# SarodYatawatta/federated-pytorch-test

Hardware: NVIDIA H100
Metric: train_images_per_sec (higher is better)
Workload: dtype tf32

## Files before the change

federated_pytorch_test_b200/csrc/bindings.cpp:

```cpp
#include <ATen/cuda/CUDAContext.h>
#include <c10/cuda/CUDAGuard.h>
#include <torch/extension.h>

#include <cstdlib>

#include "fedb200.h"

namespace fb = fedb200;
using torch::Tensor;

static cudaStream_t cur_stream() { return at::cuda::getCurrentCUDAStream().stream(); }
static const float* fptr(const Tensor& t) { return t.data_ptr<float>(); }
static float* fptr_mut(Tensor& t) { return t.data_ptr<float>(); }
static const float* opt_ptr(const c10::optional<Tensor>& t) { return (t.has_value() && t->defined()) ? t->data_ptr<float>() : nullptr; }

#define CHECK_F32_CUDA(x) TORCH_CHECK((x).is_cuda() && (x).scalar_type() == torch::kFloat32, #x " must be a CUDA float32 tensor")
#define CHECK_CONTIG(x) TORCH_CHECK((x).is_contiguous(), #x " must be contiguous")

void adam_prox(Tensor x, Tensor g, Tensor m, Tensor v, Tensor step, double lr, double b1, double b2, double eps,
               c10::optional<Tensor> z, c10::optional<Tensor> y, double rho, double l1, double l2,
               c10::optional<Tensor> rho_dev) {
  CHECK_F32_CUDA(x); CHECK_CONTIG(x); CHECK_CONTIG(g); CHECK_CONTIG(m); CHECK_CONTIG(v);
  c10::cuda::CUDAGuard guard(x.device());
  fb::adam_prox(fptr_mut(x), fptr(g), fptr_mut(m), fptr_mut(v), step.data_ptr<int>(), (int)x.numel(), (float)lr, (float)b1,
                (float)b2, (float)eps, opt_ptr(z), opt_ptr(y), (float)rho, (float)l1, (float)l2, cur_stream(), opt_ptr(rho_dev));
}
void bump_step(Tensor step) {
  c10::cuda::CUDAGuard guard(step.device());
  fb::bump_step(step.data_ptr<int>(), cur_stream());
}
Tensor l1_l2(Tensor g) {
  CHECK_F32_CUDA(g); CHECK_CONTIG(g);
  c10::cuda::CUDAGuard guard(g.device());
  auto out = torch::empty({2}, g.options());
  fb::l1_l2(fptr(g), (int)g.numel(), fptr_mut(out), cur_stream());
  return out;
}
std::vector<Tensor> make_pair(Tensor g, Tensor gprev, Tensor d, double t, double trust) {
  CHECK_F32_CUDA(g); CHECK_CONTIG(g); CHECK_CONTIG(gprev); CHECK_CONTIG(d);
  c10::cuda::CUDAGuard guard(g.device());
  auto y = torch::empty_like(g), s = torch::empty_like(g);
  auto out = torch::empty({3}, g.options());
  fb::make_pair(fptr(g), fptr(gprev), fptr(d), (float)t, (float)trust, fptr_mut(y), fptr_mut(s), (int)g.numel(), fptr_mut(out), cur_stream());
  return {y, s, out};
}
Tensor welford(Tensor g, Tensor mean, Tensor m2, int64_t n_iter) {
  CHECK_F32_CUDA(g);
  c10::cuda::CUDAGuard guard(g.device());
  auto out = torch::empty({1}, g.options());
  fb::welford(fptr(g), fptr_mut(mean), fptr_mut(m2), (int)g.numel(), 1.0f / (float)n_iter, fptr_mut(out), cur_stream());
  return out;
}
Tensor penalty_value(Tensor x, c10::optional<Tensor> z, c10::optional<Tensor> y, double rho, double l1, double l2) {
  CHECK_F32_CUDA(x); CHECK_CONTIG(x);
  c10::cuda::CUDAGuard guard(x.device());
  auto out = torch::empty({1}, x.options());
  fb::penalty_value(fptr(x), opt_ptr(z), opt_ptr(y), (float)rho, (float)l1, (float)l2, (int)x.numel(), fptr_mut(out), cur_stream());
  return out;
}
void penalty_grad(Tensor g, Tensor x, c10::optional<Tensor> z, c10::optional<Tensor> y, double rho, double l1, double l2) {
  CHECK_F32_CUDA(g); CHECK_CONTIG(g); CHECK_CONTIG(x);
  c10::cuda::CUDAGuard guard(g.device());
  fb::penalty_grad(fptr_mut(g), fptr(x), opt_ptr(z), opt_ptr(y), (float)rho, (float)l1, (float)l2, (int)g.numel(), cur_stream());
}
Tensor multi_dot(std::vector<Tensor> a, std::vector<Tensor> b) {
  TORCH_CHECK(a.size() == b.size() && !a.empty() && a.size() <= 8, "multi_dot: 1..8 pairs");
  c10::cuda::CUDAGuard guard(a[0].device());
  std::vector<const float*> pa, pb;
  for (size_t i = 0; i < a.size(); ++i) {
    CHECK_F32_CUDA(a[i]); CHECK_CONTIG(a[i]); CHECK_CONTIG(b[i]);
    TORCH_CHECK(a[i].numel() == a[0].numel() && b[i].numel() == a[0].numel(), "multi_dot: equal lengths required");
    pa.push_back(fptr(a[i])); pb.push_back(fptr(b[i]));
  }
  auto out = torch::empty({(int64_t)a.size()}, a[0].options());
  fb::multi_dot(pa.data(), pb.data(), (int)a.size(), (int)a[0].numel(), fptr_mut(out), cur_stream());
  return out;
}
Tensor lbfgs_two_loop(Tensor Y, Tensor S, Tensor order, Tensor g, double hdiag) {
  CHECK_F32_CUDA(Y); CHECK_CONTIG(Y); CHECK_CONTIG(S); CHECK_CONTIG(g);
  TORCH_CHECK(order.scalar_type() == torch::kInt32 && order.is_cuda(), "order must be a CUDA int32 tensor");
  c10::cuda::CUDAGuard guard(g.device());
  const int k = (int)order.numel(), n = (int)g.numel();
  auto d = torch::empty_like(g);
  auto work = torch::empty({(int64_t)fb::lbfgs_two_loop_work_floats(k)}, g.options());
  fb::lbfgs_two_loop(fptr(Y), fptr(S), order.data_ptr<int>(), k, n, (int)Y.size(1), fptr(g), (float)hdiag, fptr_mut(d), fptr_mut(work), cur_stream());
  return d;
}

Tensor normalize_u8(Tensor u8, std::vector<double> mean, std::vector<double> stdv, int64_t c_out, bool to_nchw) {
  TORCH_CHECK(u8.is_cuda() && u8.scalar_type() == torch::kUInt8 && u8.dim() == 4 && u8.size(3) == 3 && u8.is_contiguous(),
              "normalize_u8 expects a contiguous CUDA uint8 [N,H,W,3] tensor");
  c10::cuda::CUDAGuard guard(u8.device());
  const int64_t N = u8.size(0), H = u8.size(1), W = u8.size(2);
  float m3[3] = {(float)mean[0], (float)mean[1], (float)mean[2]}, s3[3] = {(float)stdv[0], (float)stdv[1], (float)stdv[2]};
  auto opts = torch::TensorOptions().dtype(torch::kFloat32).device(u8.device());
  Tensor out = to_nchw ? torch::empty({N, 3, H, W}, opts) : torch::empty({N, H, W, c_out}, opts);
  fb::normalize_u8_nhwc(u8.data_ptr<uint8_t>(), fptr_mut(out), (int)(N * H * W), (int)c_out, m3, s3, to_nchw ? 1 : 0, (int)H, (int)W, cur_stream());
  return out;
}
Tensor augment_normalize_u8(Tensor u8, c10::optional<Tensor> rows, int64_t key, int64_t counter, std::vector<double> mean,
                            std::vector<double> stdv, bool to_nchw) {
  TORCH_CHECK(u8.is_cuda() && u8.scalar_type() == torch::kUInt8 && u8.dim() == 4 && u8.size(3) == 3 && u8.is_contiguous(),
              "augment_normalize_u8 expects a contiguous CUDA uint8 [N,H,W,3] tensor");
  TORCH_CHECK(counter >= 0, "augment_normalize_u8: negative counter");
  c10::cuda::CUDAGuard guard(u8.device());
  int64_t N = u8.size(0);
  const int64_t H = u8.size(1), W = u8.size(2);
  const int64_t* rp = nullptr;
  if (rows.has_value() && rows->defined()) {
    TORCH_CHECK(rows->is_cuda() && rows->device() == u8.device() && rows->scalar_type() == torch::kInt64 && rows->dim() == 1 &&
                    rows->is_contiguous(),
                "augment_normalize_u8: rows must be a contiguous int64 vector on the images' device");
    N = rows->numel();
    rp = rows->data_ptr<int64_t>();
  }
  TORCH_CHECK(N * H * W < (int64_t(1) << 31), "augment_normalize_u8: batch too large");
  float m3[3] = {(float)mean[0], (float)mean[1], (float)mean[2]}, s3[3] = {(float)stdv[0], (float)stdv[1], (float)stdv[2]};
  auto opts = torch::TensorOptions().dtype(torch::kFloat32).device(u8.device());
  Tensor out = to_nchw ? torch::empty({N, 3, H, W}, opts) : torch::empty({N, H, W, 3}, opts);
  if (N == 0) return out;
  fb::augment_normalize_u8(u8.data_ptr<uint8_t>(), rp, fptr_mut(out), (int)N, (int)H, (int)W, (uint64_t)key, (uint64_t)counter,
                           m3, s3, to_nchw ? 1 : 0, cur_stream());
  return out;
}
void col_stats(Tensor y, Tensor stats) {
  CHECK_F32_CUDA(y); CHECK_CONTIG(y);
  c10::cuda::CUDAGuard guard(y.device());
  const int C = (int)y.size(-1);
  fb::col_stats(fptr(y), fptr_mut(stats), (int)(y.numel() / C), C, cur_stream());
}
std::vector<Tensor> bn_elu_fwd(Tensor y, c10::optional<Tensor> stats, Tensor gamma, Tensor beta, c10::optional<Tensor> residual,
                               c10::optional<Tensor> running_mean, c10::optional<Tensor> running_var, double eps,
                               double momentum, bool act, bool self_clean, bool use_running) {
  CHECK_F32_CUDA(y); CHECK_CONTIG(y);
  c10::cuda::CUDAGuard guard(y.device());
  const int C = (int)y.size(-1);
  const int M = (int)(y.numel() / C);
  auto out = torch::empty_like(y);
  float* rm = (running_mean.has_value() && running_mean->defined()) ? running_mean->data_ptr<float>() : nullptr;
  float* rv = (running_var.has_value() && running_var->defined()) ? running_var->data_ptr<float>() : nullptr;
  if (use_running) {
    TORCH_CHECK(rm != nullptr && rv != nullptr, "bn_elu_fwd: use_running needs running_mean and running_var");
    fb::bn_elu_fwd(fptr(y), nullptr, fptr(gamma), fptr(beta), opt_ptr(residual), fptr_mut(out), rm, rv, nullptr, nullptr, M, C,
                   (float)eps, 0.f, act ? 1 : 0, 0, cur_stream(), 1);
    return {out, Tensor(), Tensor()};
  }
  TORCH_CHECK(stats.has_value() && stats->defined(), "bn_elu_fwd: stats required");
  auto sm = torch::empty({C}, y.options()), si = torch::empty({C}, y.options());
  TORCH_CHECK(stats->numel() >= 2 * C + (self_clean ? 1 : 0), "stats buffer too small");
  fb::bn_elu_fwd(fptr(y), stats->data_ptr<float>(), fptr(gamma), fptr(beta), opt_ptr(residual), fptr_mut(out), rm, rv, fptr_mut(sm),
                 fptr_mut(si), M, C, (float)eps, (float)momentum, act ? 1 : 0, self_clean ? 1 : 0, cur_stream());
  return {out, sm, si};
}
std::vector<Tensor> bn_elu_bwd(Tensor dout, c10::optional<Tensor> out, Tensor y, Tensor mean, Tensor invstd, Tensor gamma,
                               c10::optional<Tensor> beta, c10::optional<Tensor> dgamma, c10::optional<Tensor> dbeta,
                               bool want_dres, bool act, c10::optional<Tensor> sums_buf) {
  CHECK_F32_CUDA(dout); CHECK_CONTIG(dout); CHECK_CONTIG(y);
  c10::cuda::CUDAGuard guard(y.device());
  const int C = (int)y.size(-1);
  const int M = (int)(y.numel() / C);
  const float* outp = nullptr;
  if (out.has_value() && out->defined()) { CHECK_CONTIG((*out)); outp = out->data_ptr<float>(); }
  const float* betap = opt_ptr(beta);
  static const bool fused_optin = [] { const char* e = std::getenv("FEDB200_BN_BWD_FUSED"); return e != nullptr && std::atoi(e) != 0; }();
  const bool persistent = !fused_optin && sums_buf.has_value() && sums_buf->defined();
  if (persistent) TORCH_CHECK(sums_buf->numel() == 2 * C + 1 && sums_buf->is_contiguous(), "bn_elu_bwd: sums buffer must be [2C + 1]");
  auto sums = persistent ? *sums_buf : torch::empty({2 * C + 1}, y.options());
  auto dy = torch::empty_like(y);
  Tensor dres;
  if (want_dres) dres = torch::empty_like(y);
  float* dg = (dgamma.has_value() && dgamma->defined()) ? dgamma->data_ptr<float>() : nullptr;
  float* db = (dbeta.has_value() && dbeta->defined()) ? dbeta->data_ptr<float>() : nullptr;
  if (fused_optin && fb::bn_elu_bwd_fused(fptr(dout), outp, fptr(y), fptr(mean), fptr(invstd), fptr(gamma), betap, fptr_mut(sums),
                                          fptr_mut(dy), want_dres ? dres.data_ptr<float>() : nullptr, dg, db, M, C, act ? 1 : 0,
                                          cur_stream()))
    return {dy, dres};
  fb::bn_elu_bwd_reduce(fptr(dout), outp, fptr(y), fptr(mean), fptr(invstd), fptr(gamma), betap, fptr_mut(sums), M, C,
                        act ? 1 : 0, persistent ? 1 : 0, cur_stream());
  fb::bn_elu_bwd_apply(fptr(dout), outp, fptr(y), fptr(mean), fptr(invstd), fptr(gamma), betap, fptr_mut(sums), fptr_mut(dy),
                       want_dres ? dres.data_ptr<float>() : nullptr, dg, db, M, C, act ? 1 : 0, persistent ? 1 : 0, cur_stream());
  return {dy, dres};
}
std::vector<Tensor> head_fwd(Tensor x, Tensor w, c10::optional<Tensor> bias) {
  CHECK_F32_CUDA(x); CHECK_CONTIG(x); CHECK_F32_CUDA(w); CHECK_CONTIG(w);
  TORCH_CHECK(x.dim() == 4 && w.dim() == 2 && x.size(3) == w.size(1), "head_fwd: x [N,H,W,C], w [O,C]");
  c10::cuda::CUDAGuard guard(x.device());
  const int NB = (int)x.size(0), HW = (int)(x.size(1) * x.size(2)), C = (int)x.size(3), O = (int)w.size(0);
  auto pooled = torch::empty({NB, C}, x.options());
  auto logits = torch::empty({NB, O}, x.options());
  fb::head_fwd(fptr(x), fptr(w), opt_ptr(bias), fptr_mut(pooled), fptr_mut(logits), NB, HW, C, O, cur_stream());
  return {logits, pooled};
}
Tensor head_bwd(Tensor dlogits, Tensor w, int64_t H, int64_t W) {
  CHECK_F32_CUDA(dlogits); CHECK_CONTIG(dlogits); CHECK_F32_CUDA(w); CHECK_CONTIG(w);
  c10::cuda::CUDAGuard guard(dlogits.device());
  const int NB = (int)dlogits.size(0), O = (int)dlogits.size(1), C = (int)w.size(1);
  auto dx = torch::empty({NB, H, W, C}, dlogits.options());
  fb::head_bwd(fptr(dlogits), fptr(w), fptr_mut(dx), NB, (int)(H * W), C, O, cur_stream());
  return dx;
}
Tensor avgpool_nhwc(Tensor x) {
  CHECK_F32_CUDA(x); CHECK_CONTIG(x);
  c10::cuda::CUDAGuard guard(x.device());
  auto out = torch::empty({x.size(0), x.size(3)}, x.options());
  fb::avgpool_nhwc(fptr(x), fptr_mut(out), (int)x.size(0), (int)(x.size(1) * x.size(2)), (int)x.size(3), cur_stream());
  return out;
}
Tensor avgpool_nhwc_bwd(Tensor dout, int64_t H, int64_t W) {
  CHECK_F32_CUDA(dout); CHECK_CONTIG(dout);
  c10::cuda::CUDAGuard guard(dout.device());
  auto dx = torch::empty({dout.size(0), H, W, dout.size(1)}, dout.options());
  fb::avgpool_nhwc_bwd(fptr(dout), fptr_mut(dx), (int)dout.size(0), (int)(H * W), (int)dout.size(1), cur_stream());
  return dx;
}
Tensor weight_flip(Tensor w) {
  CHECK_F32_CUDA(w); CHECK_CONTIG(w);
  c10::cuda::CUDAGuard guard(w.device());
  auto out = torch::empty({w.size(3), w.size(1), w.size(2), w.size(0)}, w.options());
  fb::weight_krsc_flip(fptr(w), fptr_mut(out), (int)w.size(0), (int)w.size(3), (int)w.size(1), (int)w.size(2), cur_stream());
  return out;
}

Tensor convT_pack(Tensor w) {
  CHECK_F32_CUDA(w);
  TORCH_CHECK(w.dim() == 4 && w.size(2) == 4 && w.size(3) == 4, "convT_pack: ConvTranspose2d(k=4) weight expected");
  c10::cuda::CUDAGuard guard(w.device());
  auto out = torch::empty({4 * w.size(1), 3, 3, w.size(0)}, w.options().memory_format(c10::MemoryFormat::Contiguous));
  fb::convT_pack(fptr(w), fptr_mut(out), (int)w.size(0), (int)w.size(1), w.stride(0), w.stride(1), w.stride(2), w.stride(3), cur_stream());
  return out;
}

Tensor linear_tf32(Tensor x, Tensor w, c10::optional<Tensor> bias, bool act) {
  CHECK_F32_CUDA(x); CHECK_F32_CUDA(w); CHECK_CONTIG(x); CHECK_CONTIG(w);
  TORCH_CHECK(x.dim() == 2 && w.dim() == 2 && x.size(1) == w.size(1), "linear_tf32: x [M,K], w [N,K]");
  c10::cuda::CUDAGuard guard(x.device());
  const int M = (int)x.size(0), K = (int)x.size(1), N = (int)w.size(0);
  auto out = torch::empty({M, N}, x.options());
  fb::linear_tf32(fptr(x), fptr(w), opt_ptr(bias), fptr_mut(out), M, N, K, K, K, N, act ? 1 : 0, cur_stream());
  return out;
}
bool conv_supported(int64_t H_out, int64_t W_out, int64_t C_in, int64_t stride) {
  return fb::conv_geometry_supported((int)H_out, (int)W_out, (int)C_in, (int)stride);
}
int64_t conv_orientation(int64_t NB, int64_t H_out, int64_t W_out, int64_t C_out, int64_t stride) {
  return fb::pick_conv_orientation((int)NB, (int)H_out, (int)W_out, (int)C_out, (int)stride);
}
bool conv_window_reuse(int64_t H_out, int64_t W_out, int64_t C_in, int64_t C_out, int64_t kh, int64_t stride, int64_t dil) {
  return fb::conv_window_reuse((int)H_out, (int)W_out, (int)C_in, (int)C_out, (int)kh, (int)stride, (int)dil);
}
Tensor conv2d_nhwc(Tensor x, Tensor w, c10::optional<Tensor> stats, int64_t stride, int64_t pad, int64_t dil, int64_t orient) {
  CHECK_F32_CUDA(x); CHECK_F32_CUDA(w); CHECK_CONTIG(x); CHECK_CONTIG(w);
  TORCH_CHECK(x.dim() == 4 && w.dim() == 4 && x.size(3) == w.size(3), "conv2d_nhwc: x [N,H,W,Ci], w [Co,kh,kw,Ci]");
  c10::cuda::CUDAGuard guard(x.device());
  const int NB = (int)x.size(0), H = (int)x.size(1), W = (int)x.size(2), Ci = (int)x.size(3);
  const int Co = (int)w.size(0), kh = (int)w.size(1), kw = (int)w.size(2);
  const int Ho = (H + 2 * (int)pad - (int)dil * (kh - 1) - 1) / (int)stride + 1;
  const int Wo = (W + 2 * (int)pad - (int)dil * (kw - 1) - 1) / (int)stride + 1;
  auto y = torch::empty({NB, Ho, Wo, Co}, x.options());
  float* st = (stats.has_value() && stats->defined()) ? stats->data_ptr<float>() : nullptr;
  fb::conv2d_nhwc_tf32(fptr(x), fptr(w), fptr_mut(y), st, NB, H, W, Ci, Co, kh, kw, (int)stride, (int)pad, (int)dil, Ho, Wo, cur_stream(),
                       (int)orient);
  return y;
}

Tensor conv2d_nhwc_sized(Tensor x, Tensor w, c10::optional<Tensor> stats, int64_t stride, int64_t pad, int64_t dil,
                         int64_t Ho, int64_t Wo) {
  CHECK_F32_CUDA(x); CHECK_F32_CUDA(w); CHECK_CONTIG(x); CHECK_CONTIG(w);
  TORCH_CHECK(x.dim() == 4 && w.dim() == 4 && x.size(3) == w.size(3), "conv2d_nhwc: x [N,H,W,Ci], w [Co,kh,kw,Ci]");
  TORCH_CHECK(Ho > 0 && Wo > 0, "conv2d_nhwc_sized: positive output size");
  c10::cuda::CUDAGuard guard(x.device());
  const int NB = (int)x.size(0), H = (int)x.size(1), W = (int)x.size(2), Ci = (int)x.size(3);
  const int Co = (int)w.size(0), kh = (int)w.size(1), kw = (int)w.size(2);
  auto y = torch::empty({NB, Ho, Wo, Co}, x.options());
  float* st = (stats.has_value() && stats->defined()) ? stats->data_ptr<float>() : nullptr;
  fb::conv2d_nhwc_tf32(fptr(x), fptr(w), fptr_mut(y), st, NB, H, W, Ci, Co, kh, kw, (int)stride, (int)pad, (int)dil, (int)Ho,
                       (int)Wo, cur_stream());
  return y;
}

bool conv_wgrad_supported(int64_t Cx, int64_t Co, int64_t stride, int64_t Wo, int64_t Ho) {
  return fb::conv_wgrad_supported((int)Cx, (int)Co, (int)stride, (int)Wo, (int)Ho);
}
void conv_wgrad(Tensor x, Tensor dy, Tensor dw, int64_t stride, int64_t pad, int64_t dil) {
  CHECK_F32_CUDA(x); CHECK_F32_CUDA(dy); CHECK_F32_CUDA(dw); CHECK_CONTIG(x); CHECK_CONTIG(dy); CHECK_CONTIG(dw);
  TORCH_CHECK(x.dim() == 4 && dy.dim() == 4 && dw.dim() == 4 && x.size(0) == dy.size(0) && dw.size(0) == dy.size(3) &&
              dw.size(3) <= x.size(3), "conv_wgrad: x [N,H,W,Cx], dy [N,Ho,Wo,Co], dw [Co,kh,kw,Cw<=Cx]");
  c10::cuda::CUDAGuard guard(x.device());
  const int NB = (int)x.size(0), H = (int)x.size(1), W = (int)x.size(2), Cx = (int)x.size(3);
  const int Ho = (int)dy.size(1), Wo = (int)dy.size(2), Co = (int)dy.size(3);
  const int kh = (int)dw.size(1), kw = (int)dw.size(2), Cw = (int)dw.size(3);
  fb::conv_wgrad_tf32(fptr(x), fptr(dy), fptr_mut(dw), NB, H, W, Cx, Cw, Co, kh, kw, (int)stride, (int)pad, (int)dil, Ho, Wo,
                      cur_stream());
}

bool conv_shuffle_supported(int64_t Ho, int64_t Wo, int64_t Cin, int64_t Ci) {
  return fb::conv_shuffle_supported((int)Ho, (int)Wo, (int)Cin, (int)Ci);
}
Tensor conv2d_nhwc_shuffle(Tensor x, Tensor w, int64_t pad, int64_t Ho, int64_t Wo) {
  CHECK_F32_CUDA(x); CHECK_F32_CUDA(w); CHECK_CONTIG(x); CHECK_CONTIG(w);
  TORCH_CHECK(x.dim() == 4 && w.dim() == 4 && x.size(3) == w.size(3) && w.size(0) % 4 == 0, "conv2d_nhwc_shuffle: x [N,H,W,Cin], w [4*Ci,kh,kw,Cin]");
  c10::cuda::CUDAGuard guard(x.device());
  const int NB = (int)x.size(0), H = (int)x.size(1), W = (int)x.size(2), Cin = (int)x.size(3);
  const int C4 = (int)w.size(0), kh = (int)w.size(1), kw = (int)w.size(2);
  auto out = torch::empty({NB, 2 * Ho, 2 * Wo, C4 / 4}, x.options());
  fb::conv2d_nhwc_shuffle_tf32(fptr(x), fptr(w), fptr_mut(out), NB, H, W, Cin, C4, kh, kw, (int)pad, (int)Ho, (int)Wo, cur_stream());
  return out;
}

bool conv_multidil_supported(int64_t Ho, int64_t Wo, int64_t Ci, int64_t stride, int64_t branches) {
  return fb::conv_multidil_supported((int)Ho, (int)Wo, (int)Ci, (int)stride, (int)branches);
}
Tensor conv2d_nhwc_multidil(Tensor x, Tensor w, c10::optional<Tensor> bias, bool act, int64_t kh, int64_t stride,
                            std::vector<int64_t> dils, std::vector<int64_t> pads, int64_t Ho, int64_t Wo) {
  CHECK_F32_CUDA(x); CHECK_F32_CUDA(w); CHECK_CONTIG(x); CHECK_CONTIG(w);
  TORCH_CHECK(x.dim() == 4 && w.dim() == 4 && x.size(3) == w.size(3), "conv2d_nhwc_multidil: x [N,H,W,Ci], w [Co,B*kh,kw,Ci]");
  const int B = (int)dils.size();
  TORCH_CHECK(B >= 1 && B <= 8 && (int)pads.size() == B && w.size(1) == B * kh, "conv2d_nhwc_multidil: branch tables");
  c10::cuda::CUDAGuard guard(x.device());
  const int NB = (int)x.size(0), H = (int)x.size(1), W = (int)x.size(2), Ci = (int)x.size(3);
  const int Co = (int)w.size(0), kw = (int)w.size(2);
  if (bias.has_value() && bias->defined()) TORCH_CHECK(bias->numel() == Co && bias->is_contiguous(), "bias must be [Co]");
  int d[8], pd[8];
  for (int b = 0; b < B; ++b) { d[b] = (int)dils[b]; pd[b] = (int)pads[b]; }
  auto y = torch::empty({NB, Ho, Wo, Co}, x.options());
  fb::conv2d_nhwc_multidil_tf32(fptr(x), fptr(w), opt_ptr(bias), act ? 1 : 0, fptr_mut(y), NB, H, W, Ci, Co, B, (int)kh, kw,
                                (int)stride, d, pd, (int)Ho, (int)Wo, cur_stream());
  return y;
}

Tensor conv2d_nhwc_accumulate(Tensor x, Tensor w, Tensor y, int64_t stride, int64_t pad, int64_t dil, int64_t orient) {
  CHECK_F32_CUDA(x); CHECK_F32_CUDA(w); CHECK_F32_CUDA(y); CHECK_CONTIG(x); CHECK_CONTIG(w); CHECK_CONTIG(y);
  TORCH_CHECK(x.dim() == 4 && w.dim() == 4 && y.dim() == 4 && x.size(3) == w.size(3), "conv2d_nhwc_accumulate: x [N,H,W,Ci], w [Co,kh,kw,Ci]");
  c10::cuda::CUDAGuard guard(x.device());
  const int NB = (int)x.size(0), H = (int)x.size(1), W = (int)x.size(2), Ci = (int)x.size(3);
  const int Co = (int)w.size(0), kh = (int)w.size(1), kw = (int)w.size(2);
  const int Ho = (H + 2 * (int)pad - (int)dil * (kh - 1) - 1) / (int)stride + 1;
  const int Wo = (W + 2 * (int)pad - (int)dil * (kw - 1) - 1) / (int)stride + 1;
  TORCH_CHECK(y.size(0) == NB && y.size(1) == Ho && y.size(2) == Wo && y.size(3) == Co, "conv2d_nhwc_accumulate: y must be [N,Ho,Wo,Co]");
  fb::conv2d_nhwc_accumulate_tf32(fptr(x), fptr(w), fptr_mut(y), NB, H, W, Ci, Co, kh, kw, (int)stride, (int)pad, (int)dil, Ho, Wo,
                                  cur_stream(), (int)orient);
  return y;
}

Tensor conv2d_nhwc_bias_act(Tensor x, Tensor w, c10::optional<Tensor> bias, bool act, int64_t stride, int64_t pad, int64_t dil) {
  CHECK_F32_CUDA(x); CHECK_F32_CUDA(w); CHECK_CONTIG(x); CHECK_CONTIG(w);
  TORCH_CHECK(x.dim() == 4 && w.dim() == 4 && x.size(3) == w.size(3), "conv2d_nhwc: x [N,H,W,Ci], w [Co,kh,kw,Ci]");
  c10::cuda::CUDAGuard guard(x.device());
  const int NB = (int)x.size(0), H = (int)x.size(1), W = (int)x.size(2), Ci = (int)x.size(3);
  const int Co = (int)w.size(0), kh = (int)w.size(1), kw = (int)w.size(2);
  const int Ho = (H + 2 * (int)pad - (int)dil * (kh - 1) - 1) / (int)stride + 1;
  const int Wo = (W + 2 * (int)pad - (int)dil * (kw - 1) - 1) / (int)stride + 1;
  TORCH_CHECK(Ho > 0 && Wo > 0, "conv2d_nhwc_bias_act: empty output");
  if (bias.has_value() && bias->defined()) TORCH_CHECK(bias->numel() == Co && bias->is_contiguous(), "bias must be [Co]");
  auto y = torch::empty({NB, Ho, Wo, Co}, x.options());
  fb::conv2d_nhwc_bias_act_tf32(fptr(x), fptr(w), opt_ptr(bias), act ? 1 : 0, fptr_mut(y), NB, H, W, Ci, Co, kh, kw, (int)stride,
                                (int)pad, (int)dil, Ho, Wo, cur_stream());
  return y;
}

Tensor conv2d_nhwc_bn_eval(Tensor x, Tensor w, Tensor gamma, Tensor beta, Tensor running_mean, Tensor running_var, double eps,
                           c10::optional<Tensor> residual, bool act, int64_t stride, int64_t pad) {
  CHECK_F32_CUDA(x); CHECK_F32_CUDA(w); CHECK_CONTIG(x); CHECK_CONTIG(w);
  TORCH_CHECK(x.dim() == 4 && w.dim() == 4 && x.size(3) == w.size(3), "conv2d_nhwc_bn_eval: x [N,H,W,Ci], w [Co,kh,kw,Ci]");
  c10::cuda::CUDAGuard guard(x.device());
  const int NB = (int)x.size(0), H = (int)x.size(1), W = (int)x.size(2), Ci = (int)x.size(3);
  const int Co = (int)w.size(0), kh = (int)w.size(1), kw = (int)w.size(2);
  const int Ho = (H + 2 * (int)pad - (kh - 1) - 1) / (int)stride + 1;
  const int Wo = (W + 2 * (int)pad - (kw - 1) - 1) / (int)stride + 1;
  TORCH_CHECK(Ho > 0 && Wo > 0, "conv2d_nhwc_bn_eval: empty output");
  for (const Tensor* t : {&gamma, &beta, &running_mean, &running_var}) {
    CHECK_F32_CUDA((*t));
    TORCH_CHECK(t->numel() == Co && t->is_contiguous(), "conv2d_nhwc_bn_eval: BatchNorm parameters and statistics must be [Co]");
  }
  const float* res = nullptr;
  if (residual.has_value() && residual->defined()) {
    CHECK_F32_CUDA((*residual)); CHECK_CONTIG((*residual));
    TORCH_CHECK(residual->dim() == 4 && residual->size(0) == NB && residual->size(1) == Ho && residual->size(2) == Wo &&
                residual->size(3) == Co, "conv2d_nhwc_bn_eval: residual must be [N,Ho,Wo,Co]");
    res = residual->data_ptr<float>();
    TORCH_CHECK((reinterpret_cast<uintptr_t>(res) & 15) == 0, "conv2d_nhwc_bn_eval: residual must be 16-byte aligned");
  }
  auto y = torch::empty({NB, Ho, Wo, Co}, x.options());
  fb::conv2d_nhwc_bn_eval_tf32(fptr(x), fptr(w), fptr(gamma), fptr(beta), fptr(running_mean), fptr(running_var), (float)eps, res,
                               act ? 1 : 0, fptr_mut(y), NB, H, W, Ci, Co, kh, kw, (int)stride, (int)pad, 1, Ho, Wo, cur_stream());
  return y;
}

std::vector<Tensor> cross_entropy_fwd(Tensor logits, Tensor labels) {
  CHECK_F32_CUDA(logits); CHECK_CONTIG(logits);
  TORCH_CHECK(labels.scalar_type() == torch::kInt64 && labels.is_cuda(), "labels must be CUDA int64");
  c10::cuda::CUDAGuard guard(logits.device());
  auto loss = torch::empty({}, logits.options());
  auto probs = torch::empty_like(logits);
  fb::cross_entropy_fwd(fptr(logits), (const long long*)labels.data_ptr<int64_t>(), fptr_mut(loss), fptr_mut(probs),
                        (int)logits.size(0), (int)logits.size(1), cur_stream());
  return {loss, probs};
}
Tensor cross_entropy_bwd(Tensor probs, Tensor labels, Tensor gout) {
  c10::cuda::CUDAGuard guard(probs.device());
  auto d = torch::empty_like(probs);
  auto g = gout.contiguous();
  fb::cross_entropy_bwd(fptr(probs), (const long long*)labels.data_ptr<int64_t>(), fptr(g), fptr_mut(d), (int)probs.size(0),
                        (int)probs.size(1), cur_stream());
  return d;
}
Tensor vae_loss_fwd(Tensor recon, Tensor x, Tensor mu, Tensor logvar) {
  CHECK_F32_CUDA(recon); CHECK_CONTIG(recon); CHECK_CONTIG(x); CHECK_CONTIG(mu); CHECK_CONTIG(logvar);
  c10::cuda::CUDAGuard guard(recon.device());
  auto out = torch::empty({}, recon.options());
  fb::vae_loss_fwd(fptr(recon), fptr(x), (int)recon.numel(), fptr(mu), fptr(logvar), (int)mu.numel(), fptr_mut(out), cur_stream());
  return out;
}
std::vector<Tensor> vae_loss_bwd(Tensor recon, Tensor x, Tensor mu, Tensor logvar, Tensor gout) {
  c10::cuda::CUDAGuard guard(recon.device());
  auto dr = torch::empty_like(recon), dm = torch::empty_like(mu), dl = torch::empty_like(logvar);
  auto g = gout.contiguous();
  fb::vae_loss_bwd(fptr(recon), fptr(x), (int)recon.numel(), fptr(mu), fptr(logvar), (int)mu.numel(), fptr(g), fptr_mut(dr),
                   fptr_mut(dm), fptr_mut(dl), cur_stream());
  return {dr, dm, dl};
}

Tensor linear_f32(Tensor x, Tensor w, c10::optional<Tensor> bias, bool act) {
  CHECK_F32_CUDA(x); CHECK_F32_CUDA(w); CHECK_CONTIG(x); CHECK_CONTIG(w);
  TORCH_CHECK(x.dim() == 2 && w.dim() == 2 && x.size(1) == w.size(1), "linear_f32: x [M,K], w [N,K]");
  c10::cuda::CUDAGuard guard(x.device());
  const int M = (int)x.size(0), K = (int)x.size(1), N = (int)w.size(0);
  auto out = torch::empty({M, N}, x.options());
  fb::gemm_f32(fptr(x), fptr(w), opt_ptr(bias), fptr_mut(out), M, N, K, K, 1, 1, K, N, act ? 1 : 0, 0, cur_stream());
  return out;
}
Tensor linear_f32_dgrad(Tensor dz, Tensor w) {
  CHECK_F32_CUDA(dz); CHECK_F32_CUDA(w); CHECK_CONTIG(dz); CHECK_CONTIG(w);
  c10::cuda::CUDAGuard guard(dz.device());
  const int M = (int)dz.size(0), N = (int)dz.size(1), K = (int)w.size(1);
  auto dx = torch::empty({M, K}, dz.options());
  fb::gemm_f32(fptr(dz), fptr(w), nullptr, fptr_mut(dx), M, K, N, N, 1, K, 1, K, 0, 0, cur_stream());
  return dx;
}
void linear_f32_wgrad(Tensor dz, Tensor x, Tensor dw, bool accumulate) {
  CHECK_F32_CUDA(dz); CHECK_F32_CUDA(x); CHECK_F32_CUDA(dw); CHECK_CONTIG(dz); CHECK_CONTIG(x); CHECK_CONTIG(dw);
  c10::cuda::CUDAGuard guard(dz.device());
  const int M = (int)dz.size(0), N = (int)dz.size(1), K = (int)x.size(1);
  TORCH_CHECK(dw.size(0) == N && dw.size(1) == K && x.size(0) == M, "linear_f32_wgrad: shape mismatch");
  fb::gemm_f32(fptr(dz), fptr(x), nullptr, fptr_mut(dw), N, K, M, 1, N, K, 1, K, 0, accumulate ? 1 : 0, cur_stream());
}
void act_bwd_bias(Tensor dout, c10::optional<Tensor> out, c10::optional<Tensor> dz, c10::optional<Tensor> db, bool act) {
  CHECK_F32_CUDA(dout); CHECK_CONTIG(dout);
  c10::cuda::CUDAGuard guard(dout.device());
  const int C = (int)dout.size(-1);
  float* dzp = (dz.has_value() && dz->defined()) ? dz->data_ptr<float>() : nullptr;
  float* dbp = (db.has_value() && db->defined()) ? db->data_ptr<float>() : nullptr;
  TORCH_CHECK(!act || (out.has_value() && out->defined()), "act_bwd_bias: the activation output is needed for ELU'");
  fb::act_bwd_bias(fptr(dout), opt_ptr(out), dzp, dbp, (long long)dout.numel(), C, act ? 1 : 0, cur_stream());
}
std::vector<Tensor> maxpool2x2_fwd(Tensor x) {
  CHECK_F32_CUDA(x);
  TORCH_CHECK(x.dim() == 4, "maxpool2x2: 4-D tensor expected");
  const bool nhwc = !x.is_contiguous() && x.is_contiguous(at::MemoryFormat::ChannelsLast);
  TORCH_CHECK(nhwc || x.is_contiguous(), "maxpool2x2: contiguous or channels_last input");
  c10::cuda::CUDAGuard guard(x.device());
  const int N = (int)x.size(0), C = (int)x.size(1), H = (int)x.size(2), W = (int)x.size(3);
  auto fmt = nhwc ? at::MemoryFormat::ChannelsLast : at::MemoryFormat::Contiguous;
  auto y = torch::empty({N, C, H / 2, W / 2}, x.options().memory_format(fmt));
  auto idx = torch::empty({N, C, H / 2, W / 2}, x.options().dtype(torch::kUInt8).memory_format(fmt));
  fb::maxpool2x2_fwd(fptr(x), fptr_mut(y), idx.data_ptr<uint8_t>(), N, C, H, W, nhwc ? 1 : 0, cur_stream());
  return {y, idx};
}
Tensor maxpool2x2_bwd(Tensor dy, Tensor idx, int64_t H, int64_t W) {
  CHECK_F32_CUDA(dy);
  const bool nhwc = !idx.is_contiguous() && idx.is_contiguous(at::MemoryFormat::ChannelsLast);
  auto fmt = nhwc ? at::MemoryFormat::ChannelsLast : at::MemoryFormat::Contiguous;
  Tensor d = dy.contiguous(fmt);
  c10::cuda::CUDAGuard guard(dy.device());
  const int N = (int)dy.size(0), C = (int)dy.size(1);
  auto dx = torch::empty({N, C, H, W}, dy.options().memory_format(fmt));
  fb::maxpool2x2_bwd(fptr(d), idx.data_ptr<uint8_t>(), fptr_mut(dx), N, C, (int)H, (int)W, nhwc ? 1 : 0, cur_stream());
  return dx;
}
void argmax_count(Tensor logits, Tensor labels, Tensor counter) {
  CHECK_F32_CUDA(logits); CHECK_CONTIG(logits);
  TORCH_CHECK(labels.scalar_type() == torch::kInt64 && counter.scalar_type() == torch::kInt64 && counter.numel() >= 2, "argmax_count: int64 labels / counter[2]");
  c10::cuda::CUDAGuard guard(logits.device());
  fb::argmax_count(fptr(logits), (const long long*)labels.data_ptr<int64_t>(), (long long*)counter.data_ptr<int64_t>(), (int)logits.size(0),
                   (int)logits.size(1), cur_stream());
}
int64_t info_nce_max_p() { return fb::info_nce_max_p(); }
int64_t info_nce_scratch_floats() { return fb::info_nce_scratch_floats(); }
std::vector<Tensor> info_nce_fwd(Tensor Z, Tensor Zh, Tensor scratch) {
  CHECK_F32_CUDA(Z); CHECK_F32_CUDA(Zh); CHECK_CONTIG(Z); CHECK_CONTIG(Zh);
  c10::cuda::CUDAGuard guard(Z.device());
  const int R = (int)Z.size(0), P = (int)Z.size(1);
  auto loss = torch::empty({}, Z.options());
  auto coef = torch::empty({(int64_t)P * P + 2 * P}, Z.options());
  fb::info_nce_fwd(fptr(Z), fptr(Zh), R, P, fptr_mut(scratch), fptr_mut(loss), fptr_mut(coef), cur_stream());
  return {loss, coef};
}
std::vector<Tensor> info_nce_bwd(Tensor Z, Tensor Zh, Tensor coef, Tensor gout) {
  CHECK_F32_CUDA(Z); CHECK_CONTIG(Z); CHECK_CONTIG(Zh);
  c10::cuda::CUDAGuard guard(Z.device());
  auto dZ = torch::empty_like(Z), dZh = torch::empty_like(Zh);
  fb::info_nce_bwd(fptr(Z), fptr(Zh), fptr(coef), fptr(gout), fptr_mut(dZ), fptr_mut(dZh), (int)Z.size(0), (int)Z.size(1), cur_stream());
  return {dZ, dZh};
}
Tensor gauss_nll_rows_fwd(Tensor x, Tensor mu, Tensor s2) {
  CHECK_F32_CUDA(x); CHECK_F32_CUDA(mu); CHECK_F32_CUDA(s2); CHECK_CONTIG(x); CHECK_CONTIG(mu); CHECK_CONTIG(s2);
  c10::cuda::CUDAGuard guard(x.device());
  const int B = (int)x.size(0), D = (int)x.size(1), rows = (int)mu.size(0);
  TORCH_CHECK(mu.size(1) == D && rows % B == 0, "gauss_nll_rows: mu [k*B, D]");
  auto out = torch::empty({rows}, x.options());
  fb::gauss_nll_rows_fwd(fptr(x), fptr(mu), fptr(s2), fptr_mut(out), rows, B, D, cur_stream());
  return out;
}
std::vector<Tensor> gauss_nll_rows_bwd(Tensor x, Tensor mu, Tensor s2, Tensor grow) {
  CHECK_F32_CUDA(x); CHECK_CONTIG(x); CHECK_CONTIG(mu); CHECK_CONTIG(s2); CHECK_CONTIG(grow);
  c10::cuda::CUDAGuard guard(x.device());
  auto dmu = torch::empty_like(mu), ds2 = torch::empty_like(s2);
  fb::gauss_nll_rows_bwd(fptr(x), fptr(mu), fptr(s2), fptr(grow), fptr_mut(dmu), fptr_mut(ds2), (int)mu.size(0), (int)x.size(0),
                         (int)x.size(1), cur_stream());
  return {dmu, ds2};
}
bool smallconv_supported(int64_t Ci, int64_t Co, int64_t k) { return fb::smallconv_supported((int)Ci, (int)Co, (int)k); }
std::vector<Tensor> smallconv_fwd(Tensor x, Tensor w, c10::optional<Tensor> bias, int64_t pad, bool act, bool pool) {
  CHECK_F32_CUDA(x); CHECK_F32_CUDA(w); CHECK_CONTIG(x); CHECK_CONTIG(w);
  c10::cuda::CUDAGuard guard(x.device());
  const int NB = (int)x.size(0), Ci = (int)x.size(1), H = (int)x.size(2), W = (int)x.size(3), Co = (int)w.size(0), k = (int)w.size(2);
  const int Ho = H + 2 * (int)pad - k + 1, Wo = W + 2 * (int)pad - k + 1;
  auto y = torch::empty({NB, Co, pool ? Ho / 2 : Ho, pool ? Wo / 2 : Wo}, x.options());
  Tensor idx = pool ? torch::empty(y.sizes(), x.options().dtype(torch::kUInt8)) : torch::empty({0}, x.options().dtype(torch::kUInt8));
  fb::smallconv_fwd(fptr(x), fptr(w), opt_ptr(bias), fptr_mut(y), pool ? idx.data_ptr<uint8_t>() : nullptr, NB, Ci, H, W, Co, k,
                    (int)pad, act ? 1 : 0, pool ? 1 : 0, cur_stream());
  return {y, idx};
}
Tensor smallconv_unpool_actbwd(Tensor dy, Tensor yout, Tensor idx, int64_t Ho, int64_t Wo, bool act, bool pool) {
  CHECK_F32_CUDA(dy); CHECK_CONTIG(dy); CHECK_CONTIG(yout);
  c10::cuda::CUDAGuard guard(dy.device());
  auto dz = torch::empty({dy.size(0), dy.size(1), Ho, Wo}, dy.options());
  fb::smallconv_unpool_actbwd(fptr(dy), fptr(yout), pool ? idx.data_ptr<uint8_t>() : nullptr, fptr_mut(dz),
                              (long long)(dy.size(0) * dy.size(1)), (int)Ho, (int)Wo, act ? 1 : 0, pool ? 1 : 0, cur_stream());
  return dz;
}
Tensor smallconv_dgrad(Tensor dz, Tensor w, int64_t H, int64_t W, int64_t pad) {
  CHECK_F32_CUDA(dz); CHECK_CONTIG(dz); CHECK_CONTIG(w);
  c10::cuda::CUDAGuard guard(dz.device());
  const int NB = (int)dz.size(0), Co = (int)w.size(0), Ci = (int)w.size(1), k = (int)w.size(2);
  auto dx = torch::empty({NB, Ci, H, W}, dz.options());
  fb::smallconv_dgrad(fptr(dz), fptr(w), fptr_mut(dx), NB, Ci, (int)H, (int)W, Co, k, (int)pad, cur_stream());
  return dx;
}
void smallconv_wgrad(Tensor dz, Tensor x, Tensor dw, c10::optional<Tensor> db, int64_t pad) {
  CHECK_F32_CUDA(dz); CHECK_CONTIG(dz); CHECK_CONTIG(x); CHECK_CONTIG(dw);
  c10::cuda::CUDAGuard guard(dz.device());
  const int NB = (int)x.size(0), Ci = (int)x.size(1), H = (int)x.size(2), W = (int)x.size(3), Co = (int)dw.size(0), k = (int)dw.size(2);
  float* dbp = (db.has_value() && db->defined()) ? db->data_ptr<float>() : nullptr;
  fb::smallconv_wgrad(fptr(dz), fptr(x), fptr_mut(dw), dbp, NB, Ci, H, W, Co, k, (int)pad, cur_stream());
}

static void set_dp(fb::CommArgs& a, double dp_std, int64_t dp_key, const c10::optional<Tensor>& dp_t,
                   const c10::optional<Tensor>& dp_stats, const c10::optional<Tensor>& dp_valid) {
  if (!dp_t.has_value() || !dp_t->defined()) return;
  TORCH_CHECK(dp_t->is_cuda() && dp_t->scalar_type() == at::kLong && dp_t->numel() >= 1, "DP round counter: int64 CUDA tensor");
  TORCH_CHECK(dp_stats.has_value() && dp_stats->defined() && dp_stats->numel() >= fb::DP_STATS_FLOATS,
              "DP rounds need the dp_clip stats record");
  CHECK_F32_CUDA((*dp_stats));
  a.dp = 1;
  a.dp_std = (float)dp_std;
  a.dp_key = (unsigned long long)dp_key;
  a.dp_t = reinterpret_cast<long long*>(dp_t->data_ptr<int64_t>());
  a.dp_stats = dp_stats->data_ptr<float>() + fb::DP_NORM;
  if (dp_valid.has_value() && dp_valid->defined()) {
    TORCH_CHECK(dp_valid->is_cuda() && dp_valid->scalar_type() == at::kByte && dp_valid->is_contiguous() &&
                    dp_valid->numel() >= (a.n + fb::DP_CHUNK - 1) / fb::DP_CHUNK,
                "DP parameter layout: uint8 CUDA tensor with one count per 32-float chunk of the block");
    a.dp_valid = dp_valid->data_ptr<uint8_t>();
  }
}
static void set_q(fb::CommArgs& a, const std::vector<int64_t>& local_idx, int64_t q_bits, int64_t q_group, int64_t q_key,
                  const c10::optional<Tensor>& q_t, const std::vector<int64_t>& q_code_ptrs,
                  const std::vector<int64_t>& q_scale_ptrs, const std::vector<Tensor>& q_ef,
                  const c10::optional<Tensor>& q_part) {
  if (q_bits == 0) return;
  TORCH_CHECK(q_bits == 8 || q_bits == 4, "compressed rounds take 8 or 4 bits, got ", q_bits);
  TORCH_CHECK(q_group == fb::Q_GROUP, "compressed rounds use groups of ", fb::Q_GROUP, " coordinates, got ", q_group);
  TORCH_CHECK(q_t.has_value() && q_t->defined() && q_t->is_cuda() && q_t->scalar_type() == at::kLong && q_t->numel() >= 1,
              "compressed round counter: int64 CUDA tensor");
  TORCH_CHECK(q_part.has_value() && q_part->defined() && q_part->numel() >= fb::Q_PART_FLOATS, "compressed rounds need the statistics buffer");
  CHECK_F32_CUDA((*q_part));
  TORCH_CHECK((int)q_code_ptrs.size() == a.K && (int)q_scale_ptrs.size() == a.K, "compressed rounds need K payload pointers");
  TORCH_CHECK(q_ef.empty() || (int)q_ef.size() == a.n_local, "error feedback: one slice per local replica");
  a.qbits = (int)q_bits;
  a.q_key = (unsigned long long)q_key;
  a.q_t = reinterpret_cast<long long*>(q_t->data_ptr<int64_t>());
  a.q_part = q_part->data_ptr<float>();
  for (int k = 0; k < a.K; ++k) {
    TORCH_CHECK(q_code_ptrs[k] % 16 == 0 && q_scale_ptrs[k] % 4 == 0, "payload slices must be 16-byte aligned");
    a.q_codes[k] = reinterpret_cast<unsigned char*>(q_code_ptrs[k]);
    a.q_scales[k] = reinterpret_cast<float*>(q_scale_ptrs[k]);
  }
  for (int j = 0; j < a.n_local; ++j) {
    a.q_worker[j] = (int)local_idx[j];
    if (!q_ef.empty()) {
      CHECK_F32_CUDA(q_ef[j]); CHECK_CONTIG(q_ef[j]);
      TORCH_CHECK(q_ef[j].numel() == a.n, "error feedback slices must have the block's length");
      a.q_ef[j] = q_ef[j].data_ptr<float>();
    }
  }
}
static void set_samp(fb::CommArgs& a, int64_t samp_S, int64_t samp_key, const c10::optional<Tensor>& samp_t,
                     const c10::optional<Tensor>& client_n) {
  if (samp_S == 0) return;
  TORCH_CHECK(samp_t.has_value() && samp_t->defined() && samp_t->is_cuda() && samp_t->scalar_type() == at::kLong &&
                  samp_t->numel() >= 1, "sampled round counter: int64 CUDA tensor");
  TORCH_CHECK(client_n.has_value() && client_n->defined() && client_n->is_cuda() && client_n->scalar_type() == at::kInt &&
                  client_n->is_contiguous() && client_n->numel() == a.K, "sample counts: one int32 CUDA value per worker");
  a.samp_S = (int)samp_S;
  a.samp_key = (unsigned long long)samp_key;
  a.samp_t = reinterpret_cast<long long*>(samp_t->data_ptr<int64_t>());
  a.client_n = client_n->data_ptr<int>();
}
static void fill_ctrl(uint32_t** dst, const std::vector<int64_t>& ctrl_ptrs, int world) {
  for (int p = 0; p < world && p < (int)ctrl_ptrs.size(); ++p) dst[p] = reinterpret_cast<uint32_t*>(ctrl_ptrs[p]);
}
void block_reduce(int64_t mode, std::vector<int64_t> x_ptrs, std::vector<int64_t> y_ptrs, std::vector<int64_t> local_idx,
                  Tensor z, int64_t n, double rho, c10::optional<Tensor> rho_dev, Tensor out, Tensor scratch,
                  std::vector<int64_t> ctrl_ptrs, Tensor sync, int64_t world, int64_t rank, int64_t mc_x, int64_t mc_y,
                  int64_t mc_z, std::vector<int64_t> xw_ptrs, std::vector<int64_t> zw_ptrs, bool two_shot,
                  int64_t max_blocks, double timeout_s, int64_t agg, int64_t trim_b, double dp_std, int64_t dp_key,
                  c10::optional<Tensor> dp_t, c10::optional<Tensor> dp_stats, c10::optional<Tensor> dp_valid,
                  int64_t q_bits, int64_t q_group, int64_t q_key,
                  c10::optional<Tensor> q_t, std::vector<int64_t> q_code_ptrs, std::vector<int64_t> q_scale_ptrs,
                  std::vector<Tensor> q_ef, c10::optional<Tensor> q_part, int64_t samp_S, int64_t samp_key,
                  c10::optional<Tensor> samp_t, c10::optional<Tensor> client_n) {
  CHECK_F32_CUDA(z); CHECK_F32_CUDA(out); CHECK_F32_CUDA(scratch);
  TORCH_CHECK(out.numel() >= fb::COMM_OUT_FLOATS && scratch.numel() >= fb::COMM_SCRATCH_FLOATS, "out / scratch too small");
  c10::cuda::CUDAGuard guard(z.device());
  fb::CommArgs a{};
  a.mode = (int)mode; a.K = (int)x_ptrs.size(); a.n_local = (int)local_idx.size(); a.world = (int)world; a.rank = (int)rank;
  a.n = (int)n; a.rho = (float)rho; a.rho_dev = opt_ptr(rho_dev);
  a.two_shot = two_shot ? 1 : 0; a.max_blocks = (int)max_blocks;
  TORCH_CHECK(a.K <= fb::COMM_MAX_K && a.n_local <= fb::COMM_MAX_LOCAL && a.world <= fb::COMM_MAX_WORLD, "block_reduce: limits exceeded");
  for (int k = 0; k < a.K; ++k) {
    a.x[k] = reinterpret_cast<const float*>(x_ptrs[k]);
    a.y[k] = y_ptrs.empty() ? nullptr : reinterpret_cast<const float*>(y_ptrs[k]);
  }
  for (int j = 0; j < a.n_local; ++j) {
    a.xl[j] = reinterpret_cast<float*>(x_ptrs[local_idx[j]]);
    a.yl[j] = y_ptrs.empty() ? nullptr : reinterpret_cast<float*>(y_ptrs[local_idx[j]]);
  }
  for (int p = 0; p < a.world; ++p) {
    a.xw[p] = p < (int)xw_ptrs.size() ? reinterpret_cast<float*>(xw_ptrs[p]) : nullptr;
    a.zw[p] = p < (int)zw_ptrs.size() ? reinterpret_cast<float*>(zw_ptrs[p]) : nullptr;
  }
  if (a.two_shot) {
    if (a.mode == 0) {
      TORCH_CHECK(mc_x != 0 || (int)xw_ptrs.size() == a.world, "two-shot FedAvg needs broadcast targets");
    } else {
      TORCH_CHECK(mc_z != 0 || (int)zw_ptrs.size() == a.world, "two-shot FedProx/ADMM needs peer-mapped z");
    }
  }
  a.mc_x = reinterpret_cast<float*>(mc_x);
  a.mc_y = reinterpret_cast<float*>(mc_y);
  a.mc_z = reinterpret_cast<float*>(mc_z);
  a.z = z.data_ptr<float>();
  a.out = out.data_ptr<float>();
  a.scratch = scratch.data_ptr<float>();
  fill_ctrl(a.ctrl, ctrl_ptrs, a.world);
  a.sync = reinterpret_cast<uint32_t*>(sync.data_ptr<int>());
  a.timeout_cycles = (long long)(timeout_s * 1.9e9);
  a.agg = (int)agg; a.trim_b = (int)trim_b;
  set_dp(a, dp_std, dp_key, dp_t, dp_stats, dp_valid);
  set_q(a, local_idx, q_bits, q_group, q_key, q_t, q_code_ptrs, q_scale_ptrs, q_ef, q_part);
  set_samp(a, samp_S, samp_key, samp_t, client_n);
  fb::block_reduce_launch(a, cur_stream());
}

void block_reduce_fedopt(int64_t opt, double lr, double beta1, double beta2, double tau, Tensor m, c10::optional<Tensor> v,
                         std::vector<int64_t> x_ptrs, std::vector<int64_t> local_idx, Tensor z, int64_t n, Tensor out,
                         Tensor scratch, std::vector<int64_t> ctrl_ptrs, Tensor sync, int64_t world, int64_t rank,
                         int64_t mc_x, int64_t mc_m, int64_t mc_v, std::vector<int64_t> xw_ptrs,
                         std::vector<int64_t> mw_ptrs, std::vector<int64_t> vw_ptrs, bool two_shot, int64_t max_blocks,
                         double timeout_s, int64_t agg, int64_t trim_b, double dp_std, int64_t dp_key,
                         c10::optional<Tensor> dp_t, c10::optional<Tensor> dp_stats,
                         c10::optional<Tensor> dp_valid, int64_t q_bits, int64_t q_group, int64_t q_key,
                         c10::optional<Tensor> q_t, std::vector<int64_t> q_code_ptrs, std::vector<int64_t> q_scale_ptrs,
                         std::vector<Tensor> q_ef, c10::optional<Tensor> q_part, int64_t samp_S, int64_t samp_key,
                         c10::optional<Tensor> samp_t, c10::optional<Tensor> client_n) {
  TORCH_CHECK(opt >= fb::FEDOPT_AVGM && opt <= fb::FEDOPT_YOGI, "block_reduce_fedopt: unknown server optimizer ", opt);
  const bool adaptive = opt != fb::FEDOPT_AVGM;
  CHECK_F32_CUDA(z); CHECK_F32_CUDA(out); CHECK_F32_CUDA(scratch); CHECK_F32_CUDA(m); CHECK_CONTIG(m);
  TORCH_CHECK(out.numel() >= fb::COMM_OUT_FLOATS && scratch.numel() >= fb::COMM_SCRATCH_FLOATS, "out / scratch too small");
  TORCH_CHECK(z.numel() == n && m.numel() == n, "block_reduce_fedopt: z and m must have the block's length");
  if (adaptive) {
    TORCH_CHECK(v.has_value() && v->defined(), "block_reduce_fedopt: adaptive server optimizers need v");
    CHECK_F32_CUDA((*v)); CHECK_CONTIG((*v));
    TORCH_CHECK(v->numel() == n, "block_reduce_fedopt: v must have the block's length");
  }
  c10::cuda::CUDAGuard guard(z.device());
  fb::CommArgs a{};
  a.mode = 0; a.K = (int)x_ptrs.size(); a.n_local = (int)local_idx.size(); a.world = (int)world; a.rank = (int)rank;
  a.n = (int)n; a.two_shot = two_shot ? 1 : 0; a.max_blocks = (int)max_blocks;
  TORCH_CHECK(a.K <= fb::COMM_MAX_K && a.n_local <= fb::COMM_MAX_LOCAL && a.world <= fb::COMM_MAX_WORLD,
              "block_reduce_fedopt: limits exceeded");
  for (int k = 0; k < a.K; ++k) a.x[k] = reinterpret_cast<const float*>(x_ptrs[k]);
  for (int j = 0; j < a.n_local; ++j) a.xl[j] = reinterpret_cast<float*>(x_ptrs[local_idx[j]]);
  for (int p = 0; p < a.world; ++p) {
    a.xw[p] = p < (int)xw_ptrs.size() ? reinterpret_cast<float*>(xw_ptrs[p]) : nullptr;
    a.mw[p] = p < (int)mw_ptrs.size() ? reinterpret_cast<float*>(mw_ptrs[p]) : nullptr;
    a.vw[p] = p < (int)vw_ptrs.size() ? reinterpret_cast<float*>(vw_ptrs[p]) : nullptr;
  }
  if (a.two_shot) {
    TORCH_CHECK(mc_x != 0 || (int)xw_ptrs.size() == a.world, "two-shot FedOpt needs broadcast targets for the weights");
    TORCH_CHECK(mc_m != 0 || (int)mw_ptrs.size() == a.world, "two-shot FedOpt needs peer-mapped m");
    TORCH_CHECK(!adaptive || mc_v != 0 || (int)vw_ptrs.size() == a.world, "two-shot FedOpt needs peer-mapped v");
  }
  a.mc_x = reinterpret_cast<float*>(mc_x);
  a.mc_m = reinterpret_cast<float*>(mc_m);
  a.mc_v = reinterpret_cast<float*>(mc_v);
  a.z = z.data_ptr<float>();
  a.out = out.data_ptr<float>();
  a.scratch = scratch.data_ptr<float>();
  fill_ctrl(a.ctrl, ctrl_ptrs, a.world);
  a.sync = reinterpret_cast<uint32_t*>(sync.data_ptr<int>());
  a.timeout_cycles = (long long)(timeout_s * 1.9e9);
  a.opt = (int)opt;
  a.lr = (float)lr; a.beta1 = (float)beta1; a.beta2 = (float)beta2; a.tau = (float)tau;
  a.m = m.data_ptr<float>();
  a.v = adaptive ? v->data_ptr<float>() : nullptr;
  a.agg = (int)agg; a.trim_b = (int)trim_b;
  set_dp(a, dp_std, dp_key, dp_t, dp_stats, dp_valid);
  set_q(a, local_idx, q_bits, q_group, q_key, q_t, q_code_ptrs, q_scale_ptrs, q_ef, q_part);
  set_samp(a, samp_S, samp_key, samp_t, client_n);
  fb::block_reduce_launch(a, cur_stream());
}

void dp_clip(std::vector<Tensor> xs, Tensor z, double bound, Tensor stats, int64_t max_blocks) {
  TORCH_CHECK(!xs.empty() && xs.size() <= (size_t)fb::COMM_MAX_LOCAL, "dp_clip: bad replica count");
  CHECK_F32_CUDA(z); CHECK_CONTIG(z); CHECK_F32_CUDA(stats);
  TORCH_CHECK(stats.numel() >= fb::DP_STATS_FLOATS, "dp_clip: stats too small");
  c10::cuda::CUDAGuard guard(z.device());
  fb::DPClipArgs a{};
  a.n = (int)z.numel(); a.n_local = (int)xs.size(); a.max_blocks = (int)max_blocks; a.bound = (float)bound;
  for (int j = 0; j < a.n_local; ++j) {
    CHECK_F32_CUDA(xs[j]); CHECK_CONTIG(xs[j]);
    TORCH_CHECK(xs[j].numel() == a.n, "dp_clip: block slices must have z's length");
    a.x[j] = fptr_mut(xs[j]);
  }
  a.z = fptr(z);
  a.stats = fptr_mut(stats);
  fb::dp_clip_launch(a, cur_stream());
}

void bb_update(std::vector<Tensor> xs, std::vector<Tensor> ys, std::vector<Tensor> yhat0s, std::vector<Tensor> x0s, Tensor z,
               std::vector<int64_t> workers, int64_t K, Tensor rho_dev, Tensor log, Tensor scratch, Tensor out,
               std::vector<int64_t> ctrl_ptrs, Tensor sync, int64_t world, int64_t rank, double epsilon, double alphacorrmin,
               double rhomax, bool seed_only, int64_t max_blocks, double timeout_s) {
  TORCH_CHECK(!xs.empty() && xs.size() == x0s.size() && xs.size() <= (size_t)fb::COMM_MAX_LOCAL, "bb_update: bad replica count");
  CHECK_F32_CUDA(z); CHECK_F32_CUDA(rho_dev); CHECK_F32_CUDA(log); CHECK_F32_CUDA(scratch);
  TORCH_CHECK(log.numel() >= 8 * K && scratch.numel() >= fb::BB_SCRATCH_FLOATS, "bb_update: log / scratch too small");
  c10::cuda::CUDAGuard guard(z.device());
  fb::BBArgs a{};
  a.K = (int)K; a.n_local = (int)xs.size(); a.world = (int)world; a.rank = (int)rank; a.n = (int)xs[0].numel();
  a.seed_only = seed_only ? 1 : 0; a.max_blocks = (int)max_blocks;
  a.epsilon = (float)epsilon; a.alphacorrmin = (float)alphacorrmin; a.rhomax = (float)rhomax;
  for (int j = 0; j < a.n_local; ++j) {
    CHECK_F32_CUDA(xs[j]); CHECK_CONTIG(xs[j]); CHECK_CONTIG(x0s[j]);
    TORCH_CHECK(xs[j].numel() == a.n && x0s[j].numel() == a.n, "bb_update: equal lengths required");
    a.x[j] = fptr(xs[j]);
    a.x0[j] = fptr_mut(x0s[j]);
    if (!seed_only) {
      CHECK_CONTIG(ys[j]); CHECK_CONTIG(yhat0s[j]);
      a.y[j] = fptr(ys[j]);
      a.yhat0[j] = fptr_mut(yhat0s[j]);
    }
    a.worker[j] = (int)workers[j];
  }
  a.z = fptr(z);
  a.rho_dev = fptr_mut(rho_dev);
  a.log = fptr_mut(log);
  a.scratch = fptr_mut(scratch);
  a.out = fptr_mut(out);
  fill_ctrl(a.ctrl, ctrl_ptrs, a.world);
  a.sync = reinterpret_cast<uint32_t*>(sync.data_ptr<int>());
  a.timeout_cycles = (long long)(timeout_s * 1.9e9);
  fb::bb_update_launch(a, cur_stream());
}

py::bytes ipc_get_handle(int64_t ptr) {
  cudaIpcMemHandle_t h;
  cudaError_t e = cudaIpcGetMemHandle(&h, reinterpret_cast<void*>(ptr));
  TORCH_CHECK(e == cudaSuccess, "cudaIpcGetMemHandle: ", cudaGetErrorString(e));
  return py::bytes(reinterpret_cast<const char*>(&h), sizeof(h));
}
int64_t ipc_open_handle(py::bytes handle) {
  std::string s = handle;
  TORCH_CHECK(s.size() == sizeof(cudaIpcMemHandle_t), "bad IPC handle size");
  cudaIpcMemHandle_t h;
  memcpy(&h, s.data(), sizeof(h));
  void* p = nullptr;
  cudaError_t e = cudaIpcOpenMemHandle(&p, h, cudaIpcMemLazyEnablePeerAccess);
  TORCH_CHECK(e == cudaSuccess, "cudaIpcOpenMemHandle: ", cudaGetErrorString(e));
  return reinterpret_cast<int64_t>(p);
}
void ipc_close_handle(int64_t ptr) { cudaIpcCloseMemHandle(reinterpret_cast<void*>(ptr)); }

int64_t launch_count() { return (int64_t)fb::launch_count(); }

PYBIND11_MODULE(TORCH_EXTENSION_NAME, m) {
  m.doc() = "federated_pytorch_test_b200: hand-written sm_90a kernels";
  m.def("launch_count", &launch_count);
  m.def("adam_prox", &adam_prox);
  m.def("bump_step", &bump_step);
  m.def("l1_l2", &l1_l2);
  m.def("make_pair", &make_pair);
  m.def("welford", &welford);
  m.def("penalty_value", &penalty_value);
  m.def("penalty_grad", &penalty_grad);
  m.def("multi_dot", &multi_dot);
  m.def("lbfgs_two_loop", &lbfgs_two_loop);
  m.def("normalize_u8", &normalize_u8);
  m.def("augment_normalize_u8", &augment_normalize_u8, py::arg("u8"), py::arg("rows"), py::arg("key"), py::arg("counter"),
        py::arg("mean"), py::arg("std"), py::arg("to_nchw"));
  m.def("col_stats", &col_stats);
  m.def("head_fwd", &head_fwd);
  m.def("head_bwd", &head_bwd);
  m.def("bn_elu_fwd", &bn_elu_fwd, py::arg("y"), py::arg("stats"), py::arg("gamma"), py::arg("beta"), py::arg("residual"),
        py::arg("running_mean"), py::arg("running_var"), py::arg("eps"), py::arg("momentum"), py::arg("act"),
        py::arg("self_clean"), py::arg("use_running") = false);
  m.def("bn_elu_bwd", &bn_elu_bwd);
  m.def("avgpool_nhwc", &avgpool_nhwc);
  m.def("avgpool_nhwc_bwd", &avgpool_nhwc_bwd);
  m.def("weight_flip", &weight_flip);
  m.def("convT_pack", &convT_pack);
  m.def("linear_tf32", &linear_tf32);
  m.def("conv_supported", &conv_supported);
  m.def("conv_orientation", &conv_orientation);
  m.def("conv_window_reuse", &conv_window_reuse, py::arg("H_out"), py::arg("W_out"), py::arg("C_in"), py::arg("C_out"), py::arg("kh"),
        py::arg("stride") = 1, py::arg("dil") = 1);
  m.def("conv2d_nhwc", &conv2d_nhwc, py::arg("x"), py::arg("w"), py::arg("stats"), py::arg("stride"), py::arg("pad"), py::arg("dil"),
        py::arg("orient") = -1);
  m.def("conv2d_nhwc_sized", &conv2d_nhwc_sized);
  m.def("conv2d_nhwc_bias_act", &conv2d_nhwc_bias_act);
  m.def("conv2d_nhwc_bn_eval", &conv2d_nhwc_bn_eval);
  m.def("conv2d_nhwc_accumulate", &conv2d_nhwc_accumulate, py::arg("x"), py::arg("w"), py::arg("y"), py::arg("stride"), py::arg("pad"),
        py::arg("dil"), py::arg("orient") = -1);
  m.def("conv2d_nhwc_shuffle", &conv2d_nhwc_shuffle);
  m.def("conv_shuffle_supported", &conv_shuffle_supported);
  m.def("conv2d_nhwc_multidil", &conv2d_nhwc_multidil);
  m.def("conv_multidil_supported", &conv_multidil_supported);
  m.def("conv_wgrad", &conv_wgrad);
  m.def("conv_wgrad_supported", &conv_wgrad_supported);
  m.def("cross_entropy_fwd", &cross_entropy_fwd);
  m.def("cross_entropy_bwd", &cross_entropy_bwd);
  m.def("vae_loss_fwd", &vae_loss_fwd);
  m.def("vae_loss_bwd", &vae_loss_bwd);
  m.def("linear_f32", &linear_f32);
  m.def("linear_f32_dgrad", &linear_f32_dgrad);
  m.def("linear_f32_wgrad", &linear_f32_wgrad);
  m.def("act_bwd_bias", &act_bwd_bias);
  m.def("maxpool2x2_fwd", &maxpool2x2_fwd);
  m.def("maxpool2x2_bwd", &maxpool2x2_bwd);
  m.def("argmax_count", &argmax_count);
  m.def("info_nce_max_p", &info_nce_max_p);
  m.def("info_nce_scratch_floats", &info_nce_scratch_floats);
  m.def("info_nce_fwd", &info_nce_fwd);
  m.def("info_nce_bwd", &info_nce_bwd);
  m.def("gauss_nll_rows_fwd", &gauss_nll_rows_fwd);
  m.def("gauss_nll_rows_bwd", &gauss_nll_rows_bwd);
  m.def("smallconv_supported", &smallconv_supported);
  m.def("smallconv_fwd", &smallconv_fwd);
  m.def("smallconv_unpool_actbwd", &smallconv_unpool_actbwd);
  m.def("smallconv_dgrad", &smallconv_dgrad);
  m.def("smallconv_wgrad", &smallconv_wgrad);
  m.def("block_reduce", &block_reduce);
  m.def("block_reduce_fedopt", &block_reduce_fedopt);
  m.def("dp_clip", &dp_clip);
  m.def("bb_update", &bb_update);
  m.def("ipc_get_handle", &ipc_get_handle);
  m.def("ipc_open_handle", &ipc_open_handle);
  m.def("ipc_close_handle", &ipc_close_handle);
}
```

federated_pytorch_test_b200/csrc/fedb200.h:

```cpp
#pragma once
#include <cuda_runtime.h>
#include <stdint.h>

namespace fedb200 {

void count_launch(int n = 1);
long long launch_count();

bool pdl_enabled();
#ifdef __CUDACC__
__device__ __forceinline__ void pdl_wait() { asm volatile("griddepcontrol.wait;" ::: "memory"); }
__device__ __forceinline__ void pdl_launch_dependents() { asm volatile("griddepcontrol.launch_dependents;" ::: "memory"); }
__device__ __forceinline__ void pdl_prologue() {
  pdl_launch_dependents();
  pdl_wait();
}
template <typename... KArgs, typename... Args>
inline cudaError_t launch_pdl(void (*kernel)(KArgs...), dim3 grid, dim3 block, size_t smem, cudaStream_t stream,
                              Args&&... args) {
  cudaLaunchConfig_t cfg{};
  cfg.gridDim = grid;
  cfg.blockDim = block;
  cfg.dynamicSmemBytes = smem;
  cfg.stream = stream;
  cudaLaunchAttribute attr[1];
  attr[0].id = cudaLaunchAttributeProgrammaticStreamSerialization;
  attr[0].val.programmaticStreamSerializationAllowed = pdl_enabled() ? 1 : 0;
  cfg.attrs = attr;
  cfg.numAttrs = 1;
  return cudaLaunchKernelEx(&cfg, kernel, KArgs(args)...);
}
#endif

int pick_block_n(int M, int N);
void linear_tf32(const float* x, const float* w, const float* bias, float* out, int M, int N, int K, int ldx, int ldw,
                 int ldo, int act, cudaStream_t stream);
bool conv_geometry_supported(int H_out, int W_out, int C_in, int stride);
enum { CONV_ORIENT_AUTO = -1, CONV_ORIENT_ROW = 0, CONV_ORIENT_PIXEL = 1, CONV_ORIENT_PIXEL_PERTAP = 2 };
int pick_conv_orientation(int NB, int H_out, int W_out, int C_out, int stride);
bool conv_window_reuse(int H_out, int W_out, int C_in, int C_out, int kh, int stride, int dil);
void conv2d_nhwc_tf32(const float* x, const float* w, float* y, float* stats, int NB, int H, int W, int C_in, int C_out,
                      int kh, int kw, int stride, int pad, int dil, int H_out, int W_out, cudaStream_t stream,
                      int orient = CONV_ORIENT_AUTO);
void conv2d_nhwc_accumulate_tf32(const float* x, const float* w, float* y, int NB, int H, int W, int C_in, int C_out, int kh,
                                 int kw, int stride, int pad, int dil, int H_out, int W_out, cudaStream_t stream,
                                 int orient = CONV_ORIENT_AUTO);
void conv2d_nhwc_bias_act_tf32(const float* x, const float* w, const float* bias, int act, float* y, int NB, int H, int W,
                               int C_in, int C_out, int kh, int kw, int stride, int pad, int dil, int H_out, int W_out,
                               cudaStream_t stream);
void conv2d_nhwc_bn_eval_tf32(const float* x, const float* w, const float* gamma, const float* beta, const float* mean,
                              const float* var, float eps, const float* residual, int act, float* y, int NB, int H, int W,
                              int C_in, int C_out, int kh, int kw, int stride, int pad, int dil, int H_out, int W_out,
                              cudaStream_t stream);

bool conv_shuffle_supported(int H_out, int W_out, int C_in, int Ci_out);
void conv2d_nhwc_shuffle_tf32(const float* x, const float* w, float* out, int NB, int H, int W, int C_in, int C4, int kh, int kw,
                              int pad, int H_out, int W_out, cudaStream_t stream);
bool conv_multidil_supported(int H_out, int W_out, int C_in, int stride, int branches);
void conv2d_nhwc_multidil_tf32(const float* x, const float* w, const float* bias, int act, float* y, int NB, int H, int W, int C_in,
                               int C_out, int branches, int kh, int kw, int stride, const int* dils, const int* pads, int H_out,
                               int W_out, cudaStream_t stream);
bool conv_wgrad_supported(int C_x, int C_out, int stride, int W_out, int H_out);
void conv_wgrad_tf32(const float* x, const float* dy, float* dw, int NB, int H, int W, int C_x, int C_w, int C_out, int kh,
                     int kw, int stride, int pad, int dil, int H_out, int W_out, cudaStream_t stream);


void adam_prox(float* x, const float* g, float* m, float* v, const int* step_dev, int n, float lr, float b1, float b2,
               float eps, const float* z, const float* y, float rho, float l1, float l2, cudaStream_t s,
               const float* rho_dev = nullptr);
void bump_step(int* step_dev, cudaStream_t s);
void l1_l2(const float* g, int n, float* out2, cudaStream_t s);
void make_pair(const float* g, const float* gprev, const float* d, float t, float trust, float* y, float* sv, int n,
               float* out3, cudaStream_t s);
void welford(const float* g, float* mean, float* m2, int n, float inv_n, float* out1, cudaStream_t s);
void penalty_value(const float* x, const float* z, const float* y, float rho, float l1, float l2, int n, float* out1,
                   cudaStream_t s);
void penalty_grad(float* g, const float* x, const float* z, const float* y, float rho, float l1, float l2, int n,
                  cudaStream_t s);
void multi_dot(const float* const* a, const float* const* b, int npairs, int n, float* out, cudaStream_t s);
void lbfgs_two_loop(const float* Y, const float* S, const int* order, int k, int n, int ld, const float* g, float hdiag,
                    float* d, float* work, cudaStream_t s);
size_t lbfgs_two_loop_work_floats(int k);

void normalize_u8_nhwc(const uint8_t* in, float* out, int npix, int c_out, const float* mean3, const float* std3,
                       int to_nchw, int H, int W, cudaStream_t s);
void augment_normalize_u8(const uint8_t* in, const int64_t* rows, float* out, int n, int H, int W, uint64_t key,
                          uint64_t counter, const float* mean3, const float* std3, int to_nchw, cudaStream_t s);
void col_stats(const float* y, float* stats, int M, int C, cudaStream_t s);
void bn_elu_fwd(const float* y, float* stats, const float* gamma, const float* beta, const float* residual,
                float* out, float* running_mean, float* running_var, float* save_mean, float* save_invstd, int M, int C,
                float eps, float momentum, int act, int self_clean, cudaStream_t s, int use_running = 0);
void bn_elu_bwd_reduce(const float* dout, const float* out, const float* y, const float* mean, const float* invstd,
                       const float* gamma, const float* beta, float* sums, int M, int C, int act, int sums_clean, cudaStream_t s);
void bn_elu_bwd_apply(const float* dout, const float* out, const float* y, const float* mean, const float* invstd,
                      const float* gamma, const float* beta, float* sums, float* dy, float* dres, float* dgamma,
                      float* dbeta, int M, int C, int act, int self_clean, cudaStream_t s);
bool bn_elu_bwd_fused(const float* dout, const float* out, const float* y, const float* mean, const float* invstd,
                      const float* gamma, const float* beta, float* sums, float* dy, float* dres, float* dgamma,
                      float* dbeta, int M, int C, int act, cudaStream_t s);
void head_fwd(const float* x, const float* w, const float* bias, float* pooled, float* logits, int NB, int HW, int C, int O,
              cudaStream_t s);
void head_bwd(const float* dlogits, const float* w, float* dx, int NB, int HW, int C, int O, cudaStream_t s);
void avgpool_nhwc(const float* x, float* out, int NB, int HW, int C, cudaStream_t s);
void avgpool_nhwc_bwd(const float* dout, float* dx, int NB, int HW, int C, cudaStream_t s);
void weight_krsc_flip(const float* w, float* out, int C_out, int C_in, int kh, int kw, cudaStream_t s);
void convT_pack(const float* w, float* out, int Ci, int Co, long long s_ci, long long s_co, long long s_r, long long s_s, cudaStream_t s);

void cross_entropy_fwd(const float* logits, const long long* labels, float* loss, float* probs, int B, int C,
                       cudaStream_t s);
void cross_entropy_bwd(const float* probs, const long long* labels, const float* gout, float* dlogits, int B, int C,
                       cudaStream_t s);
void vae_loss_fwd(const float* recon, const float* x, int n, const float* mu, const float* logvar, int nl, float* out,
                  cudaStream_t s);
void vae_loss_bwd(const float* recon, const float* x, int n, const float* mu, const float* logvar, int nl,
                  const float* gout, float* drecon, float* dmu, float* dlogvar, cudaStream_t s);

void gemm_f32(const float* a, const float* b, const float* bias, float* c, int M, int N, int K, long long sa_i, long long sa_k,
              long long sb_k, long long sb_j, int ldc, int act, int accumulate, cudaStream_t s);
void act_bwd_bias(const float* dout, const float* out, float* dz, float* db, long long total, int C, int act, cudaStream_t s);
void maxpool2x2_fwd(const float* x, float* y, unsigned char* idx, int N, int C, int H, int W, int nhwc, cudaStream_t s);
void maxpool2x2_bwd(const float* dy, const unsigned char* idx, float* dx, int N, int C, int H, int W, int nhwc, cudaStream_t s);
void argmax_count(const float* logits, const long long* labels, long long* counter, int B, int C, cudaStream_t s);
int info_nce_max_p();
int info_nce_scratch_floats();
void info_nce_fwd(const float* Z, const float* Zh, int R, int P, float* scratch, float* loss, float* coef, cudaStream_t s);
void info_nce_bwd(const float* Z, const float* Zh, const float* coef, const float* gout, float* dZ, float* dZh, int R, int P,
                  cudaStream_t s);
void gauss_nll_rows_fwd(const float* x, const float* mu, const float* s2, float* rows, int nrows, int B, int D, cudaStream_t s);
void gauss_nll_rows_bwd(const float* x, const float* mu, const float* s2, const float* grow, float* dmu, float* ds2, int nrows,
                        int B, int D, cudaStream_t s);
bool smallconv_supported(int Ci, int Co, int k);
void smallconv_fwd(const float* x, const float* w, const float* bias, float* y, unsigned char* pidx, int NB, int Ci, int H, int W,
                   int Co, int k, int pad, int act, int pool, cudaStream_t s);
void smallconv_dgrad(const float* dz, const float* w, float* dx, int NB, int Ci, int H, int W, int Co, int k, int pad, cudaStream_t s);
void smallconv_wgrad(const float* dz, const float* x, float* dw, float* db, int NB, int Ci, int H, int W, int Co, int k, int pad,
                     cudaStream_t s);
void smallconv_unpool_actbwd(const float* dy, const float* yout, const unsigned char* pidx, float* dz, long long planes, int Ho, int Wo,
                             int act, int pool, cudaStream_t s);

constexpr int COMM_MAX_K = 64;
constexpr int COMM_MAX_LOCAL = 16;
constexpr int COMM_MAX_WORLD = 16;
constexpr int COMM_THREADS = 512;
constexpr int COMM_MAX_BLOCKS = 160;

constexpr int PAD_FLAG_A = 0;
constexpr int PAD_FLAG_B = PAD_FLAG_A + COMM_MAX_BLOCKS * COMM_MAX_WORLD;
constexpr int PAD_FLAG_C = PAD_FLAG_B + COMM_MAX_BLOCKS * COMM_MAX_WORLD;
constexpr int PAD_FLAG_D = PAD_FLAG_C + COMM_MAX_WORLD;
constexpr int PAD_PAYLOAD = PAD_FLAG_D + COMM_MAX_WORLD;
constexpr int PAD_BBROWS = PAD_PAYLOAD + 4 * COMM_MAX_WORLD;
constexpr int PAD_DP_PAYLOAD = PAD_BBROWS + 8 * COMM_MAX_K;
constexpr int PAD_Q_PAYLOAD = PAD_DP_PAYLOAD + 2 * COMM_MAX_WORLD;
constexpr int COMM_PAD_WORDS = 8192;
static_assert(PAD_Q_PAYLOAD + 2 * COMM_MAX_WORLD <= COMM_PAD_WORDS, "control pad too small");

constexpr int OUT_DUAL_SQ = 0, OUT_PRIMAL = 1, OUT_NONFINITE = 2, OUT_STATUS = 3, OUT_RHO = 4, OUT_EPOCH = 5, OUT_TWO_SHOT = 6;
constexpr int OUT_DP_CLIPPED = 8, OUT_DP_NORM_SUM = 9;
constexpr int OUT_Q_ERR_SQ = 10, OUT_Q_NORM_SQ = 11;
constexpr int COMM_OUT_FLOATS = 12;
constexpr int COMM_SCRATCH_FLOATS = 4 + COMM_MAX_LOCAL;

struct CommArgs {
  int mode;
  int K, n_local, world, rank;
  int n;
  int two_shot;
  int max_blocks;
  float rho;
  const float* rho_dev;
  const float* x[COMM_MAX_K];
  const float* y[COMM_MAX_K];
  float* xl[COMM_MAX_LOCAL];
  float* yl[COMM_MAX_LOCAL];
  float* xw[COMM_MAX_WORLD];
  float* zw[COMM_MAX_WORLD];
  float* mc_x;
  float* mc_y;
  float* mc_z;
  float* z;
  float* out;
  float* scratch;
  uint32_t* ctrl[COMM_MAX_WORLD];
  uint32_t* sync;
  long long timeout_cycles;
  int opt;
  float lr, beta1, beta2, tau;
  float* m;
  float* v;
  float* mw[COMM_MAX_WORLD];
  float* vw[COMM_MAX_WORLD];
  float* mc_m;
  float* mc_v;
  int agg;
  int trim_b;
  int dp;
  float dp_std;
  unsigned long long dp_key;
  long long* dp_t;
  const float* dp_stats;
  const unsigned char* dp_valid;
  int qbits;
  unsigned long long q_key;
  long long* q_t;
  int q_worker[COMM_MAX_LOCAL];
  unsigned char* q_codes[COMM_MAX_K];
  float* q_scales[COMM_MAX_K];
  float* q_ef[COMM_MAX_LOCAL];
  float* q_part;
  int samp_S;
  unsigned long long samp_key;
  long long* samp_t;
  const int* client_n;
};
constexpr int Q_GROUP = 128;
constexpr int Q_SEG = 16;
constexpr int Q_PART_FLOATS = 2 * COMM_MAX_BLOCKS;
constexpr int DP_CHUNK = 32;
constexpr int FEDOPT_NONE = 0, FEDOPT_AVGM = 1, FEDOPT_ADAGRAD = 2, FEDOPT_ADAM = 3, FEDOPT_YOGI = 4;
constexpr int AGG_MEAN = 0, AGG_MEDIAN = 1, AGG_TRIMMED = 2;
constexpr int COMM_MAX_K_ROBUST = 16;
void block_reduce_launch(const CommArgs& args, cudaStream_t s);

struct DPClipArgs {
  int n, n_local, max_blocks;
  float bound;
  float* x[COMM_MAX_LOCAL];
  const float* z;
  float* stats;
};
constexpr int DP_PART = 0;
constexpr int DP_NORM = 2 * COMM_MAX_LOCAL * COMM_MAX_BLOCKS;
constexpr int DP_CLIPPED = DP_NORM + COMM_MAX_LOCAL;
constexpr int DP_STATS_FLOATS = DP_CLIPPED + COMM_MAX_LOCAL;
void dp_clip_launch(const DPClipArgs& args, cudaStream_t s);

struct BBArgs {
  int K, n_local, world, rank, n;
  int seed_only;
  int max_blocks;
  float epsilon, alphacorrmin, rhomax;
  const float* x[COMM_MAX_LOCAL];
  const float* y[COMM_MAX_LOCAL];
  float* yhat0[COMM_MAX_LOCAL];
  float* x0[COMM_MAX_LOCAL];
  int worker[COMM_MAX_LOCAL];
  const float* z;
  float* rho_dev;
  float* log;
  float* scratch;
  uint32_t* ctrl[COMM_MAX_WORLD];
  uint32_t* sync;
  float* out;
  long long timeout_cycles;
};
constexpr int BB_SCRATCH_FLOATS = 8 * COMM_MAX_LOCAL + 8 + COMM_MAX_LOCAL;
void bb_update_launch(const BBArgs& args, cudaStream_t s);

}
```

federated_pytorch_test_b200/csrc/gemm_wgmma.cu:

```cuda
#include "fedb200.h"
#include "igemm_wgmma.cuh"
#include "wgrad_wgmma.cuh"

#include <algorithm>
#include <cstdlib>
#include <mutex>
#include <stdexcept>
#include <string>

namespace fedb200 {

typedef CUresult (*EncodeTiledFn)(CUtensorMap*, CUtensorMapDataType, cuuint32_t, void*, const cuuint64_t*,
                                  const cuuint64_t*, const cuuint32_t*, const cuuint32_t*, CUtensorMapInterleave,
                                  CUtensorMapSwizzle, CUtensorMapL2promotion, CUtensorMapFloatOOBfill);

static EncodeTiledFn encode_fn() {
  static EncodeTiledFn fn = nullptr;
  static std::once_flag once;
  std::call_once(once, [] {
    void* p = nullptr;
    cudaDriverEntryPointQueryResult q;
    cudaError_t e = cudaGetDriverEntryPoint("cuTensorMapEncodeTiled", &p, cudaEnableDefault, &q);
    if (e != cudaSuccess || q != cudaDriverEntryPointSuccess || p == nullptr)
      throw std::runtime_error("fedb200: cuTensorMapEncodeTiled unavailable (no CUDA driver?)");
    fn = reinterpret_cast<EncodeTiledFn>(p);
  });
  return fn;
}

static CUtensorMapDataType tmap_dtype() {
  const char* v = std::getenv("FEDB200_TMAP_F32");
  return (v && std::atoi(v) == 1) ? CU_TENSOR_MAP_DATA_TYPE_FLOAT32 : CU_TENSOR_MAP_DATA_TYPE_TFLOAT32;
}

static void check_cu(CUresult r, const char* what) {
  if (r != CUDA_SUCCESS) throw std::runtime_error(std::string("fedb200: ") + what + " failed with CUresult " + std::to_string(int(r)));
}

static CUtensorMapSwizzle swizzle_for(int cw) {
  return cw == 8 ? CU_TENSOR_MAP_SWIZZLE_32B : (cw == 16 ? CU_TENSOR_MAP_SWIZZLE_64B : CU_TENSOR_MAP_SWIZZLE_128B);
}
static CUtensorMap make_tmap_2d(const float* ptr, uint64_t rows, uint64_t cols, uint64_t ld, uint32_t box_rows, int cw = IG_BLOCK_K) {
  CUtensorMap m;
  cuuint64_t dims[2] = {cols, rows};
  cuuint64_t strides[1] = {ld * sizeof(float)};
  cuuint32_t box[2] = {uint32_t(cw), box_rows};
  cuuint32_t estr[2] = {1, 1};
  check_cu(encode_fn()(&m, tmap_dtype(),2, const_cast<float*>(ptr), dims, strides, box, estr,
                       CU_TENSOR_MAP_INTERLEAVE_NONE, swizzle_for(cw), CU_TENSOR_MAP_L2_PROMOTION_L2_256B,
                       CU_TENSOR_MAP_FLOAT_OOB_FILL_NONE),
           "cuTensorMapEncodeTiled(2d)");
  return m;
}

static CUtensorMap make_tmap_out(float* ptr, uint64_t rows, uint64_t cols, uint64_t ld, uint32_t box_rows) {
  CUtensorMap m;
  cuuint64_t dims[2] = {cols, rows};
  cuuint64_t strides[1] = {ld * sizeof(float)};
  cuuint32_t box[2] = {32, box_rows};
  cuuint32_t estr[2] = {1, 1};
  check_cu(encode_fn()(&m, CU_TENSOR_MAP_DATA_TYPE_FLOAT32, 2, ptr, dims, strides, box, estr, CU_TENSOR_MAP_INTERLEAVE_NONE,
                       CU_TENSOR_MAP_SWIZZLE_128B, CU_TENSOR_MAP_L2_PROMOTION_NONE, CU_TENSOR_MAP_FLOAT_OOB_FILL_NONE),
           "cuTensorMapEncodeTiled(out)");
  return m;
}

static CUtensorMap make_tmap_nhwc(const float* ptr, uint64_t N, uint64_t H, uint64_t W, uint64_t C, uint32_t boxN,
                                  uint32_t boxH, uint32_t boxW, uint32_t stride, int cw = IG_BLOCK_K) {
  CUtensorMap m;
  cuuint64_t dims[4] = {C, W, H, N};
  cuuint64_t strides[3] = {C * sizeof(float), W * C * sizeof(float), H * W * C * sizeof(float)};
  cuuint32_t box[4] = {uint32_t(cw), boxW * stride, boxH * stride, boxN};
  cuuint32_t estr[4] = {1, stride, stride, 1};
  check_cu(encode_fn()(&m, tmap_dtype(),4, const_cast<float*>(ptr), dims, strides, box, estr,
                       CU_TENSOR_MAP_INTERLEAVE_NONE, swizzle_for(cw), CU_TENSOR_MAP_L2_PROMOTION_L2_256B,
                       CU_TENSOR_MAP_FLOAT_OOB_FILL_NONE),
           "cuTensorMapEncodeTiled(nhwc)");
  return m;
}

static int env_int(const char* name, int dflt) {
  const char* v = std::getenv(name);
  return v ? std::atoi(v) : dflt;
}

static int num_sms() {
  static int sms = 0;
  if (sms == 0) {
    int dev = 0;
    cudaGetDevice(&dev);
    cudaDeviceGetAttribute(&sms, cudaDevAttrMultiProcessorCount, dev);
    if (sms <= 0) sms = 132;
  }
  return sms;
}

static const CUtensorMap* g_out_map_override = nullptr;

template <int BN, int ST, bool EVAL_BN>
static void launch(const CUtensorMap& ta, const CUtensorMap& tb, IgemmParams p, cudaStream_t stream) {
  using S = IgemmSmem<BN, ST>;
  auto kernel = igemm_wgmma_kernel<BN, ST, EVAL_BN>;
  static bool configured = false;
  if (!configured) {
    cudaError_t e = cudaFuncSetAttribute(kernel, cudaFuncAttributeMaxDynamicSharedMemorySize, S::TOTAL);
    if (e != cudaSuccess) throw std::runtime_error(std::string("fedb200: cudaFuncSetAttribute(igemm): ") + cudaGetErrorString(e));
    configured = true;
  }
  p.m_tiles = (p.M + IG_BLOCK_M - 1) / IG_BLOCK_M;
  p.n_tiles = (p.N + BN - 1) / BN;
  p.total_tiles = p.m_tiles * p.n_tiles * p.k_splits;
  p.tma_store = ((p.ldo & 3) == 0 && (reinterpret_cast<uintptr_t>(p.out) & 15) == 0 && env_int("FEDB200_TMA_STORE", 1) != 0) ? 1 : 0;
  if (g_out_map_override != nullptr) p.tma_store = 1;
  const CUtensorMap tc = g_out_map_override != nullptr ? *g_out_map_override : (p.tma_store ? make_tmap_out(p.out, p.M, p.N, p.ldo, 32) : ta);
  const int sms = num_sms();
  const int grid = (p.total_tiles < sms || env_int("FEDB200_PERSIST", 1) == 0) ? p.total_tiles : sms;
  cudaError_t e = launch_pdl(kernel, dim3(grid), dim3(IG_THREADS), S::TOTAL, stream, ta, tb, tc, p);
  if (e != cudaSuccess) throw std::runtime_error(std::string("fedb200: igemm launch: ") + cudaGetErrorString(e));
  count_launch();
}

template <bool EVAL_BN>
static void dispatch_tile(int bn, const CUtensorMap& ta, const CUtensorMap& tb, const IgemmParams& p, cudaStream_t s) {
  switch (bn) {
    case 32: launch<32, 8, EVAL_BN>(ta, tb, p, s); break;
    case 64: launch<64, 8, EVAL_BN>(ta, tb, p, s); break;
    default: launch<128, 6, EVAL_BN>(ta, tb, p, s); break;
  }
}
static void dispatch(int bn, const CUtensorMap& ta, const CUtensorMap& tb, const IgemmParams& p, cudaStream_t s) {
  if (p.bn_gamma != nullptr) dispatch_tile<true>(bn, ta, tb, p, s);
  else dispatch_tile<false>(bn, ta, tb, p, s);
}

constexpr int PIX_STAGES = 4;
constexpr int PIX_WIN_STAGES = 3;
constexpr int PIX_WIN_KH = 3;

template <int CO, int WIN_KH>
static void launch_pix(const CUtensorMap& ta, const CUtensorMap& tb, IgemmParams p, cudaStream_t stream) {
  constexpr bool WINDOW = WIN_KH > 0;
  static_assert(!WINDOW || CO == 64, "window reuse serves 64 output channels");
  constexpr int ST = WINDOW ? PIX_WIN_STAGES : PIX_STAGES;
  using S = PixSmem<CO, ST>;
  auto kernel = igemm_wgmma_pix_kernel<CO, ST, WIN_KH>;
  const int smem = WINDOW ? S::window_total(p.win_stage_bytes) : S::TOTAL;
  static bool configured = false;
  if (!configured) {
    cudaError_t e = cudaFuncSetAttribute(kernel, cudaFuncAttributeMaxDynamicSharedMemorySize, WINDOW ? 227 * 1024 : S::TOTAL);
    if (e != cudaSuccess) throw std::runtime_error(std::string("fedb200: cudaFuncSetAttribute(igemm_pix): ") + cudaGetErrorString(e));
    configured = true;
  }
  p.m_tiles = (p.M + PX_BLOCK_M - 1) / PX_BLOCK_M;
  p.n_tiles = 1;
  p.total_tiles = p.m_tiles;
  p.tma_store = 1;
  const CUtensorMap tc = make_tmap_out(p.out, p.M, p.N, p.ldo, 32);
  const int grid = std::min(p.total_tiles, num_sms());
  cudaError_t e = launch_pdl(kernel, dim3(grid), dim3(IG_THREADS), smem, stream, ta, tb, tc, p);
  if (e != cudaSuccess) throw std::runtime_error(std::string("fedb200: igemm_pix launch: ") + cudaGetErrorString(e));
  count_launch();
}

int pick_block_n(int M, int N) {
  (void)M;
  const int forced = env_int("FEDB200_BLOCK_N", 0);
  if (forced == 32 || forced == 64 || forced == 128) return forced;
  if (N <= 32) return 32;
  if (N <= 64) return 64;
  return 128;
}

static int pick_k_splits(int M, int N, int bn, int num_k_blocks) {
  const int ctas = ((M + IG_BLOCK_M - 1) / IG_BLOCK_M) * ((N + bn - 1) / bn);
  int splits = env_int("FEDB200_SPLITK", 0);
  if (splits <= 0) {
    const int wave = num_sms() + num_sms() / 8;
    splits = 1;
    while (splits < 8 && ctas * splits * 2 <= wave && num_k_blocks / (splits * 2) >= 6) splits *= 2;
  }
  return splits;
}

void linear_tf32(const float* x, const float* w, const float* bias, float* out, int M, int N, int K, int ldx, int ldw,
                 int ldo, int act, cudaStream_t stream) {
  if ((ldx & 3) || (ldw & 3) || (reinterpret_cast<uintptr_t>(x) & 15) || (reinterpret_cast<uintptr_t>(w) & 15))
    throw std::runtime_error("fedb200: linear_tf32 needs 16-byte aligned rows");
  const int bn = pick_block_n(M, N);
  CUtensorMap ta = make_tmap_2d(x, M, K, ldx, IG_BLOCK_M);
  CUtensorMap tb = make_tmap_2d(w, N, K, ldw, bn);
  IgemmParams p{};
  p.M = M; p.N = N;
  p.cblocks = (K + IG_BLOCK_K - 1) / IG_BLOCK_K;
  p.num_k_blocks = p.cblocks;
  p.taps_w = 1; p.b_cols_per_tap = 0; p.is_conv = 0;
  p.out = out; p.ldo = ldo; p.bias = bias; p.act = act; p.stats = nullptr;
  p.k_splits = 1; p.kb_per_split = p.num_k_blocks;
  dispatch(bn, ta, tb, p, stream);
}

bool conv_geometry_supported(int H_out, int W_out, int C_in, int stride) {
  if (W_out <= 0 || H_out <= 0 || W_out > 128 || (128 % W_out) != 0) return false;
  const int rows = 128 / W_out;
  if (rows <= H_out ? (H_out % rows) != 0 : (rows % H_out) != 0) return false;
  if ((C_in & 3) != 0) return false;
  if (stride < 1 || stride > 2) return false;
  if (W_out * stride > 256) return false;
  return true;
}

static bool pix_geometry_supported(int H_out, int W_out, int stride) {
  if (W_out > PX_BLOCK_M || (PX_BLOCK_M % W_out) != 0) return false;
  const int rows = PX_BLOCK_M / W_out;
  if (rows <= H_out ? (H_out % rows) != 0 : (rows % H_out) != 0) return false;
  return (rows <= H_out ? rows : H_out) * stride <= 256;
}

static int pix_window_stage_bytes(int H_out, int W_out, int C_in, int C_out, int kh, int stride, int dil) {
  if (C_out != 64 || stride != 1 || dil != 1 || kh != PIX_WIN_KH || C_in % IG_BLOCK_K != 0) return 0;
  if (!pix_geometry_supported(H_out, W_out, 1) || PX_BLOCK_M / W_out > H_out || (W_out * IG_BLOCK_K * 4) % 1024 != 0) return 0;
  const int win_rows = PX_BLOCK_M / W_out + kh - 1;
  if (win_rows > 256) return 0;
  const int stage = (win_rows * W_out + kh * C_out) * IG_BLOCK_K * 4;
  return PixSmem<64, PIX_WIN_STAGES>::window_total(stage) <= 227 * 1024 ? stage : 0;
}

bool conv_window_reuse(int H_out, int W_out, int C_in, int C_out, int kh, int stride, int dil) {
  return pix_window_stage_bytes(H_out, W_out, C_in, C_out, kh, stride, dil) > 0;
}

int pick_conv_orientation(int NB, int H_out, int W_out, int C_out, int stride) {
  if (env_int("FEDB200_BLOCK_N", 0) != 0) return CONV_ORIENT_ROW;
  if (C_out != 64 && C_out != 128) return CONV_ORIENT_ROW;
  if (!pix_geometry_supported(H_out, W_out, stride)) return CONV_ORIENT_ROW;
  const long long tiles = (static_cast<long long>(NB) * H_out * W_out + PX_BLOCK_M - 1) / PX_BLOCK_M;
  return tiles >= num_sms() - num_sms() / 8 ? CONV_ORIENT_PIXEL : CONV_ORIENT_ROW;
}

struct BnEvalArgs {
  const float* gamma;
  const float* beta;
  const float* mean;
  const float* var;
  float eps;
  const float* residual;
};

static void conv2d_generic(const float* x, const float* w, float* y, float* stats, const float* bias, int act, int NB, int H,
                           int W, int C_in, int C_out, int kh, int kw, int stride, int pad, int dil, int H_out, int W_out,
                           cudaStream_t stream, int accumulate = 0, const BnEvalArgs* eval_bn = nullptr,
                           int orient = CONV_ORIENT_ROW);

void conv2d_nhwc_tf32(const float* x, const float* w, float* y, float* stats, int NB, int H, int W, int C_in, int C_out,
                      int kh, int kw, int stride, int pad, int dil, int H_out, int W_out, cudaStream_t stream, int orient) {
  if (orient == CONV_ORIENT_AUTO) orient = pick_conv_orientation(NB, H_out, W_out, C_out, stride);
  conv2d_generic(x, w, y, stats, nullptr, 0, NB, H, W, C_in, C_out, kh, kw, stride, pad, dil, H_out, W_out, stream, 0, nullptr,
                 orient);
}

void conv2d_nhwc_bias_act_tf32(const float* x, const float* w, const float* bias, int act, float* y, int NB, int H, int W,
                               int C_in, int C_out, int kh, int kw, int stride, int pad, int dil, int H_out, int W_out,
                               cudaStream_t stream) {
  conv2d_generic(x, w, y, nullptr, bias, act, NB, H, W, C_in, C_out, kh, kw, stride, pad, dil, H_out, W_out, stream);
}

void conv2d_nhwc_accumulate_tf32(const float* x, const float* w, float* y, int NB, int H, int W, int C_in, int C_out, int kh,
                                 int kw, int stride, int pad, int dil, int H_out, int W_out, cudaStream_t stream, int orient) {
  if (orient == CONV_ORIENT_AUTO) orient = pick_conv_orientation(NB, H_out, W_out, C_out, stride);
  conv2d_generic(x, w, y, nullptr, nullptr, 0, NB, H, W, C_in, C_out, kh, kw, stride, pad, dil, H_out, W_out, stream, 1, nullptr,
                 orient);
}

void conv2d_nhwc_bn_eval_tf32(const float* x, const float* w, const float* gamma, const float* beta, const float* mean,
                              const float* var, float eps, const float* residual, int act, float* y, int NB, int H, int W,
                              int C_in, int C_out, int kh, int kw, int stride, int pad, int dil, int H_out, int W_out,
                              cudaStream_t stream) {
  const BnEvalArgs args{gamma, beta, mean, var, eps, residual};
  conv2d_generic(x, w, y, nullptr, nullptr, act, NB, H, W, C_in, C_out, kh, kw, stride, pad, dil, H_out, W_out, stream, 0, &args);
}

static int pick_tap_pack(int C_in) {
  if (env_int("FEDB200_TAP_PACK", 1) == 0 || C_in > 16 || (C_in & 3)) return IG_BLOCK_K;
  return C_in <= 8 ? 8 : 16;
}

static void conv2d_generic(const float* x, const float* w, float* y, float* stats, const float* bias, int act, int NB, int H,
                           int W, int C_in, int C_out, int kh, int kw, int stride, int pad, int dil, int H_out, int W_out,
                           cudaStream_t stream, int accumulate, const BnEvalArgs* eval_bn, int orient) {
  if (!conv_geometry_supported(H_out, W_out, C_in, stride))
    throw std::runtime_error("fedb200: conv geometry not supported by the wgmma path");
  const bool pix = orient == CONV_ORIENT_PIXEL || orient == CONV_ORIENT_PIXEL_PERTAP;
  if (pix && ((C_out != 64 && C_out != 128) || bias != nullptr || act != 0 || eval_bn != nullptr ||
              !pix_geometry_supported(H_out, W_out, stride) || (reinterpret_cast<uintptr_t>(y) & 15) != 0))
    throw std::runtime_error("fedb200: pixel-major convolution needs C_out 64 / 128, a plain, statistics or accumulate epilogue, "
                             "whole-row 256-pixel tiles and a 16-byte aligned output");
  const int win_stage = orient == CONV_ORIENT_PIXEL ? pix_window_stage_bytes(H_out, W_out, C_in, C_out, kh, stride, dil) : 0;
  const int tile_m = pix ? PX_BLOCK_M : IG_BLOCK_M;
  const int rows = tile_m / W_out;
  const int boxH = rows <= H_out ? rows : H_out;
  const int boxN = rows <= H_out ? 1 : rows / H_out;
  const int M = NB * H_out * W_out;
  const int bn = pix ? C_out : pick_block_n(M, C_out);
  const int cw = pick_tap_pack(C_in);
  CUtensorMap ta = make_tmap_nhwc(x, NB, H, W, C_in, boxN, win_stage ? boxH + kh - 1 : boxH, W_out, stride, cw);
  CUtensorMap tb = make_tmap_2d(w, C_out, uint64_t(kh) * kw * C_in, uint64_t(kh) * kw * C_in, bn, cw);
  IgemmParams p{};
  p.M = M; p.N = C_out;
  p.cblocks = (C_in + IG_BLOCK_K - 1) / IG_BLOCK_K;
  p.num_k_blocks = kh * kw * p.cblocks;
  p.taps_total = kh * kw;
  if (cw != IG_BLOCK_K) {
    p.cw = cw;
    p.num_k_blocks = (kh * kw + IG_BLOCK_K / cw - 1) / (IG_BLOCK_K / cw);
  }
  p.taps_w = kw; p.b_cols_per_tap = C_in; p.is_conv = 1;
  p.HW_out = H_out * W_out; p.W_out = W_out;
  p.stride = stride; p.pad = pad; p.dil = dil;
  p.out = y; p.ldo = C_out; p.bias = bias; p.act = act; p.stats = stats;
  p.k_splits = 1; p.kb_per_split = p.num_k_blocks;
  p.accumulate = accumulate;
  if (win_stage) {
    p.num_k_blocks = kw * p.cblocks;
    p.kb_per_split = p.num_k_blocks;
    p.win_rows = boxH + kh - 1;
    p.win_a_bytes = p.win_rows * W_out * IG_BLOCK_K * 4;
    p.win_stage_bytes = win_stage;
    launch_pix<64, PIX_WIN_KH>(ta, tb, p, stream);
    return;
  }
  if (pix) {
    if (C_out == 64) launch_pix<64, 0>(ta, tb, p, stream);
    else launch_pix<128, 0>(ta, tb, p, stream);
    return;
  }
  if (bias == nullptr && (act == 0 || eval_bn != nullptr)) {
    const int splits = pick_k_splits(M, C_out, bn, p.num_k_blocks);
    if (splits > 1) {
      p.kb_per_split = (p.num_k_blocks + splits - 1) / splits;
      p.k_splits = (p.num_k_blocks + p.kb_per_split - 1) / p.kb_per_split;
      p.stats = nullptr;
      if (!accumulate) cudaMemsetAsync(y, 0, size_t(M) * C_out * sizeof(float), stream);
    }
  }
  if (eval_bn != nullptr) {
    if ((C_out & 3) != 0) throw std::runtime_error("fedb200: eval-mode BatchNorm epilogue needs C_out % 4 == 0");
    if (p.k_splits > 1) {
      p.act = 0;
    } else {
      p.bn_gamma = eval_bn->gamma; p.bn_beta = eval_bn->beta; p.bn_mean = eval_bn->mean; p.bn_var = eval_bn->var;
      p.bn_eps = eval_bn->eps; p.residual = eval_bn->residual; p.ldr = C_out;
    }
  }
  dispatch(bn, ta, tb, p, stream);
  if (p.k_splits > 1 && stats != nullptr) col_stats(y, stats, M, C_out, stream);
  if (p.k_splits > 1 && eval_bn != nullptr)
    bn_elu_fwd(y, nullptr, eval_bn->gamma, eval_bn->beta, eval_bn->residual, y, const_cast<float*>(eval_bn->mean),
               const_cast<float*>(eval_bn->var), nullptr, nullptr, M, C_out, eval_bn->eps, 0.f, act, 0, stream, 1);
}

bool conv_shuffle_supported(int H_out, int W_out, int C_in, int Ci_out) {
  if (env_int("FEDB200_SHUFFLE_STORE", 1) == 0) return false;
  if (!conv_geometry_supported(H_out, W_out, C_in, 1)) return false;
  if (Ci_out % 32 != 0) return false;
  if (W_out > 32 || (32 % W_out) != 0) return false;
  return true;
}

void conv2d_nhwc_shuffle_tf32(const float* x, const float* w, float* out, int NB, int H, int W, int C_in, int C4, int kh, int kw,
                              int pad, int H_out, int W_out, cudaStream_t stream) {
  const int Ci = C4 / 4;
  if (!conv_shuffle_supported(H_out, W_out, C_in, Ci)) throw std::runtime_error("fedb200: shuffled conv store not supported for this shape");
  const int rows = 128 / W_out;
  const int boxH = rows <= H_out ? rows : H_out;
  const int boxN = rows <= H_out ? 1 : rows / H_out;
  const int M = NB * H_out * W_out;
  const int bn = pick_block_n(M, C4);
  CUtensorMap ta = make_tmap_nhwc(x, NB, H, W, C_in, boxN, boxH, W_out, 1);
  CUtensorMap tb = make_tmap_2d(w, C4, uint64_t(kh) * kw * C_in, uint64_t(kh) * kw * C_in, bn);
  CUtensorMap tc;
  {
    cuuint64_t dims[5] = {cuuint64_t(Ci), 2, cuuint64_t(W_out), 2, cuuint64_t(NB) * H_out};
    cuuint64_t strides[4] = {cuuint64_t(Ci) * 4, cuuint64_t(2) * Ci * 4, cuuint64_t(2) * W_out * Ci * 4, cuuint64_t(4) * W_out * Ci * 4};
    cuuint32_t box[5] = {32, 1, cuuint32_t(W_out), 1, cuuint32_t(32 / W_out)};
    cuuint32_t estr[5] = {1, 1, 1, 1, 1};
    check_cu(encode_fn()(&tc, CU_TENSOR_MAP_DATA_TYPE_FLOAT32, 5, out, dims, strides, box, estr, CU_TENSOR_MAP_INTERLEAVE_NONE,
                         CU_TENSOR_MAP_SWIZZLE_128B, CU_TENSOR_MAP_L2_PROMOTION_NONE, CU_TENSOR_MAP_FLOAT_OOB_FILL_NONE),
             "cuTensorMapEncodeTiled(shuffle)");
  }
  IgemmParams p{};
  p.M = M; p.N = C4;
  p.cblocks = (C_in + IG_BLOCK_K - 1) / IG_BLOCK_K;
  p.num_k_blocks = kh * kw * p.cblocks;
  p.taps_w = kw; p.b_cols_per_tap = C_in; p.is_conv = 1;
  p.HW_out = H_out * W_out; p.W_out = W_out;
  p.stride = 1; p.pad = pad; p.dil = 1;
  p.out = out; p.ldo = C4; p.bias = nullptr; p.act = 0; p.stats = nullptr;
  p.k_splits = 1; p.kb_per_split = p.num_k_blocks;
  p.shuffle_ci = Ci;
  {
    const int splits = pick_k_splits(M, C4, bn, p.num_k_blocks);
    if (splits > 1) {
      p.kb_per_split = (p.num_k_blocks + splits - 1) / splits;
      p.k_splits = (p.num_k_blocks + p.kb_per_split - 1) / p.kb_per_split;
      cudaMemsetAsync(out, 0, size_t(M) * C4 * sizeof(float), stream);
    }
  }
  g_out_map_override = &tc;
  try {
    dispatch(bn, ta, tb, p, stream);
  } catch (...) {
    g_out_map_override = nullptr;
    throw;
  }
  g_out_map_override = nullptr;
}

bool conv_multidil_supported(int H_out, int W_out, int C_in, int stride, int branches) {
  if (branches < 1 || branches > 8) return false;
  return conv_geometry_supported(H_out, W_out, C_in, stride);
}

void conv2d_nhwc_multidil_tf32(const float* x, const float* w, const float* bias, int act, float* y, int NB, int H, int W, int C_in,
                               int C_out, int branches, int kh, int kw, int stride, const int* dils, const int* pads, int H_out,
                               int W_out, cudaStream_t stream) {
  if (!conv_multidil_supported(H_out, W_out, C_in, stride, branches))
    throw std::runtime_error("fedb200: multi-dilation convolution not supported for this shape");
  const int rows = 128 / W_out;
  const int boxH = rows <= H_out ? rows : H_out;
  const int boxN = rows <= H_out ? 1 : rows / H_out;
  const int M = NB * H_out * W_out;
  const int bn = pick_block_n(M, C_out);
  const int kh_all = branches * kh;
  const int cw = pick_tap_pack(C_in);
  CUtensorMap ta = make_tmap_nhwc(x, NB, H, W, C_in, boxN, boxH, W_out, stride, cw);
  CUtensorMap tb = make_tmap_2d(w, C_out, uint64_t(kh_all) * kw * C_in, uint64_t(kh_all) * kw * C_in, bn, cw);
  IgemmParams p{};
  p.M = M; p.N = C_out;
  p.cblocks = (C_in + IG_BLOCK_K - 1) / IG_BLOCK_K;
  p.num_k_blocks = kh_all * kw * p.cblocks;
  p.taps_total = kh_all * kw;
  if (cw != IG_BLOCK_K) {
    p.cw = cw;
    p.num_k_blocks = (kh_all * kw + IG_BLOCK_K / cw - 1) / (IG_BLOCK_K / cw);
  }
  p.taps_w = kw; p.b_cols_per_tap = C_in; p.is_conv = 1;
  p.HW_out = H_out * W_out; p.W_out = W_out;
  p.stride = stride; p.pad = 0; p.dil = 1;
  p.out = y; p.ldo = C_out; p.bias = bias; p.act = act; p.stats = nullptr;
  p.k_splits = 1; p.kb_per_split = p.num_k_blocks;
  p.ms_kh = kh;
  for (int b = 0; b < branches; ++b) {
    if (dils[b] < 1 || dils[b] > 255 || pads[b] < 0 || pads[b] > 255) throw std::runtime_error("fedb200: multi-dilation: dilation / padding out of range");
    p.ms_dil |= (unsigned long long)(dils[b]) << (8 * b);
    p.ms_pad |= (unsigned long long)(pads[b]) << (8 * b);
  }
  dispatch(bn, ta, tb, p, stream);
}

bool conv_wgrad_supported(int C_x, int C_out, int stride, int W_out, int H_out) {
  if ((C_x & 3) || (C_out & 3)) return false;
  if (stride < 1 || stride > 8) return false;
  return W_out > 0 && H_out > 0;
}

template <int BN>
static void launch_wgrad(const float* x, const float* dy, const WgradParams& p, int grid, cudaStream_t stream) {
  constexpr int smem = 2 * (WG_A_BYTES + BN * WG_BK * 4);
  auto kernel = wgrad_wgmma_kernel<BN>;
  static bool configured = false;
  if (!configured) {
    cudaError_t e = cudaFuncSetAttribute(kernel, cudaFuncAttributeMaxDynamicSharedMemorySize, smem);
    if (e != cudaSuccess) throw std::runtime_error(std::string("fedb200: cudaFuncSetAttribute(wgrad): ") + cudaGetErrorString(e));
    configured = true;
  }
  cudaError_t e = launch_pdl(kernel, dim3(grid), dim3(WG_THREADS), size_t(smem), stream, x, dy, p);
  if (e != cudaSuccess) throw std::runtime_error(std::string("fedb200: wgrad launch: ") + cudaGetErrorString(e));
  count_launch();
}

void conv_wgrad_tf32(const float* x, const float* dy, float* dw, int NB, int H, int W, int C_x, int C_w, int C_out, int kh,
                     int kw, int stride, int pad, int dil, int H_out, int W_out, cudaStream_t stream) {
  if (!conv_wgrad_supported(C_x, C_out, stride, W_out, H_out))
    throw std::runtime_error("fedb200: wgrad geometry not supported by the wgmma path");
  WgradParams p{};
  p.H = H; p.W = W; p.Cx = C_x; p.Cw = C_w; p.Co = C_out;
  p.kw = kw; p.stride = stride; p.pad = pad; p.dil = dil; p.H_out = H_out; p.W_out = W_out;
  p.J = kh * kw * C_w;
  p.P = NB * H_out * W_out;
  p.dw = dw;
  const int bn = C_out <= 32 ? 32 : (C_out <= 64 ? 64 : 128);
  p.j_tiles = (p.J + WG_BM - 1) / WG_BM;
  p.co_tiles = (C_out + bn - 1) / bn;
  const int kb_total = (p.P + WG_BK - 1) / WG_BK;
  const int base = p.j_tiles * p.co_tiles;
  int splits = env_int("FEDB200_WGRAD_SPLITS", 0);
  if (splits <= 0) {
    splits = std::max(1, 2 * num_sms() / base);
    splits = std::min(splits, std::max(1, kb_total / 8));
  }
  splits = std::max(1, std::min(splits, kb_total));
  p.kb_per_split = (kb_total + splits - 1) / splits;
  splits = (kb_total + p.kb_per_split - 1) / p.kb_per_split;
  const int grid = base * splits;
  switch (bn) {
    case 32: launch_wgrad<32>(x, dy, p, grid, stream); break;
    case 64: launch_wgrad<64>(x, dy, p, grid, stream); break;
    default: launch_wgrad<128>(x, dy, p, grid, stream); break;
  }
}

}
```

federated_pytorch_test_b200/csrc/igemm_wgmma.cuh:

```cuda
#pragma once
#include "sm90.cuh"
#include "fedb200.h"

namespace fedb200 {

constexpr int IG_BLOCK_M = 128;
constexpr int IG_BLOCK_K = 32;
constexpr int IG_MMA_K = 8;
constexpr int IG_THREADS = 384;

struct IgemmParams {
  int M, N;
  int num_k_blocks;
  int cblocks;
  int taps_w;
  int b_cols_per_tap;
  int is_conv;
  int HW_out, W_out;
  int stride, pad, dil;
  float* out;
  int ldo;
  const float* bias;
  int act;
  float* stats;
  int kb_per_split;
  int k_splits;
  int m_tiles, n_tiles, total_tiles;
  int accumulate;
  int tma_store;
  int cw;
  int taps_total;
  int ms_kh;
  unsigned long long ms_dil, ms_pad;
  int shuffle_ci;
  const float* bn_gamma;
  const float* bn_beta;
  const float* bn_mean;
  const float* bn_var;
  float bn_eps;
  const float* residual;
  int ldr;
  int win_rows;
  int win_a_bytes;
  int win_stage_bytes;
};

template <int BLOCK_N, int STAGES>
struct IgemmSmem {
  static constexpr int A_BYTES = IG_BLOCK_M * IG_BLOCK_K * 4;
  static constexpr int B_BYTES = BLOCK_N * IG_BLOCK_K * 4;
  static constexpr int STAGE_BYTES = A_BYTES + B_BYTES;
  static constexpr int STAGING_BYTES = 2 * 64 * 32 * 4;
  static constexpr int STATS_BYTES = 2 * BLOCK_N * 4;
  static constexpr int BAR_BYTES = 2 * STAGES * 8;
  static constexpr int TOTAL = STAGES * STAGE_BYTES + STAGING_BYTES + STATS_BYTES + BAR_BYTES + 1024;
};

struct TileCoord {
  int m0, n0, kb_begin, kb_count;
};
__device__ __forceinline__ TileCoord decode_tile(const IgemmParams& p, int t, int block_m, int block_n) {
  const int n_idx = t % p.n_tiles;
  const int rest = t / p.n_tiles;
  const int m_idx = rest % p.m_tiles;
  const int z = rest / p.m_tiles;
  TileCoord c;
  c.m0 = m_idx * block_m;
  c.n0 = n_idx * block_n;
  c.kb_begin = z * p.kb_per_split;
  c.kb_count = min(p.kb_per_split, p.num_k_blocks - c.kb_begin);
  return c;
}

__device__ __forceinline__ void named_bar_sync(uint32_t id, uint32_t n) {
  asm volatile("bar.sync %0, %1;" ::"r"(id), "r"(n) : "memory");
}
__device__ __forceinline__ void named_bar_arrive(uint32_t id, uint32_t n) {
  asm volatile("bar.arrive %0, %1;" ::"r"(id), "r"(n) : "memory");
}

template <int TILE_M, int BLOCK_N, int STAGES, int A_BYTES, int STAGE_BYTES>
__device__ __forceinline__ void igemm_produce(const IgemmParams& p, uint8_t* tiles, uint64_t* full_bar, uint64_t* empty_bar,
                                              const CUtensorMap* tmap_a, const CUtensorMap* tmap_b) {
  int s = 0;
  uint32_t ph = 0;
  const int cwp = (p.cw == 8 || p.cw == 16) ? p.cw : 0;
  const int tpk = cwp ? IG_BLOCK_K / cwp : 1;
  const int img_oob = p.is_conv ? p.M / p.HW_out + 1 : 0;
  const int col_oob = p.taps_total * p.b_cols_per_tap + IG_BLOCK_K;
  auto tap_offset = [&](int rr_, int sx_, int& cw_, int& ch_) {
    cw_ = sx_ * p.dil - p.pad;
    ch_ = rr_ * p.dil;
    if (p.ms_kh > 0) {
      const int br = rr_ / p.ms_kh, rr = rr_ - br * p.ms_kh;
      const int d = int((p.ms_dil >> (8 * br)) & 0xffull), pd = int((p.ms_pad >> (8 * br)) & 0xffull);
      cw_ = sx_ * d - pd;
      ch_ = rr * d - pd;
    }
  };
  for (int t = blockIdx.x; t < p.total_tiles; t += gridDim.x) {
    const TileCoord c = decode_tile(p, t, TILE_M, BLOCK_N);
    int img = 0, h0 = 0;
    if (p.is_conv) {
      img = c.m0 / p.HW_out;
      h0 = ((c.m0 - img * p.HW_out) / p.W_out) * p.stride - p.pad;
    }
    int tap = c.kb_begin / p.cblocks;
    int cb = c.kb_begin - tap * p.cblocks;
    int r = tap / p.taps_w, sx = tap - r * p.taps_w;
    for (int kb = c.kb_begin; kb < c.kb_begin + c.kb_count; ++kb) {
      mbar_wait(&empty_bar[s], ph ^ 1);
      uint8_t* a_dst = tiles + s * STAGE_BYTES;
      uint8_t* b_dst = a_dst + A_BYTES;
      mbar_arrive_expect_tx(&full_bar[s], uint32_t(STAGE_BYTES));
      if (cwp) {
        const int sub_a = TILE_M * cwp * 4, sub_b = BLOCK_N * cwp * 4;
        for (int jt = 0; jt < tpk; ++jt) {
          const int tp = kb * tpk + jt;
          const bool real = tp < p.taps_total;
          int cw = 0, ch = 0;
          if (real) tap_offset(tp / p.taps_w, tp % p.taps_w, cw, ch);
          tma_load_4d(a_dst + jt * sub_a, tmap_a, &full_bar[s], 0, cw, h0 + ch, real ? img : img_oob);
          tma_load_2d(b_dst + jt * sub_b, tmap_b, &full_bar[s], real ? tp * p.b_cols_per_tap : col_oob, c.n0);
        }
      } else {
        int cw, ch;
        tap_offset(r, sx, cw, ch);
        if (p.is_conv)
          tma_load_4d(a_dst, tmap_a, &full_bar[s], cb * IG_BLOCK_K, cw, h0 + ch, img);
        else
          tma_load_2d(a_dst, tmap_a, &full_bar[s], kb * IG_BLOCK_K, c.m0);
        tma_load_2d(b_dst, tmap_b, &full_bar[s], (r * p.taps_w + sx) * p.b_cols_per_tap + cb * IG_BLOCK_K, c.n0);
        if (++cb == p.cblocks) {
          cb = 0;
          if (++sx == p.taps_w) { sx = 0; ++r; }
        }
      }
      if (++s == STAGES) { s = 0; ph ^= 1; }
    }
  }
}

template <int BLOCK_N, int STAGES, bool EVAL_BN>
__global__ void __launch_bounds__(IG_THREADS, 1)
igemm_wgmma_kernel(const __grid_constant__ CUtensorMap tmap_a, const __grid_constant__ CUtensorMap tmap_b,
                   const __grid_constant__ CUtensorMap tmap_c, const IgemmParams p) {
  using S = IgemmSmem<BLOCK_N, STAGES>;
  static_assert(BLOCK_N == 32 || BLOCK_N == 64 || BLOCK_N == 128, "BLOCK_N must be 32, 64 or 128");
  static_assert(S::TOTAL <= 227 * 1024, "shared memory budget");
  static_assert(S::STAGE_BYTES % 1024 == 0, "stages must keep the 1024-byte swizzle alignment");
  constexpr int NACC = BLOCK_N / 2;

  extern __shared__ uint8_t smem_raw[];
  uint8_t* smem = reinterpret_cast<uint8_t*>((reinterpret_cast<uintptr_t>(smem_raw) + 1023) & ~uintptr_t(1023));
  uint8_t* tiles = smem;
  float* staging = reinterpret_cast<float*>(smem + STAGES * S::STAGE_BYTES);
  float* colsum = reinterpret_cast<float*>(smem + STAGES * S::STAGE_BYTES + S::STAGING_BYTES);
  uint64_t* full_bar = reinterpret_cast<uint64_t*>(colsum + 2 * BLOCK_N);
  uint64_t* empty_bar = full_bar + STAGES;

  const int wg = threadIdx.x >> 7;
  const int tid = threadIdx.x & 127;

  pdl_launch_dependents();
  if (threadIdx.x == 0) {
    tma_prefetch_desc(&tmap_a);
    tma_prefetch_desc(&tmap_b);
    if (p.tma_store) tma_prefetch_desc(&tmap_c);
    for (int s = 0; s < STAGES; ++s) {
      mbar_init(&full_bar[s], 1);
      mbar_init(&empty_bar[s], 2);
    }
    fence_barrier_init();
  }
  for (int i = threadIdx.x; i < 2 * BLOCK_N; i += IG_THREADS) colsum[i] = 0.f;
  __syncthreads();
  pdl_wait();

  if (wg == 0) {
    if (threadIdx.x == 0)
      igemm_produce<IG_BLOCK_M, BLOCK_N, STAGES, S::A_BYTES, S::STAGE_BYTES>(p, tiles, full_bar, empty_bar, &tmap_a, &tmap_b);
    return;
  }

  const int g = wg - 1;
  const int warp = tid >> 5, lane = tid & 31;
  const uint32_t cwq = (p.cw == 8 || p.cw == 16) ? uint32_t(p.cw) : uint32_t(IG_BLOCK_K);
  const uint32_t mma_per_sub = cwq / IG_MMA_K;
  const uint64_t adesc0 = make_kmajor_desc(smem_u32(tiles) + uint32_t(g) * 64u * cwq * 4u, cwq * 4u);
  const uint64_t bdesc0 = make_kmajor_desc(smem_u32(tiles) + uint32_t(S::A_BYTES), cwq * 4u);
  uint32_t a_off[IG_BLOCK_K / IG_MMA_K], b_off[IG_BLOCK_K / IG_MMA_K];
#pragma unroll
  for (int k = 0; k < IG_BLOCK_K / IG_MMA_K; ++k) {
    const uint32_t sub = uint32_t(k) / mma_per_sub, in = uint32_t(k) - sub * mma_per_sub;
    a_off[k] = (sub * uint32_t(IG_BLOCK_M) * cwq * 4u + in * 32u) >> 4;
    b_off[k] = (sub * uint32_t(BLOCK_N) * cwq * 4u + in * 32u) >> 4;
  }
  float* stg = staging + g * 2048;
  const uint32_t wg_bar = 1 + uint32_t(g);
  const int row_in = 16 * warp + (lane >> 2);
  const int col_in = 2 * (lane & 3);

  float acc[NACC];
#pragma unroll
  for (int i = 0; i < NACC; ++i) acc[i] = 0.f;
  int s = 0;
  uint32_t ph = 0;
  for (int t = blockIdx.x; t < p.total_tiles; t += gridDim.x) {
    const TileCoord c = decode_tile(p, t, IG_BLOCK_M, BLOCK_N);
    if constexpr (EVAL_BN) {
      named_bar_sync(3, 256);
      for (int cc = threadIdx.x - 128; cc < BLOCK_N; cc += 256) {
        const int col = c.n0 + cc;
        float sc = 0.f, sh = 0.f;
        if (col < p.N) {
          sc = __ldg(p.bn_gamma + col) * rsqrtf(__ldg(p.bn_var + col) + p.bn_eps);
          sh = fmaf(-__ldg(p.bn_mean + col), sc, __ldg(p.bn_beta + col));
        }
        colsum[cc] = sc;
        colsum[BLOCK_N + cc] = sh;
      }
      named_bar_sync(3, 256);
    }
    int prev = -1;
    for (int i = 0; i < c.kb_count; ++i) {
      mbar_wait(&full_bar[s], ph);
      const uint64_t so = uint64_t(uint32_t(s) * uint32_t(S::STAGE_BYTES >> 4));
      wgmma_fence();
      wgmma_fence_acc(acc);
#pragma unroll
      for (int k = 0; k < IG_BLOCK_K / IG_MMA_K; ++k)
        wgmma_tf32<BLOCK_N>(acc, adesc0 + so + a_off[k], bdesc0 + so + b_off[k], (i > 0 || k > 0) ? 1u : 0u);
      wgmma_commit();
      wgmma_fence_acc(acc);
      wgmma_wait<1>();
      if (prev >= 0 && tid == 0) mbar_arrive(&empty_bar[prev]);
      prev = s;
      if (++s == STAGES) { s = 0; ph ^= 1; }
    }
    wgmma_wait<0>();
    wgmma_fence_acc(acc);
    if (prev >= 0 && tid == 0) mbar_arrive(&empty_bar[prev]);

    const int row_a = c.m0 + 64 * g + row_in, row_b = row_a + 8;
    const bool ok_a = row_a < p.M, ok_b = row_b < p.M;
#pragma unroll
    for (int i = 0; i < NACC / 4; ++i) {
      float2 ra = make_float2(0.f, 0.f), rb = ra;
      if constexpr (EVAL_BN) {
        if (p.residual != nullptr && c.n0 + 8 * i + col_in < p.N) {
          const float* r0 = p.residual + c.n0 + 8 * i + col_in;
          if (ok_a) ra = __ldg(reinterpret_cast<const float2*>(r0 + size_t(row_a) * p.ldr));
          if (ok_b) rb = __ldg(reinterpret_cast<const float2*>(r0 + size_t(row_b) * p.ldr));
        }
      }
#pragma unroll
      for (int e = 0; e < 2; ++e) {
        const int col = c.n0 + 8 * i + col_in + e;
        float va = acc[4 * i + e], vb = acc[4 * i + 2 + e];
        if (p.bias != nullptr && col < p.N) {
          const float b = __ldg(p.bias + col);
          va += b;
          vb += b;
        }
        if constexpr (EVAL_BN) {
          const float sc = colsum[8 * i + col_in + e], sh = colsum[BLOCK_N + 8 * i + col_in + e];
          va = fmaf(va, sc, sh) + (e ? ra.y : ra.x);
          vb = fmaf(vb, sc, sh) + (e ? rb.y : rb.x);
        }
        if (p.act) { va = elu1(va); vb = elu1(vb); }
        acc[4 * i + e] = ok_a ? va : 0.f;
        acc[4 * i + 2 + e] = ok_b ? vb : 0.f;
      }
    }
    if (p.stats != nullptr) {
#pragma unroll
      for (int i = 0; i < NACC / 4; ++i) {
#pragma unroll
        for (int e = 0; e < 2; ++e) {
          const float va = acc[4 * i + e], vb = acc[4 * i + 2 + e];
          float s1 = va + vb, s2 = fmaf(va, va, vb * vb);
#pragma unroll
          for (int o = 4; o < 32; o <<= 1) {
            s1 += __shfl_xor_sync(0xffffffffu, s1, o);
            s2 += __shfl_xor_sync(0xffffffffu, s2, o);
          }
          if (lane < 4) {
            atomicAdd(&colsum[8 * i + col_in + e], s1);
            atomicAdd(&colsum[BLOCK_N + 8 * i + col_in + e], s2);
          }
        }
      }
    }
    if (p.tma_store) {
#pragma unroll
      for (int c0 = 0; c0 < BLOCK_N; c0 += 32) {
        if (tid == 0) tma_store_wait_read();
        named_bar_sync(wg_bar, 128);
#pragma unroll
        for (int ii = 0; ii < 4; ++ii) {
          const int i = c0 / 8 + ii;
          const int cc = 8 * ii + col_in;
#pragma unroll
          for (int h = 0; h < 2; ++h) {
            const int r = row_in + 8 * h;
            const int rr = r & 31;
            float* dst = stg + (r >> 5) * 1024 + rr * 32 + (((uint32_t(cc) >> 2) ^ uint32_t(rr & 7)) << 2) + (cc & 3);
            *reinterpret_cast<float2*>(dst) = make_float2(acc[4 * i + 2 * h], acc[4 * i + 2 * h + 1]);
          }
        }
        fence_proxy_async();
        named_bar_sync(wg_bar, 128);
        if (tid == 0) {
          const int pc = c.n0 + c0;
          for (int b = 0; b < 2; ++b) {
            const int row0 = c.m0 + 64 * g + 32 * b;
            if (row0 >= p.M || pc >= p.N) continue;
            const float* src = stg + b * 1024;
            if (p.shuffle_ci > 0) {
              const int phase = pc / p.shuffle_ci;
              if (p.k_splits > 1) tma_reduce_add_5d(&tmap_c, src, pc - phase * p.shuffle_ci, phase & 1, 0, phase >> 1, row0 / p.W_out);
              else tma_store_5d(&tmap_c, src, pc - phase * p.shuffle_ci, phase & 1, 0, phase >> 1, row0 / p.W_out);
            } else if (p.k_splits > 1 || p.accumulate) {
              tma_reduce_add_2d(&tmap_c, src, pc, row0);
            } else {
              tma_store_2d(&tmap_c, src, pc, row0);
            }
          }
          tma_store_commit();
        }
      }
    } else {
#pragma unroll
      for (int i = 0; i < NACC / 4; ++i) {
#pragma unroll
        for (int h = 0; h < 2; ++h) {
          const int row = h ? row_b : row_a;
          if (!(h ? ok_b : ok_a)) continue;
#pragma unroll
          for (int e = 0; e < 2; ++e) {
            const int col = c.n0 + 8 * i + col_in + e;
            if (col >= p.N) continue;
            float* dst = p.out + size_t(row) * p.ldo + col;
            if (p.k_splits > 1 || p.accumulate) atomicAdd(dst, acc[4 * i + 2 * h + e]);
            else *dst = acc[4 * i + 2 * h + e];
          }
        }
      }
    }
    if (p.stats != nullptr) {
      named_bar_sync(3, 256);
      for (int cc = threadIdx.x - 128; cc < BLOCK_N; cc += 256) {
        if (c.n0 + cc < p.N) {
          atomicAdd(p.stats + c.n0 + cc, colsum[cc]);
          atomicAdd(p.stats + p.N + c.n0 + cc, colsum[BLOCK_N + cc]);
        }
        colsum[cc] = 0.f;
        colsum[BLOCK_N + cc] = 0.f;
      }
      named_bar_sync(3, 256);
    }
  }
  if (p.tma_store && tid == 0) tma_store_wait_read();
}

constexpr int PX_BLOCK_M = 256;

template <int CO, int STAGES>
struct PixSmem {
  static constexpr int A_BYTES = PX_BLOCK_M * IG_BLOCK_K * 4;
  static constexpr int B_BYTES = CO * IG_BLOCK_K * 4;
  static constexpr int STAGE_BYTES = A_BYTES + B_BYTES;
  static constexpr int STAGING_BYTES = 2 * 2 * 2 * 32 * 32 * 4;
  static constexpr int BAR_BYTES = 2 * STAGES * 8;
  static constexpr int TOTAL = STAGES * STAGE_BYTES + STAGING_BYTES + BAR_BYTES + 1024;
  static constexpr int window_total(int stage_bytes) { return STAGES * stage_bytes + STAGING_BYTES + BAR_BYTES + 1024; }
};

template <int CO, int STAGES, int KH>
__device__ __forceinline__ void igemm_produce_window(const IgemmParams& p, uint8_t* tiles, uint64_t* full_bar, uint64_t* empty_bar,
                                                     const CUtensorMap* tmap_a, const CUtensorMap* tmap_b) {
  constexpr uint32_t W_BOX = CO * IG_BLOCK_K * 4;
  const uint32_t stage_bytes = uint32_t(p.win_stage_bytes);
  int s = 0;
  uint32_t ph = 0;
  for (int t = blockIdx.x; t < p.total_tiles; t += gridDim.x) {
    const TileCoord c = decode_tile(p, t, PX_BLOCK_M, CO);
    const int img = c.m0 / p.HW_out;
    const int h0 = (c.m0 - img * p.HW_out) / p.W_out - p.pad;
    for (int sx = 0; sx < p.taps_w; ++sx) {
      for (int cb = 0; cb < p.cblocks; ++cb) {
        mbar_wait(&empty_bar[s], ph ^ 1);
        uint8_t* a_dst = tiles + s * stage_bytes;
        uint8_t* b_dst = a_dst + p.win_a_bytes;
        mbar_arrive_expect_tx(&full_bar[s], stage_bytes);
        tma_load_4d(a_dst, tmap_a, &full_bar[s], cb * IG_BLOCK_K, sx - p.pad, h0, img);
#pragma unroll
        for (int r = 0; r < KH; ++r)
          tma_load_2d(b_dst + r * W_BOX, tmap_b, &full_bar[s], (r * p.taps_w + sx) * p.b_cols_per_tap + cb * IG_BLOCK_K, 0);
        if (++s == STAGES) { s = 0; ph ^= 1; }
      }
    }
  }
}

template <int CO, int STAGES, int WIN_KH>
__global__ void __launch_bounds__(IG_THREADS, 1)
igemm_wgmma_pix_kernel(const __grid_constant__ CUtensorMap tmap_a, const __grid_constant__ CUtensorMap tmap_b,
                 const __grid_constant__ CUtensorMap tmap_c, const IgemmParams p) {
  using S = PixSmem<CO, STAGES>;
  constexpr bool WINDOW = WIN_KH > 0;
  static_assert(CO == 64 || CO == 128, "pixel-major tiles serve 64 or 128 output channels");
  static_assert(WINDOW || S::TOTAL <= 227 * 1024, "shared memory budget");
  static_assert(S::STAGE_BYTES % 1024 == 0, "stages must keep the 1024-byte swizzle alignment");
  constexpr bool PINGPONG = CO == 64;
  const uint32_t stage_bytes = WINDOW ? uint32_t(p.win_stage_bytes) : uint32_t(S::STAGE_BYTES);

  extern __shared__ uint8_t smem_raw[];
  uint8_t* smem = reinterpret_cast<uint8_t*>((reinterpret_cast<uintptr_t>(smem_raw) + 1023) & ~uintptr_t(1023));
  uint8_t* tiles = smem;
  float* staging = reinterpret_cast<float*>(smem + STAGES * stage_bytes);
  uint64_t* full_bar = reinterpret_cast<uint64_t*>(smem + STAGES * stage_bytes + S::STAGING_BYTES);
  uint64_t* empty_bar = full_bar + STAGES;

  const int wg = threadIdx.x >> 7;
  const int tid = threadIdx.x & 127;

  pdl_launch_dependents();
  if (threadIdx.x == 0) {
    tma_prefetch_desc(&tmap_a);
    tma_prefetch_desc(&tmap_b);
    tma_prefetch_desc(&tmap_c);
    for (int s = 0; s < STAGES; ++s) {
      mbar_init(&full_bar[s], 1);
      mbar_init(&empty_bar[s], PINGPONG ? 1 : 2);
    }
    fence_barrier_init();
  }
  __syncthreads();
  pdl_wait();

  if (wg == 0) {
    setmaxnreg_dec<40>();
    if (threadIdx.x == 0) {
      if constexpr (WINDOW) igemm_produce_window<CO, STAGES, WIN_KH>(p, tiles, full_bar, empty_bar, &tmap_a, &tmap_b);
      else igemm_produce<PX_BLOCK_M, CO, STAGES, S::A_BYTES, S::STAGE_BYTES>(p, tiles, full_bar, empty_bar, &tmap_a, &tmap_b);
    }
    return;
  }
  setmaxnreg_inc<232>();

  const int g = wg - 1;
  const int warp = tid >> 5, lane = tid & 31;
  const int ch_wg = PINGPONG ? 0 : 64 * g;
  const uint32_t cwq = (p.cw == 8 || p.cw == 16) ? uint32_t(p.cw) : uint32_t(IG_BLOCK_K);
  const uint32_t mma_per_sub = cwq / IG_MMA_K;
  const uint32_t a_bytes = WINDOW ? uint32_t(p.win_a_bytes) : uint32_t(S::A_BYTES);
  const uint64_t adesc0 = make_kmajor_desc(smem_u32(tiles) + a_bytes + uint32_t(ch_wg) * cwq * 4u, cwq * 4u);
  const uint64_t bdesc0 = make_kmajor_desc(smem_u32(tiles), cwq * 4u);
  uint32_t a_off[IG_BLOCK_K / IG_MMA_K], b_off[IG_BLOCK_K / IG_MMA_K];
#pragma unroll
  for (int k = 0; k < IG_BLOCK_K / IG_MMA_K; ++k) {
    const uint32_t sub = uint32_t(k) / mma_per_sub, in = uint32_t(k) - sub * mma_per_sub;
    a_off[k] = (sub * uint32_t(CO) * cwq * 4u + in * 32u) >> 4;
    b_off[k] = (sub * uint32_t(PX_BLOCK_M) * cwq * 4u + in * 32u) >> 4;
  }
  float* stg = staging + g * 4096;
  const uint32_t wg_bar = 1 + uint32_t(g);
  const int ch_lo = 16 * warp + (lane >> 2);
  const int px_in = 2 * (lane & 3);

  float acc[128];
  const int step = PINGPONG ? 2 : 1;
  for (int j = PINGPONG ? g : 0, t = blockIdx.x + j * gridDim.x; t < p.total_tiles; j += step, t += step * gridDim.x) {
    const TileCoord c = decode_tile(p, t, PX_BLOCK_M, CO);
    const uint32_t pos = uint32_t(j) * uint32_t(c.kb_count);
    int s = int(pos % STAGES);
    uint32_t ph = (pos / STAGES) & 1u;
    if (PINGPONG && j > 0) named_bar_sync(3 + uint32_t(g), 256);
    int prev = -1;
    for (int i = 0; i < c.kb_count; ++i) {
      mbar_wait(&full_bar[s], ph);
      const uint64_t so = uint64_t(uint32_t(s) * (stage_bytes >> 4));
      wgmma_fence();
      wgmma_fence_acc(acc);
      if constexpr (WINDOW) {
        const uint32_t px_row = uint32_t(p.W_out) * 8u;
#pragma unroll
        for (int r = 0; r < WIN_KH; ++r) {
          const uint64_t ao = so + uint32_t(r) * uint32_t(CO * 8), bo = so + uint32_t(r) * px_row;
#pragma unroll
          for (int k = 0; k < IG_BLOCK_K / IG_MMA_K; ++k)
            wgmma_tf32_n256(acc, adesc0 + ao + a_off[k], bdesc0 + bo + b_off[k], (i > 0 || r > 0 || k > 0) ? 1u : 0u);
        }
      } else {
#pragma unroll
        for (int k = 0; k < IG_BLOCK_K / IG_MMA_K; ++k)
          wgmma_tf32_n256(acc, adesc0 + so + a_off[k], bdesc0 + so + b_off[k], (i > 0 || k > 0) ? 1u : 0u);
      }
      wgmma_commit();
      wgmma_fence_acc(acc);
      wgmma_wait<1>();
      if (prev >= 0 && tid == 0) mbar_arrive(&empty_bar[prev]);
      prev = s;
      if (++s == STAGES) { s = 0; ph ^= 1; }
    }
    if (PINGPONG && t + gridDim.x < p.total_tiles) named_bar_arrive(4 - uint32_t(g), 256);
    wgmma_wait<0>();
    wgmma_fence_acc(acc);
    if (prev >= 0 && tid == 0) mbar_arrive(&empty_bar[prev]);

    if (c.m0 + PX_BLOCK_M > p.M) {
#pragma unroll
      for (int i = 0; i < 32; ++i)
#pragma unroll
        for (int e = 0; e < 2; ++e)
          if (c.m0 + 8 * i + px_in + e >= p.M) { acc[4 * i + e] = 0.f; acc[4 * i + 2 + e] = 0.f; }
    }
    if (p.stats != nullptr) {
      float s1a = 0.f, s2a = 0.f, s1b = 0.f, s2b = 0.f;
#pragma unroll
      for (int i = 0; i < 32; ++i) {
#pragma unroll
        for (int e = 0; e < 2; ++e) {
          const float va = acc[4 * i + e], vb = acc[4 * i + 2 + e];
          s1a += va; s2a = fmaf(va, va, s2a);
          s1b += vb; s2b = fmaf(vb, vb, s2b);
        }
      }
#pragma unroll
      for (int o = 1; o < 4; o <<= 1) {
        s1a += __shfl_xor_sync(0xffffffffu, s1a, o);
        s2a += __shfl_xor_sync(0xffffffffu, s2a, o);
        s1b += __shfl_xor_sync(0xffffffffu, s1b, o);
        s2b += __shfl_xor_sync(0xffffffffu, s2b, o);
      }
      if ((lane & 3) == 0) {
        const int ca = ch_wg + ch_lo;
        atomicAdd(p.stats + ca, s1a);
        atomicAdd(p.stats + p.N + ca, s2a);
        atomicAdd(p.stats + ca + 8, s1b);
        atomicAdd(p.stats + p.N + ca + 8, s2b);
      }
    }
#pragma unroll
    for (int q = 0; q < PX_BLOCK_M / 32; ++q) {
      float* buf = stg + (q & 1) * 2048;
      if (tid == 0) tma_store_wait_read_n<1>();
      named_bar_sync(wg_bar, 128);
#pragma unroll
      for (int ii = 0; ii < 4; ++ii) {
        const int i = 4 * q + ii;
#pragma unroll
        for (int h = 0; h < 2; ++h) {
          const int ch = ch_lo + 8 * h;
          const int cc = ch & 31;
#pragma unroll
          for (int e = 0; e < 2; ++e) {
            const int px = 8 * ii + px_in + e;
            buf[(ch >> 5) * 1024 + px * 32 + (((uint32_t(cc) >> 2) ^ uint32_t(px & 7)) << 2) + (cc & 3)] = acc[4 * i + 2 * h + e];
          }
        }
      }
      fence_proxy_async();
      named_bar_sync(wg_bar, 128);
      if (tid == 0) {
        const int row0 = c.m0 + 32 * q;
        if (row0 < p.M) {
#pragma unroll
          for (int b = 0; b < 2; ++b) {
            if (p.accumulate) tma_reduce_add_2d(&tmap_c, buf + b * 1024, ch_wg + 32 * b, row0);
            else tma_store_2d(&tmap_c, buf + b * 1024, ch_wg + 32 * b, row0);
          }
        }
        tma_store_commit();
      }
    }
  }
  if (tid == 0) tma_store_wait_read();
}

}
```

federated_pytorch_test_b200/csrc/sm90.cuh:

```cuda
#pragma once
#include <cuda.h>
#include <cuda_runtime.h>
#include <stdint.h>

namespace fedb200 {

__device__ __forceinline__ uint32_t smem_u32(const void* p) {
  return static_cast<uint32_t>(__cvta_generic_to_shared(p));
}

__device__ __forceinline__ void mbar_init(uint64_t* bar, uint32_t count) {
  asm volatile("mbarrier.init.shared::cta.b64 [%0], %1;" ::"r"(smem_u32(bar)), "r"(count) : "memory");
}
__device__ __forceinline__ void fence_barrier_init() {
  asm volatile("fence.mbarrier_init.release.cluster;" ::: "memory");
}
__device__ __forceinline__ void fence_proxy_async() {
  asm volatile("fence.proxy.async.shared::cta;" ::: "memory");
}
__device__ __forceinline__ void mbar_arrive_expect_tx(uint64_t* bar, uint32_t bytes) {
  asm volatile("mbarrier.arrive.expect_tx.shared::cta.b64 _, [%0], %1;" ::"r"(smem_u32(bar)), "r"(bytes) : "memory");
}
__device__ __forceinline__ void mbar_arrive(uint64_t* bar) {
  asm volatile("mbarrier.arrive.shared::cta.b64 _, [%0];" ::"r"(smem_u32(bar)) : "memory");
}
__device__ __forceinline__ bool mbar_try_wait(uint64_t* bar, uint32_t parity) {
  uint32_t done;
  asm volatile(
      "{\n\t.reg .pred p;\n\t"
      "mbarrier.try_wait.parity.shared::cta.b64 p, [%1], %2;\n\t"
      "selp.u32 %0, 1, 0, p;\n\t}\n"
      : "=r"(done)
      : "r"(smem_u32(bar)), "r"(parity)
      : "memory");
  return done != 0;
}
__device__ __forceinline__ void mbar_wait(uint64_t* bar, uint32_t parity) {
  asm volatile(
      "{\n\t.reg .pred P1;\n\t.reg .b32 T;\n\t"
      "mov.u32 T, 0;\n\t"
      "MBW_%=:\n\t"
      "mbarrier.try_wait.parity.shared::cta.b64 P1, [%0], %1;\n\t"
      "@P1 bra MBD_%=;\n\t"
      "add.u32 T, T, 1;\n\t"
      "setp.lt.u32 P1, T, 0x1000000;\n\t"
      "@P1 bra MBW_%=;\n\t"
      "trap;\n\t"
      "MBD_%=:\n\t}\n"
      :
      : "r"(smem_u32(bar)), "r"(parity)
      : "memory");
}

__device__ __forceinline__ void tma_prefetch_desc(const CUtensorMap* m) {
  asm volatile("prefetch.tensormap [%0];" ::"l"(reinterpret_cast<uint64_t>(m)) : "memory");
}
__device__ __forceinline__ void tma_load_2d(void* dst, const CUtensorMap* m, uint64_t* bar, int c0, int c1) {
  asm volatile(
      "cp.async.bulk.tensor.2d.shared::cluster.global.mbarrier::complete_tx::bytes [%0], [%1, {%3, %4}], [%2];"
      ::"r"(smem_u32(dst)), "l"(reinterpret_cast<uint64_t>(m)), "r"(smem_u32(bar)), "r"(c0), "r"(c1)
      : "memory");
}
__device__ __forceinline__ void tma_load_4d(void* dst, const CUtensorMap* m, uint64_t* bar, int c0, int c1, int c2,
                                            int c3) {
  asm volatile(
      "cp.async.bulk.tensor.4d.shared::cluster.global.mbarrier::complete_tx::bytes [%0], [%1, {%3, %4, %5, %6}], [%2];"
      ::"r"(smem_u32(dst)), "l"(reinterpret_cast<uint64_t>(m)), "r"(smem_u32(bar)), "r"(c0), "r"(c1), "r"(c2), "r"(c3)
      : "memory");
}

__device__ __forceinline__ void tma_store_2d(const CUtensorMap* m, const void* src, int c0, int c1) {
  asm volatile("cp.async.bulk.tensor.2d.global.shared::cta.bulk_group [%0, {%2, %3}], [%1];"
               ::"l"(reinterpret_cast<uint64_t>(m)), "r"(smem_u32(src)), "r"(c0), "r"(c1) : "memory");
}
__device__ __forceinline__ void tma_reduce_add_2d(const CUtensorMap* m, const void* src, int c0, int c1) {
  asm volatile("cp.reduce.async.bulk.tensor.2d.global.shared::cta.add.tile.bulk_group [%0, {%2, %3}], [%1];"
               ::"l"(reinterpret_cast<uint64_t>(m)), "r"(smem_u32(src)), "r"(c0), "r"(c1) : "memory");
}
__device__ __forceinline__ void tma_store_5d(const CUtensorMap* m, const void* src, int c0, int c1, int c2, int c3, int c4) {
  asm volatile("cp.async.bulk.tensor.5d.global.shared::cta.bulk_group [%0, {%2, %3, %4, %5, %6}], [%1];"
               ::"l"(reinterpret_cast<uint64_t>(m)), "r"(smem_u32(src)), "r"(c0), "r"(c1), "r"(c2), "r"(c3), "r"(c4) : "memory");
}
__device__ __forceinline__ void tma_reduce_add_5d(const CUtensorMap* m, const void* src, int c0, int c1, int c2, int c3, int c4) {
  asm volatile("cp.reduce.async.bulk.tensor.5d.global.shared::cta.add.tile.bulk_group [%0, {%2, %3, %4, %5, %6}], [%1];"
               ::"l"(reinterpret_cast<uint64_t>(m)), "r"(smem_u32(src)), "r"(c0), "r"(c1), "r"(c2), "r"(c3), "r"(c4) : "memory");
}
__device__ __forceinline__ void tma_store_commit() { asm volatile("cp.async.bulk.commit_group;" ::: "memory"); }
__device__ __forceinline__ void tma_store_wait_read() { asm volatile("cp.async.bulk.wait_group.read 0;" ::: "memory"); }
template <int N>
__device__ __forceinline__ void tma_store_wait_read_n() { asm volatile("cp.async.bulk.wait_group.read %0;" ::"n"(N) : "memory"); }

__device__ __forceinline__ void wgmma_fence() { asm volatile("wgmma.fence.sync.aligned;" ::: "memory"); }
__device__ __forceinline__ void wgmma_commit() { asm volatile("wgmma.commit_group.sync.aligned;" ::: "memory"); }
template <int N>
__device__ __forceinline__ void wgmma_wait() { asm volatile("wgmma.wait_group.sync.aligned %0;" ::"n"(N) : "memory"); }
template <int R>
__device__ __forceinline__ void wgmma_fence_acc(float (&d)[R]) {
#pragma unroll
  for (int i = 0; i < R; ++i) asm volatile("" : "+f"(d[i])::"memory");
}

__device__ __forceinline__ uint64_t make_kmajor_desc(uint32_t smem_addr, uint32_t sw) {
  uint64_t d = 0;
  d |= static_cast<uint64_t>((smem_addr >> 4) & 0x3FFF);
  d |= static_cast<uint64_t>(1) << 16;
  d |= static_cast<uint64_t>((8u * sw) >> 4) << 32;
  d |= static_cast<uint64_t>(sw == 128u ? 1u : (sw == 64u ? 2u : 3u)) << 62;
  return d;
}
__device__ __forceinline__ uint64_t make_kmajor_interleave_desc(uint32_t smem_addr, uint32_t lbo, uint32_t sbo) {
  uint64_t d = 0;
  d |= static_cast<uint64_t>((smem_addr >> 4) & 0x3FFF);
  d |= static_cast<uint64_t>((lbo >> 4) & 0x3FFF) << 16;
  d |= static_cast<uint64_t>((sbo >> 4) & 0x3FFF) << 32;
  return d;
}

__device__ __forceinline__ void wgmma_tf32_n32(float (&d)[16], uint64_t adesc, uint64_t bdesc, uint32_t accumulate) {
  asm volatile(
      "{\n\t.reg .pred p;\n\t"
      "setp.ne.b32 p, %18, 0;\n\t"
      "wgmma.mma_async.sync.aligned.m64n32k8.f32.tf32.tf32 "
      "{"
      "%0, %1, %2, %3, %4, %5, %6, %7, %8, %9, %10, %11, %12, %13, %14, %15"
      "}, %16, %17, p, 1, 1;\n\t}\n"
      : "+f"(d[0]), "+f"(d[1]), "+f"(d[2]), "+f"(d[3]), "+f"(d[4]), "+f"(d[5]), "+f"(d[6]), "+f"(d[7]),
        "+f"(d[8]), "+f"(d[9]), "+f"(d[10]), "+f"(d[11]), "+f"(d[12]), "+f"(d[13]), "+f"(d[14]), "+f"(d[15])
      : "l"(adesc), "l"(bdesc), "r"(accumulate));
}
__device__ __forceinline__ void wgmma_tf32_n64(float (&d)[32], uint64_t adesc, uint64_t bdesc, uint32_t accumulate) {
  asm volatile(
      "{\n\t.reg .pred p;\n\t"
      "setp.ne.b32 p, %34, 0;\n\t"
      "wgmma.mma_async.sync.aligned.m64n64k8.f32.tf32.tf32 "
      "{"
      "%0, %1, %2, %3, %4, %5, %6, %7, %8, %9, %10, %11, %12, %13, %14, %15, "
      "%16, %17, %18, %19, %20, %21, %22, %23, %24, %25, %26, %27, %28, %29, %30, %31"
      "}, %32, %33, p, 1, 1;\n\t}\n"
      : "+f"(d[0]), "+f"(d[1]), "+f"(d[2]), "+f"(d[3]), "+f"(d[4]), "+f"(d[5]), "+f"(d[6]), "+f"(d[7]),
        "+f"(d[8]), "+f"(d[9]), "+f"(d[10]), "+f"(d[11]), "+f"(d[12]), "+f"(d[13]), "+f"(d[14]), "+f"(d[15]),
        "+f"(d[16]), "+f"(d[17]), "+f"(d[18]), "+f"(d[19]), "+f"(d[20]), "+f"(d[21]), "+f"(d[22]), "+f"(d[23]),
        "+f"(d[24]), "+f"(d[25]), "+f"(d[26]), "+f"(d[27]), "+f"(d[28]), "+f"(d[29]), "+f"(d[30]), "+f"(d[31])
      : "l"(adesc), "l"(bdesc), "r"(accumulate));
}
__device__ __forceinline__ void wgmma_tf32_n128(float (&d)[64], uint64_t adesc, uint64_t bdesc, uint32_t accumulate) {
  asm volatile(
      "{\n\t.reg .pred p;\n\t"
      "setp.ne.b32 p, %66, 0;\n\t"
      "wgmma.mma_async.sync.aligned.m64n128k8.f32.tf32.tf32 "
      "{"
      "%0, %1, %2, %3, %4, %5, %6, %7, %8, %9, %10, %11, %12, %13, %14, %15, "
      "%16, %17, %18, %19, %20, %21, %22, %23, %24, %25, %26, %27, %28, %29, %30, %31, "
      "%32, %33, %34, %35, %36, %37, %38, %39, %40, %41, %42, %43, %44, %45, %46, %47, "
      "%48, %49, %50, %51, %52, %53, %54, %55, %56, %57, %58, %59, %60, %61, %62, %63"
      "}, %64, %65, p, 1, 1;\n\t}\n"
      : "+f"(d[0]), "+f"(d[1]), "+f"(d[2]), "+f"(d[3]), "+f"(d[4]), "+f"(d[5]), "+f"(d[6]), "+f"(d[7]),
        "+f"(d[8]), "+f"(d[9]), "+f"(d[10]), "+f"(d[11]), "+f"(d[12]), "+f"(d[13]), "+f"(d[14]), "+f"(d[15]),
        "+f"(d[16]), "+f"(d[17]), "+f"(d[18]), "+f"(d[19]), "+f"(d[20]), "+f"(d[21]), "+f"(d[22]), "+f"(d[23]),
        "+f"(d[24]), "+f"(d[25]), "+f"(d[26]), "+f"(d[27]), "+f"(d[28]), "+f"(d[29]), "+f"(d[30]), "+f"(d[31]),
        "+f"(d[32]), "+f"(d[33]), "+f"(d[34]), "+f"(d[35]), "+f"(d[36]), "+f"(d[37]), "+f"(d[38]), "+f"(d[39]),
        "+f"(d[40]), "+f"(d[41]), "+f"(d[42]), "+f"(d[43]), "+f"(d[44]), "+f"(d[45]), "+f"(d[46]), "+f"(d[47]),
        "+f"(d[48]), "+f"(d[49]), "+f"(d[50]), "+f"(d[51]), "+f"(d[52]), "+f"(d[53]), "+f"(d[54]), "+f"(d[55]),
        "+f"(d[56]), "+f"(d[57]), "+f"(d[58]), "+f"(d[59]), "+f"(d[60]), "+f"(d[61]), "+f"(d[62]), "+f"(d[63])
      : "l"(adesc), "l"(bdesc), "r"(accumulate));
}

__device__ __forceinline__ void wgmma_tf32_n256(float (&d)[128], uint64_t adesc, uint64_t bdesc, uint32_t accumulate) {
  asm volatile(
      "{\n\t.reg .pred p;\n\t"
      "setp.ne.b32 p, %130, 0;\n\t"
      "wgmma.mma_async.sync.aligned.m64n256k8.f32.tf32.tf32 "
      "{"
      "%0, %1, %2, %3, %4, %5, %6, %7, %8, %9, %10, %11, %12, %13, %14, %15, "
      "%16, %17, %18, %19, %20, %21, %22, %23, %24, %25, %26, %27, %28, %29, %30, %31, "
      "%32, %33, %34, %35, %36, %37, %38, %39, %40, %41, %42, %43, %44, %45, %46, %47, "
      "%48, %49, %50, %51, %52, %53, %54, %55, %56, %57, %58, %59, %60, %61, %62, %63, "
      "%64, %65, %66, %67, %68, %69, %70, %71, %72, %73, %74, %75, %76, %77, %78, %79, "
      "%80, %81, %82, %83, %84, %85, %86, %87, %88, %89, %90, %91, %92, %93, %94, %95, "
      "%96, %97, %98, %99, %100, %101, %102, %103, %104, %105, %106, %107, %108, %109, %110, %111, "
      "%112, %113, %114, %115, %116, %117, %118, %119, %120, %121, %122, %123, %124, %125, %126, %127"
      "}, %128, %129, p, 1, 1;\n\t}\n"
      : "+f"(d[0]), "+f"(d[1]), "+f"(d[2]), "+f"(d[3]), "+f"(d[4]), "+f"(d[5]), "+f"(d[6]), "+f"(d[7]),
        "+f"(d[8]), "+f"(d[9]), "+f"(d[10]), "+f"(d[11]), "+f"(d[12]), "+f"(d[13]), "+f"(d[14]), "+f"(d[15]),
        "+f"(d[16]), "+f"(d[17]), "+f"(d[18]), "+f"(d[19]), "+f"(d[20]), "+f"(d[21]), "+f"(d[22]), "+f"(d[23]),
        "+f"(d[24]), "+f"(d[25]), "+f"(d[26]), "+f"(d[27]), "+f"(d[28]), "+f"(d[29]), "+f"(d[30]), "+f"(d[31]),
        "+f"(d[32]), "+f"(d[33]), "+f"(d[34]), "+f"(d[35]), "+f"(d[36]), "+f"(d[37]), "+f"(d[38]), "+f"(d[39]),
        "+f"(d[40]), "+f"(d[41]), "+f"(d[42]), "+f"(d[43]), "+f"(d[44]), "+f"(d[45]), "+f"(d[46]), "+f"(d[47]),
        "+f"(d[48]), "+f"(d[49]), "+f"(d[50]), "+f"(d[51]), "+f"(d[52]), "+f"(d[53]), "+f"(d[54]), "+f"(d[55]),
        "+f"(d[56]), "+f"(d[57]), "+f"(d[58]), "+f"(d[59]), "+f"(d[60]), "+f"(d[61]), "+f"(d[62]), "+f"(d[63]),
        "+f"(d[64]), "+f"(d[65]), "+f"(d[66]), "+f"(d[67]), "+f"(d[68]), "+f"(d[69]), "+f"(d[70]), "+f"(d[71]),
        "+f"(d[72]), "+f"(d[73]), "+f"(d[74]), "+f"(d[75]), "+f"(d[76]), "+f"(d[77]), "+f"(d[78]), "+f"(d[79]),
        "+f"(d[80]), "+f"(d[81]), "+f"(d[82]), "+f"(d[83]), "+f"(d[84]), "+f"(d[85]), "+f"(d[86]), "+f"(d[87]),
        "+f"(d[88]), "+f"(d[89]), "+f"(d[90]), "+f"(d[91]), "+f"(d[92]), "+f"(d[93]), "+f"(d[94]), "+f"(d[95]),
        "+f"(d[96]), "+f"(d[97]), "+f"(d[98]), "+f"(d[99]), "+f"(d[100]), "+f"(d[101]), "+f"(d[102]), "+f"(d[103]),
        "+f"(d[104]), "+f"(d[105]), "+f"(d[106]), "+f"(d[107]), "+f"(d[108]), "+f"(d[109]), "+f"(d[110]), "+f"(d[111]),
        "+f"(d[112]), "+f"(d[113]), "+f"(d[114]), "+f"(d[115]), "+f"(d[116]), "+f"(d[117]), "+f"(d[118]), "+f"(d[119]),
        "+f"(d[120]), "+f"(d[121]), "+f"(d[122]), "+f"(d[123]), "+f"(d[124]), "+f"(d[125]), "+f"(d[126]), "+f"(d[127])
      : "l"(adesc), "l"(bdesc), "r"(accumulate));
}

template <int N>
__device__ __forceinline__ void wgmma_tf32(float (&d)[N / 2], uint64_t adesc, uint64_t bdesc, uint32_t accumulate) {
  if constexpr (N == 32) wgmma_tf32_n32(d, adesc, bdesc, accumulate);
  else if constexpr (N == 64) wgmma_tf32_n64(d, adesc, bdesc, accumulate);
  else wgmma_tf32_n128(d, adesc, bdesc, accumulate);
}


template <int N>
__device__ __forceinline__ void setmaxnreg_dec() { asm volatile("setmaxnreg.dec.sync.aligned.u32 %0;" ::"n"(N)); }
template <int N>
__device__ __forceinline__ void setmaxnreg_inc() { asm volatile("setmaxnreg.inc.sync.aligned.u32 %0;" ::"n"(N)); }

__device__ __forceinline__ float elu1(float v) { return v > 0.f ? v : (__expf(v) - 1.f); }

__device__ __forceinline__ float warp_sum(float v) {
#pragma unroll
  for (int o = 16; o > 0; o >>= 1) v += __shfl_xor_sync(0xffffffffu, v, o);
  return v;
}

}
```

federated_pytorch_test_b200/ops/conv_math.py:

```python
from __future__ import annotations

from typing import Callable

import torch
import torch.nn.functional as F

_TAP3 = {(0, 0): 1, (1, 0): 2, (1, 1): 0}


def _tap_index_table(k: int) -> torch.Tensor:
    zero = k * k
    idx = torch.full((2, 2, 2, 2), zero, dtype=torch.long)
    for ph in (0, 1):
        for pw in (0, 1):
            for dr in (0, 1):
                for ds in (0, 1):
                    if k == 3:
                        r, s = _TAP3.get((ph, dr)), _TAP3.get((pw, ds))
                    else:
                        r = 0 if (ph == 0 and dr == 0) else None
                        s = 0 if (pw == 0 and ds == 0) else None
                    if r is not None and s is not None:
                        idx[ph, pw, dr, ds] = r * k + s
    return idx


def pack_dgrad_s2_weight(w_krsc: torch.Tensor) -> torch.Tensor:
    Co, kh, kw, Ci = w_krsc.shape
    assert kh == kw and kh in (1, 3), "stride-2 phase decomposition implemented for 1x1/pad0 and 3x3/pad1"
    flat = w_krsc.reshape(Co, kh * kw, Ci)
    zero = w_krsc.new_zeros(Co, Ci)
    idx = _tap_index_table(kh).reshape(-1).tolist()
    sel = torch.stack([flat[:, i] if i < kh * kw else zero for i in idx], dim=1).reshape(Co, 2, 2, 2, 2, Ci)
    return sel.permute(1, 2, 5, 3, 4, 0).reshape(4 * Ci, 2, 2, Co).contiguous()


def dgrad_s2(dy_nhwc: torch.Tensor, w_packed: torch.Tensor, conv2x2: Callable[[torch.Tensor, torch.Tensor], torch.Tensor]
             ) -> torch.Tensor:
    N, Ho, Wo, _ = dy_nhwc.shape
    Ci = w_packed.shape[0] // 4
    y = conv2x2(dy_nhwc, w_packed)
    return y.view(N, Ho, Wo, 2, 2, Ci).permute(0, 1, 3, 2, 4, 5).reshape(N, 2 * Ho, 2 * Wo, Ci)


def conv2x2_oracle(x_nhwc: torch.Tensor, w_krsc: torch.Tensor) -> torch.Tensor:
    x = F.pad(x_nhwc.permute(0, 3, 1, 2), (0, 1, 0, 1))
    return F.conv2d(x, w_krsc.permute(0, 3, 1, 2)).permute(0, 2, 3, 1).contiguous()


_TAP4 = {(0, 0): 3, (0, 1): 1, (1, 1): 2, (1, 2): 0}


def pack_convT_s2_weight(w_iokk: torch.Tensor) -> torch.Tensor:
    Ci, Co, kh, kw = w_iokk.shape
    assert kh == 4 and kw == 4, "phase decomposition implemented for ConvTranspose2d(k=4, stride=2, padding=1)"
    zero = w_iokk.new_zeros(Co, Ci)
    taps = []
    for ph in (0, 1):
        for pw in (0, 1):
            for tr in (0, 1, 2):
                for ts in (0, 1, 2):
                    r, s_ = _TAP4.get((ph, tr)), _TAP4.get((pw, ts))
                    taps.append(w_iokk[:, :, r, s_].t() if (r is not None and s_ is not None) else zero)
    sel = torch.stack(taps, dim=0).reshape(2, 2, 3, 3, Co, Ci)
    return sel.permute(0, 1, 4, 2, 3, 5).reshape(4 * Co, 3, 3, Ci).contiguous()


def convT_s2(x_nhwc: torch.Tensor, w_packed: torch.Tensor, conv3x3: Callable[[torch.Tensor, torch.Tensor], torch.Tensor]
             ) -> torch.Tensor:
    N, H, W, _ = x_nhwc.shape
    Co = w_packed.shape[0] // 4
    y = conv3x3(x_nhwc, w_packed)
    return y.view(N, H, W, 2, 2, Co).permute(0, 1, 3, 2, 4, 5).reshape(N, 2 * H, 2 * W, Co)


def conv3x3_oracle(x_nhwc: torch.Tensor, w_krsc: torch.Tensor) -> torch.Tensor:
    return F.conv2d(x_nhwc.permute(0, 3, 1, 2), w_krsc.permute(0, 3, 1, 2), None, 1, 1).permute(0, 2, 3, 1).contiguous()


def pack_multidil_weight(ws_oikk) -> torch.Tensor:
    B = len(ws_oikk)
    Co, Ci, k, _ = ws_oikk[0].shape
    w_all = torch.stack([w.permute(0, 2, 3, 1) for w in ws_oikk])
    wm = w_all.new_zeros(B, Co, B, k, k, Ci)
    wm.diagonal(dim1=0, dim2=2).copy_(w_all.permute(1, 2, 3, 4, 0))
    return wm.view(B * Co, B * k, k, Ci)


def multidil_conv_oracle(x_nhwc: torch.Tensor, wm: torch.Tensor, k: int, stride: int, dils, pads) -> torch.Tensor:
    N, H, W, Ci = x_nhwc.shape
    B = len(dils)
    Ho = (H + 2 * pads[0] - dils[0] * (k - 1) - 1) // stride + 1
    Wo = (W + 2 * pads[0] - dils[0] * (k - 1) - 1) // stride + 1
    big = max(max(pads), max(d * (k - 1) for d in dils))
    xp = F.pad(x_nhwc, (0, 0, big, big + stride, big, big + stride))
    y = x_nhwc.new_zeros(N, Ho, Wo, wm.shape[0])
    for R in range(B * k):
        b, r = divmod(R, k)
        d, p = dils[b], pads[b]
        for s in range(k):
            h0, w0 = big + r * d - p, big + s * d - p
            tap = xp[:, h0: h0 + (Ho - 1) * stride + 1: stride, w0: w0 + (Wo - 1) * stride + 1: stride, :]
            y = y + tap @ wm[:, R, s, :].t()
    return y


def tap_packed_gemm_oracle(x_nhwc: torch.Tensor, w_krsc: torch.Tensor, stride: int, pad: int, cw: int) -> torch.Tensor:
    N, H, W, Ci = x_nhwc.shape
    Co, kh, kw, _ = w_krsc.shape
    assert Ci <= cw and 32 % cw == 0
    tpk = 32 // cw
    Ho, Wo = (H + 2 * pad - kh) // stride + 1, (W + 2 * pad - kw) // stride + 1
    xp = F.pad(x_nhwc, (0, 0, pad, pad, pad, pad))
    wmat = w_krsc.reshape(Co, kh * kw * Ci)
    wmat = F.pad(wmat, (0, 32))
    taps = kh * kw
    y = x_nhwc.new_zeros(N * Ho * Wo, Co)
    for kb in range(-(-taps // tpk)):
        a = x_nhwc.new_zeros(N * Ho * Wo, 32)
        bmat = x_nhwc.new_zeros(Co, 32)
        for j in range(tpk):
            t = kb * tpk + j
            if t < taps:
                r, s = divmod(t, kw)
                tap = xp[:, r: r + (Ho - 1) * stride + 1: stride, s: s + (Wo - 1) * stride + 1: stride, :]
                a[:, j * cw: j * cw + Ci] = tap.reshape(-1, Ci)
                bmat[:, j * cw: (j + 1) * cw] = wmat[:, t * Ci: t * Ci + cw]
        y = y + a @ bmat.t()
    return y.view(N, Ho, Wo, Co)


def shuffle_store_oracle(y_packed: torch.Tensor) -> torch.Tensor:
    N, Ho, Wo, C4 = y_packed.shape
    Ci = C4 // 4
    assert Ci % 32 == 0 and 32 % Wo == 0, "a chunk must stay inside one phase and cover whole output rows"
    out = y_packed.new_zeros(N, 2 * Ho, 2 * Wo, Ci)
    view5 = out.view(N * Ho, 2, Wo, 2, Ci)
    rows = y_packed.reshape(N * Ho * Wo, C4)
    for row0 in range(0, rows.shape[0], 32):
        for pc in range(0, C4, 32):
            phase, ci0 = divmod(pc, Ci)
            ph, pw = phase >> 1, phase & 1
            hon0 = row0 // Wo
            nrow = min(32, rows.shape[0] - row0)
            chunk = rows[row0: row0 + nrow, pc: pc + 32].reshape(nrow // Wo, Wo, 32)
            view5[hon0: hon0 + nrow // Wo, ph, :, pw, ci0: ci0 + 32] = chunk
    return out


def window_reuse_conv_oracle(x_nhwc: torch.Tensor, w_krsc: torch.Tensor, pad: int, rows: int) -> torch.Tensor:
    N, H, W, Ci = x_nhwc.shape
    Co, kh, kw, _ = w_krsc.shape
    Ho, Wo = H + 2 * pad - kh + 1, W + 2 * pad - kw + 1
    assert Ho % rows == 0, "a tile is whole output rows of one image"
    win_rows = rows + kh - 1
    y = x_nhwc.new_zeros(N, Ho, Wo, Co)
    for n in range(N):
        for h0 in range(0, Ho, rows):
            acc = x_nhwc.new_zeros(rows * Wo, Co)
            for s in range(kw):
                for c0 in range(0, Ci, 32):
                    c1 = min(c0 + 32, Ci)
                    window = x_nhwc.new_zeros(win_rows, Wo, c1 - c0)
                    for i in range(win_rows):
                        hi = h0 - pad + i
                        if not 0 <= hi < H:
                            continue
                        w_lo, w_hi = max(0, s - pad), min(W, s - pad + Wo)
                        if w_lo < w_hi:
                            window[i, w_lo - (s - pad): w_hi - (s - pad)] = x_nhwc[n, hi, w_lo:w_hi, c0:c1]
                    for r in range(kh):
                        acc = acc + window[r: r + rows].reshape(rows * Wo, c1 - c0) @ w_krsc[:, r, s, c0:c1].t()
            y[n, h0: h0 + rows] = acc.view(rows, Wo, Co)
    return y
```

Measured before the change: 35160.

## Add 2x2 thread-block-cluster implicit-GEMM conv with TMA multicast of A/B tiles

Adds a clustered variant of the wgmma implicit-GEMM conv kernel. Four CTAs form a 2x2 cluster, and each CTA loads half of the A and B tiles and multicasts them to its peers, with empty barriers released across the cluster. The aim is to cut global/L2 operand traffic per tile. The variant is gated behind FEDB200_CLUSTER=4, which defaults off. Separately, the per-CTA column statistics now use per-warp smem partial sums in place of shared atomics, which also affects the default path and costs extra shared memory.

Result: faster. 36430 (median of 6 runs) (+3.6%).

```diff
diff --git a/federated_pytorch_test_b200/csrc/bindings.cpp b/federated_pytorch_test_b200/csrc/bindings.cpp
--- a/federated_pytorch_test_b200/csrc/bindings.cpp
+++ b/federated_pytorch_test_b200/csrc/bindings.cpp
@@ -247,6 +247,9 @@
 }
 bool conv_window_reuse(int64_t H_out, int64_t W_out, int64_t C_in, int64_t C_out, int64_t kh, int64_t stride, int64_t dil) {
   return fb::conv_window_reuse((int)H_out, (int)W_out, (int)C_in, (int)C_out, (int)kh, (int)stride, (int)dil);
+}
+bool conv_cluster(int64_t NB, int64_t H_out, int64_t W_out, int64_t C_in, int64_t C_out, int64_t kh, int64_t kw, int64_t stride) {
+  return fb::conv_cluster_launch((int)NB, (int)H_out, (int)W_out, (int)C_in, (int)C_out, (int)kh, (int)kw, (int)stride);
 }
 Tensor conv2d_nhwc(Tensor x, Tensor w, c10::optional<Tensor> stats, int64_t stride, int64_t pad, int64_t dil, int64_t orient) {
   CHECK_F32_CUDA(x); CHECK_F32_CUDA(w); CHECK_CONTIG(x); CHECK_CONTIG(w);
@@ -835,6 +838,8 @@
   m.def("conv_orientation", &conv_orientation);
   m.def("conv_window_reuse", &conv_window_reuse, py::arg("H_out"), py::arg("W_out"), py::arg("C_in"), py::arg("C_out"), py::arg("kh"),
         py::arg("stride") = 1, py::arg("dil") = 1);
+  m.def("conv_cluster", &conv_cluster, py::arg("NB"), py::arg("H_out"), py::arg("W_out"), py::arg("C_in"), py::arg("C_out"),
+        py::arg("kh") = 3, py::arg("kw") = 3, py::arg("stride") = 1);
   m.def("conv2d_nhwc", &conv2d_nhwc, py::arg("x"), py::arg("w"), py::arg("stats"), py::arg("stride"), py::arg("pad"), py::arg("dil"),
         py::arg("orient") = -1);
   m.def("conv2d_nhwc_sized", &conv2d_nhwc_sized);
diff --git a/federated_pytorch_test_b200/csrc/fedb200.h b/federated_pytorch_test_b200/csrc/fedb200.h
--- a/federated_pytorch_test_b200/csrc/fedb200.h
+++ b/federated_pytorch_test_b200/csrc/fedb200.h
@@ -39,6 +39,7 @@
 enum { CONV_ORIENT_AUTO = -1, CONV_ORIENT_ROW = 0, CONV_ORIENT_PIXEL = 1, CONV_ORIENT_PIXEL_PERTAP = 2 };
 int pick_conv_orientation(int NB, int H_out, int W_out, int C_out, int stride);
 bool conv_window_reuse(int H_out, int W_out, int C_in, int C_out, int kh, int stride, int dil);
+bool conv_cluster_launch(int NB, int H_out, int W_out, int C_in, int C_out, int kh, int kw, int stride);
 void conv2d_nhwc_tf32(const float* x, const float* w, float* y, float* stats, int NB, int H, int W, int C_in, int C_out,
                       int kh, int kw, int stride, int pad, int dil, int H_out, int W_out, cudaStream_t stream,
                       int orient = CONV_ORIENT_AUTO);
diff --git a/federated_pytorch_test_b200/csrc/gemm_wgmma.cu b/federated_pytorch_test_b200/csrc/gemm_wgmma.cu
--- a/federated_pytorch_test_b200/csrc/gemm_wgmma.cu
+++ b/federated_pytorch_test_b200/csrc/gemm_wgmma.cu
@@ -97,22 +97,33 @@
 
 static const CUtensorMap* g_out_map_override = nullptr;
 
-template <int BN, int ST, bool EVAL_BN>
-static void launch(const CUtensorMap& ta, const CUtensorMap& tb, IgemmParams p, cudaStream_t stream) {
+template <int BN, int ST, bool EVAL_BN, bool CLUSTER>
+static auto igemm_kernel() {
   using S = IgemmSmem<BN, ST>;
-  auto kernel = igemm_wgmma_kernel<BN, ST, EVAL_BN>;
+  auto kernel = igemm_wgmma_kernel<BN, ST, EVAL_BN, CLUSTER>;
   static bool configured = false;
   if (!configured) {
     cudaError_t e = cudaFuncSetAttribute(kernel, cudaFuncAttributeMaxDynamicSharedMemorySize, S::TOTAL);
     if (e != cudaSuccess) throw std::runtime_error(std::string("fedb200: cudaFuncSetAttribute(igemm): ") + cudaGetErrorString(e));
     configured = true;
   }
+  return kernel;
+}
+
+static CUtensorMap igemm_out_map(IgemmParams& p, const CUtensorMap& ta) {
+  p.tma_store = ((p.ldo & 3) == 0 && (reinterpret_cast<uintptr_t>(p.out) & 15) == 0 && env_int("FEDB200_TMA_STORE", 1) != 0) ? 1 : 0;
+  if (g_out_map_override != nullptr) p.tma_store = 1;
+  return g_out_map_override != nullptr ? *g_out_map_override : (p.tma_store ? make_tmap_out(p.out, p.M, p.N, p.ldo, 32) : ta);
+}
+
+template <int BN, int ST, bool EVAL_BN>
+static void launch(const CUtensorMap& ta, const CUtensorMap& tb, IgemmParams p, cudaStream_t stream) {
+  using S = IgemmSmem<BN, ST>;
+  auto kernel = igemm_kernel<BN, ST, EVAL_BN, false>();
   p.m_tiles = (p.M + IG_BLOCK_M - 1) / IG_BLOCK_M;
   p.n_tiles = (p.N + BN - 1) / BN;
   p.total_tiles = p.m_tiles * p.n_tiles * p.k_splits;
-  p.tma_store = ((p.ldo & 3) == 0 && (reinterpret_cast<uintptr_t>(p.out) & 15) == 0 && env_int("FEDB200_TMA_STORE", 1) != 0) ? 1 : 0;
-  if (g_out_map_override != nullptr) p.tma_store = 1;
-  const CUtensorMap tc = g_out_map_override != nullptr ? *g_out_map_override : (p.tma_store ? make_tmap_out(p.out, p.M, p.N, p.ldo, 32) : ta);
+  const CUtensorMap tc = igemm_out_map(p, ta);
   const int sms = num_sms();
   const int grid = (p.total_tiles < sms || env_int("FEDB200_PERSIST", 1) == 0) ? p.total_tiles : sms;
   cudaError_t e = launch_pdl(kernel, dim3(grid), dim3(IG_THREADS), S::TOTAL, stream, ta, tb, tc, p);
@@ -120,17 +131,70 @@
   count_launch();
 }
 
+constexpr int CL_BN = 128, CL_ST = 6, CL_SIZE = 4;
+
+static cudaLaunchConfig_t cluster_config(int grid, cudaLaunchAttribute (&attr)[2], cudaStream_t stream) {
+  cudaLaunchConfig_t cfg{};
+  cfg.gridDim = dim3(grid);
+  cfg.blockDim = dim3(IG_THREADS);
+  cfg.dynamicSmemBytes = IgemmSmem<CL_BN, CL_ST>::TOTAL;
+  cfg.stream = stream;
+  attr[0].id = cudaLaunchAttributeClusterDimension;
+  attr[0].val.clusterDim.x = CL_SIZE;
+  attr[0].val.clusterDim.y = 1;
+  attr[0].val.clusterDim.z = 1;
+  attr[1].id = cudaLaunchAttributeProgrammaticStreamSerialization;
+  attr[1].val.programmaticStreamSerializationAllowed = pdl_enabled() ? 1 : 0;
+  cfg.attrs = attr;
+  cfg.numAttrs = 2;
+  return cfg;
+}
+
 template <bool EVAL_BN>
-static void dispatch_tile(int bn, const CUtensorMap& ta, const CUtensorMap& tb, const IgemmParams& p, cudaStream_t s) {
+static void launch_cluster(const CUtensorMap& ta, const CUtensorMap& tb, IgemmParams p, cudaStream_t stream) {
+  auto kernel = igemm_kernel<CL_BN, CL_ST, EVAL_BN, true>();
+  p.m_tiles = (p.M + IG_BLOCK_M - 1) / IG_BLOCK_M;
+  p.n_tiles = (p.N + CL_BN - 1) / CL_BN;
+  p.total_tiles = CL_SIZE * ((p.m_tiles + 1) / 2) * (p.n_tiles / 2) * p.k_splits;
+  const CUtensorMap tc = igemm_out_map(p, ta);
+  cudaLaunchAttribute attr[2];
+  const cudaLaunchConfig_t cfg = cluster_config(p.total_tiles, attr, stream);
+  cudaError_t e = cudaLaunchKernelEx(&cfg, kernel, ta, tb, tc, p);
+  if (e != cudaSuccess) throw std::runtime_error(std::string("fedb200: igemm cluster launch: ") + cudaGetErrorString(e));
+  count_launch();
+}
+
+static bool pick_cluster(int N, int bn, int cw, int boxN, int boxH) {
+  if (env_int("FEDB200_CLUSTER", 0) != 4 || bn != CL_BN || cw != IG_BLOCK_K) return false;
+  const int n_tiles = (N + bn - 1) / bn;
+  return n_tiles % 2 == 0 && (boxN % 2 == 0 || (boxN == 1 && boxH % 2 == 0));
+}
+
+static void cluster_half_box(int boxN, int boxH, int stride, IgemmParams& p, int& half_n, int& half_h) {
+  if (boxN >= 2) {
+    half_n = boxN / 2; half_h = boxH;
+    p.cl_img_step = half_n; p.cl_h_step = 0;
+  } else {
+    half_n = 1; half_h = boxH / 2;
+    p.cl_img_step = 0; p.cl_h_step = half_h * stride;
+  }
+}
+
+template <bool EVAL_BN>
+static void dispatch_tile(int bn, const CUtensorMap& ta, const CUtensorMap& tb, const IgemmParams& p, cudaStream_t s, bool cluster) {
+  if (cluster) {
+    launch_cluster<EVAL_BN>(ta, tb, p, s);
+    return;
+  }
   switch (bn) {
     case 32: launch<32, 8, EVAL_BN>(ta, tb, p, s); break;
     case 64: launch<64, 8, EVAL_BN>(ta, tb, p, s); break;
     default: launch<128, 6, EVAL_BN>(ta, tb, p, s); break;
   }
 }
-static void dispatch(int bn, const CUtensorMap& ta, const CUtensorMap& tb, const IgemmParams& p, cudaStream_t s) {
-  if (p.bn_gamma != nullptr) dispatch_tile<true>(bn, ta, tb, p, s);
-  else dispatch_tile<false>(bn, ta, tb, p, s);
+static void dispatch(int bn, const CUtensorMap& ta, const CUtensorMap& tb, const IgemmParams& p, cudaStream_t s, bool cluster = false) {
+  if (p.bn_gamma != nullptr) dispatch_tile<true>(bn, ta, tb, p, s, cluster);
+  else dispatch_tile<false>(bn, ta, tb, p, s, cluster);
 }
 
 constexpr int PIX_STAGES = 4;
@@ -302,8 +366,9 @@
   const int M = NB * H_out * W_out;
   const int bn = pix ? C_out : pick_block_n(M, C_out);
   const int cw = pick_tap_pack(C_in);
+  const uint64_t K = uint64_t(kh) * kw * C_in;
   CUtensorMap ta = make_tmap_nhwc(x, NB, H, W, C_in, boxN, win_stage ? boxH + kh - 1 : boxH, W_out, stride, cw);
-  CUtensorMap tb = make_tmap_2d(w, C_out, uint64_t(kh) * kw * C_in, uint64_t(kh) * kw * C_in, bn, cw);
+  CUtensorMap tb = make_tmap_2d(w, C_out, K, K, bn, cw);
   IgemmParams p{};
   p.M = M; p.N = C_out;
   p.cblocks = (C_in + IG_BLOCK_K - 1) / IG_BLOCK_K;
@@ -351,11 +416,27 @@
       p.bn_eps = eval_bn->eps; p.residual = eval_bn->residual; p.ldr = C_out;
     }
   }
-  dispatch(bn, ta, tb, p, stream);
+  const bool cluster = pick_cluster(C_out, bn, cw, boxN, boxH);
+  if (cluster) {
+    int half_n, half_h;
+    cluster_half_box(boxN, boxH, stride, p, half_n, half_h);
+    ta = make_tmap_nhwc(x, NB, H, W, C_in, half_n, half_h, W_out, stride, cw);
+    tb = make_tmap_2d(w, C_out, K, K, bn / 2, cw);
+  }
+  dispatch(bn, ta, tb, p, stream, cluster);
   if (p.k_splits > 1 && stats != nullptr) col_stats(y, stats, M, C_out, stream);
   if (p.k_splits > 1 && eval_bn != nullptr)
     bn_elu_fwd(y, nullptr, eval_bn->gamma, eval_bn->beta, eval_bn->residual, y, const_cast<float*>(eval_bn->mean),
                const_cast<float*>(eval_bn->var), nullptr, nullptr, M, C_out, eval_bn->eps, 0.f, act, 0, stream, 1);
+}
+
+bool conv_cluster_launch(int NB, int H_out, int W_out, int C_in, int C_out, int kh, int kw, int stride) {
+  (void)kh; (void)kw;
+  if (!conv_geometry_supported(H_out, W_out, C_in, stride)) return false;
+  const int rows = IG_BLOCK_M / W_out;
+  const int boxH = rows <= H_out ? rows : H_out;
+  const int boxN = rows <= H_out ? 1 : rows / H_out;
+  return pick_cluster(C_out, pick_block_n(NB * H_out * W_out, C_out), pick_tap_pack(C_in), boxN, boxH);
 }
 
 bool conv_shuffle_supported(int H_out, int W_out, int C_in, int Ci_out) {
@@ -405,9 +486,16 @@
       cudaMemsetAsync(out, 0, size_t(M) * C4 * sizeof(float), stream);
     }
   }
+  const bool cluster = pick_cluster(C4, bn, IG_BLOCK_K, boxN, boxH);
+  if (cluster) {
+    int half_n, half_h;
+    cluster_half_box(boxN, boxH, 1, p, half_n, half_h);
+    ta = make_tmap_nhwc(x, NB, H, W, C_in, half_n, half_h, W_out, 1);
+    tb = make_tmap_2d(w, C4, uint64_t(kh) * kw * C_in, uint64_t(kh) * kw * C_in, bn / 2);
+  }
   g_out_map_override = &tc;
   try {
-    dispatch(bn, ta, tb, p, stream);
+    dispatch(bn, ta, tb, p, stream, cluster);
   } catch (...) {
     g_out_map_override = nullptr;
     throw;
diff --git a/federated_pytorch_test_b200/csrc/igemm_wgmma.cuh b/federated_pytorch_test_b200/csrc/igemm_wgmma.cuh
--- a/federated_pytorch_test_b200/csrc/igemm_wgmma.cuh
+++ b/federated_pytorch_test_b200/csrc/igemm_wgmma.cuh
@@ -43,6 +43,7 @@
   int win_rows;
   int win_a_bytes;
   int win_stage_bytes;
+  int cl_img_step, cl_h_step;
 };
 
 template <int BLOCK_N, int STAGES>
@@ -52,8 +53,9 @@
   static constexpr int STAGE_BYTES = A_BYTES + B_BYTES;
   static constexpr int STAGING_BYTES = 2 * 64 * 32 * 4;
   static constexpr int STATS_BYTES = 2 * BLOCK_N * 4;
+  static constexpr int WSUM_BYTES = 8 * 2 * BLOCK_N * 4;
   static constexpr int BAR_BYTES = 2 * STAGES * 8;
-  static constexpr int TOTAL = STAGES * STAGE_BYTES + STAGING_BYTES + STATS_BYTES + BAR_BYTES + 1024;
+  static constexpr int TOTAL = STAGES * STAGE_BYTES + STAGING_BYTES + STATS_BYTES + WSUM_BYTES + BAR_BYTES + 1024;
 };
 
 struct TileCoord {
@@ -67,6 +69,20 @@
   TileCoord c;
   c.m0 = m_idx * block_m;
   c.n0 = n_idx * block_n;
+  c.kb_begin = z * p.kb_per_split;
+  c.kb_count = min(p.kb_per_split, p.num_k_blocks - c.kb_begin);
+  return c;
+}
+
+__device__ __forceinline__ TileCoord decode_cluster_tile(const IgemmParams& p, int q, uint32_t rank, int block_m, int block_n) {
+  const int n_pairs = p.n_tiles / 2, m_pairs = (p.m_tiles + 1) / 2;
+  const int np = q % n_pairs;
+  const int rest = q / n_pairs;
+  const int mp = rest % m_pairs;
+  const int z = rest / m_pairs;
+  TileCoord c;
+  c.m0 = (2 * mp + int(rank & 1u)) * block_m;
+  c.n0 = (2 * np + int(rank >> 1)) * block_n;
   c.kb_begin = z * p.kb_per_split;
   c.kb_count = min(p.kb_per_split, p.num_k_blocks - c.kb_begin);
   return c;
@@ -141,12 +157,46 @@
   }
 }
 
-template <int BLOCK_N, int STAGES, bool EVAL_BN>
+template <int BLOCK_N, int STAGES, int A_BYTES, int STAGE_BYTES>
+__device__ __forceinline__ void igemm_produce_cluster(const IgemmParams& p, const TileCoord& c, uint32_t rank, uint8_t* tiles,
+                                                      uint64_t* full_bar, uint64_t* empty_bar, const CUtensorMap* tmap_a,
+                                                      const CUtensorMap* tmap_b) {
+  constexpr int B_HALF_ROWS = BLOCK_N / 2;
+  const int ha = int(rank >> 1), hb = int(rank & 1u);
+  const uint16_t mask_a = uint16_t((1u << rank) | (1u << (rank ^ 2u)));
+  const uint16_t mask_b = uint16_t((1u << rank) | (1u << (rank ^ 1u)));
+  const int img0 = c.m0 / p.HW_out;
+  const int img = img0 + ha * p.cl_img_step;
+  const int h0 = ((c.m0 - img0 * p.HW_out) / p.W_out) * p.stride - p.pad + ha * p.cl_h_step;
+  int s = 0;
+  uint32_t ph = 0;
+  int tap = c.kb_begin / p.cblocks;
+  int cb = c.kb_begin - tap * p.cblocks;
+  int r = tap / p.taps_w, sx = tap - r * p.taps_w;
+  for (int kb = 0; kb < c.kb_count; ++kb) {
+    mbar_wait(&empty_bar[s], ph ^ 1);
+    uint8_t* a_dst = tiles + s * STAGE_BYTES;
+    uint8_t* b_dst = a_dst + A_BYTES;
+    mbar_arrive_expect_tx(&full_bar[s], uint32_t(STAGE_BYTES));
+    tma_load_4d_mc(a_dst + ha * (A_BYTES / 2), tmap_a, &full_bar[s], cb * IG_BLOCK_K, sx * p.dil - p.pad, h0 + r * p.dil, img,
+                   mask_a);
+    tma_load_2d_mc(b_dst + hb * (B_HALF_ROWS * IG_BLOCK_K * 4), tmap_b, &full_bar[s],
+                   (r * p.taps_w + sx) * p.b_cols_per_tap + cb * IG_BLOCK_K, c.n0 + hb * B_HALF_ROWS, mask_b);
+    if (++cb == p.cblocks) {
+      cb = 0;
+      if (++sx == p.taps_w) { sx = 0; ++r; }
+    }
+    if (++s == STAGES) { s = 0; ph ^= 1; }
+  }
+}
+
+template <int BLOCK_N, int STAGES, bool EVAL_BN, bool CLUSTER>
 __global__ void __launch_bounds__(IG_THREADS, 1)
 igemm_wgmma_kernel(const __grid_constant__ CUtensorMap tmap_a, const __grid_constant__ CUtensorMap tmap_b,
                    const __grid_constant__ CUtensorMap tmap_c, const IgemmParams p) {
   using S = IgemmSmem<BLOCK_N, STAGES>;
   static_assert(BLOCK_N == 32 || BLOCK_N == 64 || BLOCK_N == 128, "BLOCK_N must be 32, 64 or 128");
+  static_assert(!CLUSTER || BLOCK_N == 128, "the cluster launch serves 128-column tiles");
   static_assert(S::TOTAL <= 227 * 1024, "shared memory budget");
   static_assert(S::STAGE_BYTES % 1024 == 0, "stages must keep the 1024-byte swizzle alignment");
   constexpr int NACC = BLOCK_N / 2;
@@ -156,11 +206,13 @@
   uint8_t* tiles = smem;
   float* staging = reinterpret_cast<float*>(smem + STAGES * S::STAGE_BYTES);
   float* colsum = reinterpret_cast<float*>(smem + STAGES * S::STAGE_BYTES + S::STAGING_BYTES);
-  uint64_t* full_bar = reinterpret_cast<uint64_t*>(colsum + 2 * BLOCK_N);
+  float* wsum = colsum + 2 * BLOCK_N;
+  uint64_t* full_bar = reinterpret_cast<uint64_t*>(wsum + 16 * BLOCK_N);
   uint64_t* empty_bar = full_bar + STAGES;
 
   const int wg = threadIdx.x >> 7;
   const int tid = threadIdx.x & 127;
+  const uint32_t rank = CLUSTER ? cluster_ctarank() : 0u;
 
   pdl_launch_dependents();
   if (threadIdx.x == 0) {
@@ -169,17 +221,25 @@
     if (p.tma_store) tma_prefetch_desc(&tmap_c);
     for (int s = 0; s < STAGES; ++s) {
       mbar_init(&full_bar[s], 1);
-      mbar_init(&empty_bar[s], 2);
+      mbar_init(&empty_bar[s], CLUSTER ? 6 : 2);
     }
     fence_barrier_init();
   }
-  for (int i = threadIdx.x; i < 2 * BLOCK_N; i += IG_THREADS) colsum[i] = 0.f;
-  __syncthreads();
+  if constexpr (CLUSTER) cluster_sync();
+  else __syncthreads();
   pdl_wait();
 
   if (wg == 0) {
-    if (threadIdx.x == 0)
+    if constexpr (CLUSTER) {
+      if (threadIdx.x == 0)
+        igemm_produce_cluster<BLOCK_N, STAGES, S::A_BYTES, S::STAGE_BYTES>(
+            p, decode_cluster_tile(p, blockIdx.x >> 2, rank, IG_BLOCK_M, BLOCK_N), rank, tiles, full_bar, empty_bar, &tmap_a,
+            &tmap_b);
+      __syncwarp();
+      cluster_sync();
+    } else if (threadIdx.x == 0) {
       igemm_produce<IG_BLOCK_M, BLOCK_N, STAGES, S::A_BYTES, S::STAGE_BYTES>(p, tiles, full_bar, empty_bar, &tmap_a, &tmap_b);
+    }
     return;
   }
 
@@ -201,13 +261,21 @@
   const int row_in = 16 * warp + (lane >> 2);
   const int col_in = 2 * (lane & 3);
 
+  auto release = [&](int st) {
+    if constexpr (CLUSTER) {
+      if (tid < 3) mbar_arrive_cluster(&empty_bar[st], rank ^ uint32_t(tid));
+    } else {
+      if (tid == 0) mbar_arrive(&empty_bar[st]);
+    }
+  };
+
   float acc[NACC];
 #pragma unroll
   for (int i = 0; i < NACC; ++i) acc[i] = 0.f;
   int s = 0;
   uint32_t ph = 0;
   for (int t = blockIdx.x; t < p.total_tiles; t += gridDim.x) {
-    const TileCoord c = decode_tile(p, t, IG_BLOCK_M, BLOCK_N);
+    const TileCoord c = CLUSTER ? decode_cluster_tile(p, t >> 2, rank, IG_BLOCK_M, BLOCK_N) : decode_tile(p, t, IG_BLOCK_M, BLOCK_N);
     if constexpr (EVAL_BN) {
       named_bar_sync(3, 256);
       for (int cc = threadIdx.x - 128; cc < BLOCK_N; cc += 256) {
@@ -234,13 +302,13 @@
       wgmma_commit();
       wgmma_fence_acc(acc);
       wgmma_wait<1>();
-      if (prev >= 0 && tid == 0) mbar_arrive(&empty_bar[prev]);
+      if (prev >= 0) release(prev);
       prev = s;
       if (++s == STAGES) { s = 0; ph ^= 1; }
     }
     wgmma_wait<0>();
     wgmma_fence_acc(acc);
-    if (prev >= 0 && tid == 0) mbar_arrive(&empty_bar[prev]);
+    if (prev >= 0) release(prev);
 
     const int row_a = c.m0 + 64 * g + row_in, row_b = row_a + 8;
     const bool ok_a = row_a < p.M, ok_b = row_b < p.M;
@@ -274,6 +342,7 @@
       }
     }
     if (p.stats != nullptr) {
+      float* ws = wsum + (4 * g + warp) * 2 * BLOCK_N;
 #pragma unroll
       for (int i = 0; i < NACC / 4; ++i) {
 #pragma unroll
@@ -286,8 +355,8 @@
             s2 += __shfl_xor_sync(0xffffffffu, s2, o);
           }
           if (lane < 4) {
-            atomicAdd(&colsum[8 * i + col_in + e], s1);
-            atomicAdd(&colsum[BLOCK_N + 8 * i + col_in + e], s2);
+            ws[8 * i + col_in + e] = s1;
+            ws[BLOCK_N + 8 * i + col_in + e] = s2;
           }
         }
       }
@@ -352,16 +421,24 @@
       named_bar_sync(3, 256);
       for (int cc = threadIdx.x - 128; cc < BLOCK_N; cc += 256) {
         if (c.n0 + cc < p.N) {
-          atomicAdd(p.stats + c.n0 + cc, colsum[cc]);
-          atomicAdd(p.stats + p.N + c.n0 + cc, colsum[BLOCK_N + cc]);
-        }
-        colsum[cc] = 0.f;
-        colsum[BLOCK_N + cc] = 0.f;
+          float s1 = 0.f, s2 = 0.f;
+#pragma unroll
+          for (int w = 0; w < 8; ++w) {
+            s1 += wsum[w * 2 * BLOCK_N + cc];
+            s2 += wsum[w * 2 * BLOCK_N + BLOCK_N + cc];
+          }
+          atomicAdd(p.stats + c.n0 + cc, s1);
+          atomicAdd(p.stats + p.N + c.n0 + cc, s2);
+        }
       }
       named_bar_sync(3, 256);
     }
   }
   if (p.tma_store && tid == 0) tma_store_wait_read();
+  if constexpr (CLUSTER) {
+    __syncwarp();
+    cluster_sync();
+  }
 }
 
 constexpr int PX_BLOCK_M = 256;
diff --git a/federated_pytorch_test_b200/csrc/sm90.cuh b/federated_pytorch_test_b200/csrc/sm90.cuh
--- a/federated_pytorch_test_b200/csrc/sm90.cuh
+++ b/federated_pytorch_test_b200/csrc/sm90.cuh
@@ -52,6 +52,23 @@
       : "memory");
 }
 
+__device__ __forceinline__ uint32_t cluster_ctarank() {
+  uint32_t r;
+  asm volatile("mov.u32 %0, %%cluster_ctarank;" : "=r"(r));
+  return r;
+}
+__device__ __forceinline__ void cluster_sync() {
+  asm volatile("barrier.cluster.arrive.release.aligned;\n\tbarrier.cluster.wait.acquire.aligned;" ::: "memory");
+}
+__device__ __forceinline__ void mbar_arrive_cluster(uint64_t* bar, uint32_t rank) {
+  asm volatile(
+      "{\n\t.reg .b32 ra;\n\t"
+      "mapa.shared::cluster.u32 ra, %0, %1;\n\t"
+      "mbarrier.arrive.release.cluster.shared::cluster.b64 _, [ra];\n\t}\n"
+      ::"r"(smem_u32(bar)), "r"(rank)
+      : "memory");
+}
+
 __device__ __forceinline__ void tma_prefetch_desc(const CUtensorMap* m) {
   asm volatile("prefetch.tensormap [%0];" ::"l"(reinterpret_cast<uint64_t>(m)) : "memory");
 }
@@ -66,6 +83,22 @@
   asm volatile(
       "cp.async.bulk.tensor.4d.shared::cluster.global.mbarrier::complete_tx::bytes [%0], [%1, {%3, %4, %5, %6}], [%2];"
       ::"r"(smem_u32(dst)), "l"(reinterpret_cast<uint64_t>(m)), "r"(smem_u32(bar)), "r"(c0), "r"(c1), "r"(c2), "r"(c3)
+      : "memory");
+}
+__device__ __forceinline__ void tma_load_2d_mc(void* dst, const CUtensorMap* m, uint64_t* bar, int c0, int c1, uint16_t mask) {
+  asm volatile(
+      "cp.async.bulk.tensor.2d.shared::cluster.global.mbarrier::complete_tx::bytes.multicast::cluster"
+      " [%0], [%1, {%3, %4}], [%2], %5;"
+      ::"r"(smem_u32(dst)), "l"(reinterpret_cast<uint64_t>(m)), "r"(smem_u32(bar)), "r"(c0), "r"(c1), "h"(mask)
+      : "memory");
+}
+__device__ __forceinline__ void tma_load_4d_mc(void* dst, const CUtensorMap* m, uint64_t* bar, int c0, int c1, int c2, int c3,
+                                               uint16_t mask) {
+  asm volatile(
+      "cp.async.bulk.tensor.4d.shared::cluster.global.mbarrier::complete_tx::bytes.multicast::cluster"
+      " [%0], [%1, {%3, %4, %5, %6}], [%2], %7;"
+      ::"r"(smem_u32(dst)), "l"(reinterpret_cast<uint64_t>(m)), "r"(smem_u32(bar)), "r"(c0), "r"(c1), "r"(c2), "r"(c3),
+        "h"(mask)
       : "memory");
 }
 
diff --git a/federated_pytorch_test_b200/ops/conv_math.py b/federated_pytorch_test_b200/ops/conv_math.py
--- a/federated_pytorch_test_b200/ops/conv_math.py
+++ b/federated_pytorch_test_b200/ops/conv_math.py
@@ -173,3 +173,94 @@
                         acc = acc + window[r: r + rows].reshape(rows * Wo, c1 - c0) @ w_krsc[:, r, s, c0:c1].t()
             y[n, h0: h0 + rows] = acc.view(rows, Wo, Co)
     return y
+
+
+CLUSTER_TILE = 128
+
+
+def cluster_tiles(m_tiles: int, n_tiles: int, k_splits: int):
+    assert n_tiles % 2 == 0, "the cluster launch pairs n-tiles"
+    n_pairs, m_pairs = n_tiles // 2, (m_tiles + 1) // 2
+    out = []
+    for cta in range(4 * m_pairs * n_pairs * k_splits):
+        q, rank = divmod(cta, 4)
+        rest, np_ = divmod(q, n_pairs)
+        z, mp = divmod(rest, m_pairs)
+        out.append((cta, rank, 2 * mp + (rank & 1), 2 * np_ + (rank >> 1), z))
+    return out
+
+
+def cluster_loads(rank: int):
+    return [("A", rank >> 1, (rank, rank ^ 2)), ("B", rank & 1, (rank, rank ^ 1))]
+
+
+def cluster_half_box(box_n: int, box_h: int, stride: int):
+    if box_n >= 2:
+        return box_n // 2, box_h, box_n // 2, 0
+    assert box_h % 2 == 0, "a one-image tile halves along its rows"
+    return 1, box_h // 2, 0, (box_h // 2) * stride
+
+
+def _nhwc_box(x: torch.Tensor, c0: int, w0: int, h0: int, img0: int, box_n: int, box_h: int, w_out: int, stride: int) -> torch.Tensor:
+    N, H, W, C = x.shape
+    out = x.new_zeros(box_n, box_h, w_out, 32)
+    for n in range(box_n):
+        i = img0 + n
+        if not 0 <= i < N:
+            continue
+        for hh in range(box_h):
+            h = h0 + hh * stride
+            if not 0 <= h < H:
+                continue
+            for ww in range(w_out):
+                w = w0 + ww * stride
+                if 0 <= w < W:
+                    out[n, hh, ww, : max(0, min(32, C - c0))] = x[i, h, w, c0: c0 + 32]
+    return out.reshape(-1, 32)
+
+
+def cluster_conv_oracle(x_nhwc: torch.Tensor, w_krsc: torch.Tensor, stride: int, pad: int, k_splits: int = 1) -> torch.Tensor:
+    N, H, W, Ci = x_nhwc.shape
+    Co, kh, kw, _ = w_krsc.shape
+    Ho, Wo = (H + 2 * pad - kh) // stride + 1, (W + 2 * pad - kw) // stride + 1
+    M, HW = N * Ho * Wo, Ho * Wo
+    rows = CLUSTER_TILE // Wo
+    box_h, box_n = (rows, 1) if rows <= Ho else (Ho, rows // Ho)
+    half_n, half_h, img_step, h_step = cluster_half_box(box_n, box_h, stride)
+    cblocks = -(-Ci // 32)
+    kb_total = kh * kw * cblocks
+    per = -(-kb_total // k_splits)
+    m_tiles, n_tiles = -(-M // CLUSTER_TILE), -(-Co // CLUSTER_TILE)
+    wmat = w_krsc.reshape(Co, kh * kw * Ci)
+    ctas = cluster_tiles(m_tiles, n_tiles, k_splits)
+    y = x_nhwc.new_zeros((m_tiles + 1) // 2 * 2 * CLUSTER_TILE, Co)
+    half = CLUSTER_TILE // 2
+    for cta, rank, m_t, n_t, z in ctas:
+        base = cta - rank
+        acc = x_nhwc.new_zeros(CLUSTER_TILE, CLUSTER_TILE)
+        for kb in range(z * per, min(kb_total, (z + 1) * per)):
+            tap, cb = divmod(kb, cblocks)
+            r, s = divmod(tap, kw)
+            a_stage = x_nhwc.new_zeros(CLUSTER_TILE, 32)
+            b_stage = x_nhwc.new_zeros(CLUSTER_TILE, 32)
+            for src in range(4):
+                _, _, sm, sn, _ = ctas[base + src]
+                for operand, h, dst in cluster_loads(src):
+                    if rank not in dst:
+                        continue
+                    if operand == "A":
+                        m0 = sm * CLUSTER_TILE
+                        img0 = m0 // HW
+                        h0 = ((m0 - img0 * HW) // Wo) * stride - pad
+                        a_stage[h * half: (h + 1) * half] = _nhwc_box(x_nhwc, cb * 32, s - pad, h0 + r + h * h_step,
+                                                                      img0 + h * img_step, half_n, half_h, Wo, stride)
+                    else:
+                        n_lo = sn * CLUSTER_TILE + h * half
+                        col = tap * Ci + cb * 32
+                        blk = wmat[n_lo: n_lo + half, col: col + min(32, Ci - cb * 32)]
+                        b_stage[h * half: h * half + blk.shape[0], : blk.shape[1]] = blk
+            acc = acc + a_stage @ b_stage.t()
+        n0 = n_t * CLUSTER_TILE
+        ncols = min(CLUSTER_TILE, Co - n0)
+        y[m_t * CLUSTER_TILE: (m_t + 1) * CLUSTER_TILE, n0: n0 + ncols] += acc[:, :ncols]
+    return y[:M].reshape(N, Ho, Wo, Co)
```
